# skokec/DAU-ConvNet

Hardware: AMD Instinct MI355X
Metric: DAU fwd+bwd GSamples/s (N*H*W/s) (higher is better)
Workload: dtype f32

## Files before the change

### dau-convnet_amd/csrc/dau_common.hpp

```cpp
#pragma once
#include <hip/hip_runtime.h>
#include <cstddef>
#include <cmath>
#include <cstdint>
#include <type_traits>
#include "dau_conv.h"

#ifdef DAU_TUNING
#include <cstdlib>
#define DAU_TUNE_INT(name, dflt) (getenv(name) ? atoi(getenv(name)) : (dflt))
#define DAU_TUNE_SET(name) (getenv(name) != nullptr)
#else
#define DAU_TUNE_INT(name, dflt) (dflt)
#define DAU_TUNE_SET(name) (false)
#endif

namespace dau {

enum ActFormat : int { kActF32 = 0, kActBF16 = 1, kActF16 = 2 };
__device__ __forceinline__ float f16_bits_to_float(unsigned bits) {
    return (float)__builtin_bit_cast(_Float16, (unsigned short)bits);
}
__device__ __forceinline__ float load_act(const float* base, long idx, int act) {
    if (act == kActF32) return base[idx];
// ... 8 lines not shown
__device__ __forceinline__ typename RawAct<A>::type load_raw(const float* base, long idx) {
    if constexpr (A == kActF32) return base[idx];
    else if constexpr (A == kActBF16) return reinterpret_cast<const unsigned short*>(base)[idx];
    else return F16Bits{reinterpret_cast<const unsigned short*>(base)[idx]};
}
__device__ __forceinline__ float act_of(float v) { return v; }
__device__ __forceinline__ float act_of(unsigned v) { return __uint_as_float(v << 16); }
__device__ __forceinline__ float act_of(F16Bits v) { return f16_bits_to_float(v.bits); }
template <int A>
__device__ __forceinline__ float load_act_t(const float* base, long idx) { return act_of(load_raw<A>(base, idx)); }
template <class F>
__device__ __forceinline__ void with_act(int act, F&& f) {
    if (act == kActBF16) f(std::integral_constant<int, kActBF16>{});
    else if (act == kActF16) f(std::integral_constant<int, kActF16>{});
    else f(std::integral_constant<int, kActF32>{});
}
constexpr int kNhwcArg = 0x100;
template <class T> struct NhwcOut : T {};
template <class T> struct IsNhwcOut : std::false_type {};
template <class T> struct IsNhwcOut<NhwcOut<T>> : std::true_type {};
constexpr int kEpiArg = 0x200;
template <class T> struct EpiOut : T {};
template <class T> struct IsEpiOut : std::false_type {};
template <class T> struct IsEpiOut<EpiOut<T>> : std::true_type {};
template <class T> struct IsNhwcOut<EpiOut<T>> : IsNhwcOut<T> {};
struct Epilogue {
    const float* bias = nullptr;
    bool relu = false;
    const float* residual = nullptr;
    const float* gate = nullptr;
    bool on() const { return bias != nullptr || relu || residual != nullptr || gate != nullptr; }
};
__device__ __forceinline__ float gate_value(float v, float g) { return g <= 0.0f ? 0.0f : v; }
__device__ __forceinline__ float epilogue_value(float v, float b, bool has_bias, bool relu, float r = 0.0f, bool has_res = false) {
    asm("" : "+v"(v));
    if (has_bias) v = v + b;
    asm("" : "+v"(v));
    if (has_res) v = v + r;
    asm("" : "+v"(v));
    return (relu && v <= 0.0f) ? 0.0f : v;
}
__device__ __forceinline__ long nhwc_index(long n, int c, int y, int x, int C, int H, int W) { return ((n * H + y) * W + x) * C + c; }
__device__ __forceinline__ int xcd_contiguous_id(int b, int nblk) {
    const int xcd = b % 8, idx = b / 8, per = nblk / 8, rem = nblk % 8;
    return (xcd < rem ? xcd * (per + 1) : rem * (per + 1) + (xcd - rem) * per) + idx;
}
__device__ __forceinline__ float relu_in(float v, bool on) { return (on && v <= 0.0f) ? 0.0f : v; }
__device__ __forceinline__ float mask_act(float v, bool keep) { return __uint_as_float(__float_as_uint(v) & (keep ? 0xffffffffu : 0u)); }
#ifndef DAU_LOAD_BATCH
#define DAU_LOAD_BATCH 6
#endif
constexpr int kLoadBatch = DAU_LOAD_BATCH;
template <class V, class Load, class Store>
__device__ __forceinline__ void load_phase(int rows_, int cols_, int wave, int nw, int lane, Load&& ld, Store&& st) {
    if (cols_ >= 56) {
        for (int x0 = 0; x0 < cols_; x0 += 64) {
            const int x = x0 + lane, xc = x < cols_ ? x : cols_ - 1;
            for (int r0 = wave; r0 < rows_; r0 += nw * kLoadBatch) {
                V v[kLoadBatch];
#pragma unroll
                for (int u = 0; u < kLoadBatch; ++u) { const int r = r0 + u * nw; v[u] = ld(r < rows_ ? r : rows_ - 1, xc); }
#pragma unroll
                for (int u = 0; u < kLoadBatch; ++u) { const int r = r0 + u * nw; if (r < rows_ && x < cols_) st(r, x, v[u]); }
            }
        }
    } else {
        const int total = rows_ * cols_;
        for (int t0 = wave * 64 + lane; t0 < total; t0 += nw * 64 * kLoadBatch) {
            V v[kLoadBatch];
            int rr[kLoadBatch];
#pragma unroll
            for (int u = 0; u < kLoadBatch; ++u) {
                const int t = t0 + u * nw * 64, tc = t < total ? t : total - 1;
                rr[u] = tc / cols_;
                v[u] = ld(rr[u], tc - rr[u] * cols_);
            }
#pragma unroll
            for (int u = 0; u < kLoadBatch; ++u) { const int t = t0 + u * nw * 64; if (t < total) st(rr[u], t - rr[u] * cols_, v[u]); }
        }
    }
}
__device__ __forceinline__ void store_act(float* base, long idx, float v, bool bf16, bool accumulate) {
    if (!bf16) { base[idx] = accumulate ? base[idx] + v : v; return; }
    unsigned short* p = reinterpret_cast<unsigned short*>(base) + idx;
    if (accumulate) v += __uint_as_float((unsigned)*p << 16);
    unsigned u = __float_as_uint(v);
    u = (v != v) ? 0x7fc00000u : u + 0x7fffu + ((u >> 16) & 1u);
    *p = (unsigned short)(u >> 16);
}
__device__ __forceinline__ unsigned bf16_bits(float v) {
    const unsigned u = __float_as_uint(v);
    return ((v != v) ? 0x7fc00000u : u + 0x7fffu + ((u >> 16) & 1u)) >> 16;
}
__device__ __forceinline__ void store_act_f16(float* base, long idx, float v, bool accumulate) {
    unsigned short* p = reinterpret_cast<unsigned short*>(base) + idx;
    if (accumulate) v += f16_bits_to_float(*p);
    *p = __builtin_bit_cast(unsigned short, (_Float16)v);
}
template <int A>
__device__ __forceinline__ void store_act_t(float* base, long idx, float v, bool accumulate) {
    if constexpr (A == kActF16) store_act_f16(base, idx, v, accumulate);
    else store_act(base, idx, v, A == kActBF16, accumulate);
}
__device__ __forceinline__ void store_act(float* base, long idx, float v, int act, bool accumulate) {
    if (act == kActF16) store_act_f16(base, idx, v, accumulate);
    else store_act(base, idx, v, act == kActBF16, accumulate);
}


constexpr int kMaxBlurSupport = 17;
constexpr int kFilterPlane = kMaxBlurSupport * kMaxBlurSupport;
constexpr int kNumK = 4;
constexpr int kTapPitch = 32;
enum Tap1d { kTapGX = 0, kTapGY, kTapAX, kTapAY, kTapCX, kTapBY, kTapGXR, kTapGYR, kNumTap1d };
constexpr int kTaps1dOffset = 6 * kFilterPlane;
constexpr int kFilterFloats = kTaps1dOffset + kNumTap1d * kTapPitch;

struct Status {
    unsigned int max_abs_mu_bits;
    unsigned int nan_seen;
    unsigned int ticket;
    unsigned int outlier_units;
    unsigned int off_line_units, line_radius;
    unsigned int dot_off_line_units, dot_line_radius;
};
constexpr unsigned kRingTakenBit = 0x80000000u;
static_assert(sizeof(Status) == 32, "the status block is eight words");
static_assert(offsetof(Status, max_abs_mu_bits) == 0 && offsetof(Status, nan_seen) == 4 && offsetof(Status, ticket) == 8 &&
              offsetof(Status, outlier_units) == 12 && offsetof(Status, off_line_units) == 16 && offsetof(Status, line_radius) == 20 &&
              offsetof(Status, dot_off_line_units) == 24 && offsetof(Status, dot_line_radius) == 28,
              "the status block keeps the order of its words");

struct HostStatus {
    unsigned int max_abs_mu_bits, nan_seen, valid, sigma_needed;
    unsigned int bad_max_abs_mu_bits, bad_nan_seen, sigma_worst, pad1;
};
static_assert(sizeof(HostStatus) == 32, "the pinned status mirror is 32 bytes (include/dau_conv.h, Ownership)");

struct Guard {
    const Status* status;
    float lo, hi;
    unsigned cnt_lo = 0u, cnt_hi = 0xffffffffu;
    float cnt_upto = INFINITY;
    int line = 0;
};
__device__ __forceinline__ bool guard_pass(const Guard& g) {
    if (!g.status) return true;
    const float mx = __uint_as_float(g.status->max_abs_mu_bits);
    const unsigned cnt = g.status->outlier_units & ~kRingTakenBit;
    if (!(mx > g.lo && mx <= g.hi && (mx > g.cnt_upto || (cnt >= g.cnt_lo && cnt <= g.cnt_hi)))) return false;
    if (g.line == 0) return true;
    const bool on_line = g.status->off_line_units == 0u;
    return g.line > 0 ? on_line : (mx > (float)-g.line || !on_line);
}

struct UnitRef {
    int ox, oy;
    float w00, w01, w10, w11;
};

struct Shape {
    int N, S, F, G, H, W;
};

void launch_synth_filters(hipStream_t st, const float* sigma_dev, int k, int flags, float* filters6, HostStatus* host_status = nullptr,
                          Status* status = nullptr);
void launch_synth_filters_compact(hipStream_t st, const float* sigma_dev, int k, int flags, float* planes6);
void launch_prepare_units(hipStream_t st, const float* w, const float* mu1, const float* mu2, Shape sh,
                          int ignore, int flags, int bucket, bool transposed_negated, UnitRef* table,
                          Status* status, HostStatus* host_status, int count_ignore = -1, Status* line_status = nullptr,
                          bool line_dot = false);
void launch_finalize_grads(hipStream_t st, const float* r4, const float* w, Shape sh, int ignore, float lr,
                           int need_mask, bool single_dim, float* dw, float* dmu1, float* dmu2, float* dsigma);
void launch_zero_words(hipStream_t st, void* p, size_t bytes);
void launch_blur_direct(hipStream_t st, const float* x, long planes, int H, int W, const float* filters,
                        int nfilt, int k, float* out);
void launch_gather_sum_direct(hipStream_t st, const float* xb, const UnitRef* table, int N, int Sin, int Fout,
                              int G, int H, int W, float* y);
void launch_gather_dot_direct(hipStream_t st, const float* xk4, const float* err, const UnitRef* table, Shape sh,
                              int drop_col, int drop_row, float* r4);

}
```

### dau-convnet_amd/csrc/dau_conv_api.hip

```cpp
#include <cmath>
#include <cstdarg>
#include <cstdio>
#include <algorithm>
#include <atomic>
#include <cstring>
#include <memory>
#include <mutex>
#include <new>
#include <string>
#include <utility>
#include <vector>

#include "dau_common.hpp"
#include "dau_tiled.hpp"

using namespace dau;

namespace {

thread_local std::string g_last_error;

int fail(int code, const char* fmt, ...) {
    char buf[512];
    va_list ap;
    va_start(ap, fmt);
    vsnprintf(buf, sizeof(buf), fmt, ap);
    va_end(ap);
    g_last_error = buf;
    return code;
}

#define DAU_HIP(expr)                                                                        \
    do {                                                                                     \
        hipError_t e_ = (expr);                                                              \
        if (e_ != hipSuccess) return fail(DAU_INTERNAL, "%s failed: %s", #expr, hipGetErrorString(e_)); \
    } while (0)

inline size_t align_up(size_t v, size_t a = 256) { return (v + a - 1) / a * a; }

struct Carver {
    char* base;
    size_t off = 0;
    explicit Carver(void* p) : base(static_cast<char*>(p)) {}
    template <typename T>
    T* take(size_t count) {
        T* p = base ? reinterpret_cast<T*>(base + off) : nullptr;
        off = align_up(off + count * sizeof(T));
        return p;
    }
};

inline const float* slab_ptr(const float* base, size_t elements, size_t esize) {
    return reinterpret_cast<const float*>(reinterpret_cast<const char*>(base) + elements * esize);
}
inline float* slab_ptr(float* base, size_t elements, size_t esize) {
    return reinterpret_cast<float*>(reinterpret_cast<char*>(base) + elements * esize);
}

int edge_disabled(int size) {
    if (size >= 64) return size % 64 == 0;
    if (size >= 32) return size % 32 == 0;
    if (size >= 16) return size % 16 == 0;
    if (size >= 8) return size % 8 == 0;
    return 0;
}

}

enum Member {
    kTiledGather,
    kSplit2, kSplit3, kSplit4,
    kLine4, kLine8,
    kBf16R3, kBf16R4,
    kTiledDot,
    kDotLine4, kDotLine8,
    kSplitDot,
    kWgradR3, kWgradR4,
    kNumMembers
};
enum PassKind { kGatherSum, kGatherDot };
enum Family { kFamTiledGather, kFamDense, kFamTiledDot, kFamSplitDot, kFamWgrad };
struct MemberInfo {
    int kind;
    int family;
    int slot;
    int radius;
    bool ahead;
    bool line;
    int info_bit;
};
constexpr MemberInfo kMember[kNumMembers] = {
    {kGatherSum, kFamTiledGather, 0, 0, false, false, -1},
    {kGatherSum, kFamDense, 0, 2, true, false, 2},
    {kGatherSum, kFamDense, 1, 3, true, false, 3},
    {kGatherSum, kFamDense, 2, 4, true, false, 4},
    {kGatherSum, kFamDense, 3, 4, true, true, 6},
    {kGatherSum, kFamDense, 4, 8, true, true, 7},
    {kGatherSum, kFamDense, 5, 3, true, false, -1},
    {kGatherSum, kFamDense, 6, 4, false, false, -1},
    {kGatherDot, kFamTiledDot, 0, 0, false, false, -1},
    {kGatherDot, kFamSplitDot, 0, 4, true, true, 8},
    {kGatherDot, kFamSplitDot, 1, 8, true, true, 9},
    {kGatherDot, kFamSplitDot, 2, 4, true, false, -1},
    {kGatherDot, kFamWgrad, 0, 3, true, false, -1},
    {kGatherDot, kFamWgrad, 1, 4, false, false, -1},
};
constexpr int kRingInfoBit = 5;
constexpr int kFirst[2] = {kTiledGather, kTiledDot}, kEnd[2] = {kTiledDot, kNumMembers};
enum Dir { kFwd, kDx };

struct DenseFns {
    bool (*configure)(int, int, int, int, int, int, int, int, int, DenseConfig*);
    size_t (*workspace_bytes)(const DenseConfig&);
    void (*init)(const DenseConfig&);
    void (*prepare)(hipStream_t, const DenseConfig&, const float*, const float*, bool, const UnitRef*, void*, const Guard&);
    void (*run)(hipStream_t, const DenseConfig&, float*, void*, const Guard&, const Epilogue&);
};
template <void (*Run)(hipStream_t, const DenseConfig&, float*, void*, const Guard&)>
void run_plain(hipStream_t st, const DenseConfig& c, float* out, void* ws, const Guard& g, const Epilogue&) { Run(st, c, out, ws, g); }
const DenseFns kDense[] = {
    {s2::split_gather_configure, s2::split_gather_workspace_bytes, s2::split_gather_init, s2::split_gather_prepare, s2::split_gather_run},
    {s3::split_gather_configure, s3::split_gather_workspace_bytes, s3::split_gather_init, s3::split_gather_prepare, s3::split_gather_run},
    {s4::split_gather_configure, s4::split_gather_workspace_bytes, s4::split_gather_init, s4::split_gather_prepare, s4::split_gather_run},
    {l4::split_gather_configure, l4::split_gather_workspace_bytes, l4::split_gather_init, l4::split_gather_prepare, l4::split_gather_run},
    {l8::split_gather_configure, l8::split_gather_workspace_bytes, l8::split_gather_init, l8::split_gather_prepare, l8::split_gather_run},
    {r3::dense_gather_configure, r3::dense_gather_workspace_bytes, r3::dense_gather_init, r3::dense_gather_prepare, run_plain<r3::dense_gather_run>},
    {r4::dense_gather_configure, r4::dense_gather_workspace_bytes, r4::dense_gather_init, r4::dense_gather_prepare, run_plain<r4::dense_gather_run>},
};
constexpr int kNumDense = sizeof(kDense) / sizeof(kDense[0]);
struct SplitDotFns {
    bool (*configure)(const Shape&, int, int, SplitDotConfig*);
    size_t (*workspace_bytes)(const SplitDotConfig&);
    void (*init)(const SplitDotConfig&);
    void (*prepare)(hipStream_t, const SplitDotConfig&, const float*, const float*, const float*, int, int, void*, const Guard&);
    void (*run)(hipStream_t, const SplitDotConfig&, const UnitRef*, float*, void*, const Guard&);
};
const SplitDotFns kSplitDotFns[] = {
    {d4::split_dot_configure, d4::split_dot_workspace_bytes, d4::split_dot_init, d4::split_dot_prepare, d4::split_dot_run},
    {d8::split_dot_configure, d8::split_dot_workspace_bytes, d8::split_dot_init, d8::split_dot_prepare, d8::split_dot_run},
    {split_dot_configure, split_dot_workspace_bytes, split_dot_init, split_dot_prepare, split_dot_run},
};
constexpr int kNumSplitDot = sizeof(kSplitDotFns) / sizeof(kSplitDotFns[0]);
struct WgradFns {
    bool (*configure)(const Shape&, int, bool, WgradConfig*);
    size_t (*workspace_bytes)(const WgradConfig&);
    void (*init)(const WgradConfig&);
    void (*run)(hipStream_t, const WgradConfig&, const float*, const float*, const float*, const UnitRef*, int, int, float*, void*,
                const Guard&, int);
};
const WgradFns kWgrad[] = {
    {r3::dense_wgrad_configure, r3::dense_wgrad_workspace_bytes, r3::dense_wgrad_init, r3::dense_wgrad_run},
    {r4::dense_wgrad_configure, r4::dense_wgrad_workspace_bytes, r4::dense_wgrad_init, r4::dense_wgrad_run},
};
static_assert(kMember[kBf16R4].slot == kNumDense - 1 && kMember[kSplitDot].slot == kNumSplitDot - 1 && kMember[kWgradR4].slot == 1,
              "a member's slot is its row in its family's function table");

struct BucketSet {
    int bucket = 0;
    bool has[kNumMembers] = {};
    TiledConfig tiled[2];
    DenseConfig dense[kNumDense][2];
    TiledDotConfig tiled_dot;
    SplitDotConfig sdot[kNumSplitDot];
    WgradConfig wgrad[2];
    int slab_gather = 0, slab_dot = 0;
    bool ring = false;
    unsigned ring_limit = 0;
    RingConfig ringcfg[2];
    const DenseConfig& ring_dense(int dir) const { return dense[kMember[kSplit3].slot][dir]; }
};
constexpr int kRingLimitPermille = 10;
constexpr int kBuckets[] = {4, 8, 16, 18, 20, 24, 32};
constexpr int kNumBuckets = sizeof(kBuckets) / sizeof(kBuckets[0]);

template <class F>
auto with_member(const BucketSet& bs, int m, int dir, F&& f) {
    const int i = kMember[m].slot;
    switch (kMember[m].family) {
    case kFamTiledGather: return f(tiled_gather_workspace_bytes, tiled_gather_init, bs.tiled[dir]);
    case kFamDense: return f(kDense[i].workspace_bytes, kDense[i].init, bs.dense[i][dir]);
    case kFamTiledDot: return f(tiled_dot_workspace_bytes, tiled_dot_init, bs.tiled_dot);
    case kFamSplitDot: return f(kSplitDotFns[i].workspace_bytes, kSplitDotFns[i].init, bs.sdot[i]);
    default: return f(kWgrad[i].workspace_bytes, kWgrad[i].init, bs.wgrad[i]);
    }
}
size_t pass_bytes(const BucketSet& bs, int kind, int dir = kFwd) {
    size_t need = 0;
    for (int m = kFirst[kind]; m < kEnd[kind]; ++m)
        if (bs.has[m]) need = std::max(need, with_member(bs, m, dir, [](auto bytes, auto, const auto& cfg) { return bytes(cfg); }));
    if (kind == kGatherSum && bs.ring) need = std::max(need, s3::split_gather_workspace_bytes(bs.ring_dense(dir)) + ring_workspace_bytes(bs.ringcfg[dir]));
    return need;
}

bool split_pays(double taps, int Cin, int Cout, int G_live, int H, int W) {
    const double hp = (H + 7) / 8 * 8, wp = (W + 7) / 8 * 8, fp = (Cout + 127) / 128 * 128, sp = (Cin + 15) / 16 * 16;
    const double dense = hp * wp * (fp * sp * taps * 3.0 / 16.0 / 0.55 + sp * 430.0);
    const double exact = (double)H * W * Cout * Cin * G_live * 4.0 / ((H < 32 || W < 32) ? 0.45 : 0.60);
    return dense < 1.1 * exact;
}

struct dau_conv_plan {
    dau_conv_desc d;
    Shape sh;
    int bucket;
    int blur_k;
    int drop_col, drop_row;
    int algo_fwd, algo_bwd;
    int nsets = 0;
    BucketSet sets[kNumBuckets];
    bool dynamic = false;
    HostStatus* host_status = nullptr;
    mutable std::atomic<unsigned long long> attrs_devices{0};
    mutable std::mutex attrs_mutex;
    const BucketSet& top() const { return sets[nsets - 1]; }
    long units() const { return (long)sh.S * sh.G * sh.F; }
    size_t esize() const { return (d.flags & (DAU_FLAG_IO_BF16 | DAU_FLAG_IO_F16)) ? 2 : 4; }
    int act() const { return (d.flags & DAU_FLAG_IO_F16) ? kActF16 : (d.flags & DAU_FLAG_IO_BF16) ? kActBF16 : kActF32; }
    mutable bool profiling = false;
    mutable std::vector<std::pair<hipEvent_t, hipEvent_t>> prof_events[DAU_PROFILE_SLOTS];
    mutable size_t prof_used[DAU_PROFILE_SLOTS] = {0, 0, 0};
    mutable int prof_passes[DAU_PROFILE_SLOTS] = {0, 0, 0};
};

namespace {

struct ProfScope {
    const dau_conv_plan* p;
    int slot;
    hipStream_t st;
    hipEvent_t stop = nullptr;
    ProfScope(const dau_conv_plan* plan, int slot_, hipStream_t st_) : p(plan), slot(slot_), st(st_) {
        if (!p->profiling) return;
        auto& pool = p->prof_events[slot];
        size_t& used = p->prof_used[slot];
        if (used == pool.size()) {
            hipEvent_t a, b;
            if (hipEventCreate(&a) != hipSuccess || hipEventCreate(&b) != hipSuccess) return;
            pool.emplace_back(a, b);
        }
        (void)hipEventRecord(pool[used].first, st);
        stop = pool[used].second;
        ++used;
    }
    ~ProfScope() {
        if (stop) (void)hipEventRecord(stop, st);
    }
};

struct Candidate {
    const BucketSet* set;
    Guard guard;
    int member;
    bool ring = false;
};

void clear_host_status(const dau_conv_plan* p) {
    if (!p->host_status) return;
    volatile HostStatus* h = p->host_status;
    h->valid = 0u; h->nan_seen = 0u; h->max_abs_mu_bits = 0u; h->bad_max_abs_mu_bits = 0u; h->bad_nan_seen = 0u;
}
void clear_reported_status(const dau_conv_plan* p, unsigned max_bits, bool nan_seen) {
    if (!p->host_status) return;
    volatile HostStatus* h = p->host_status;
    h->valid = 0u; h->nan_seen = 0u; h->max_abs_mu_bits = 0u;
    if (h->bad_max_abs_mu_bits == max_bits) h->bad_max_abs_mu_bits = 0u;
    if (nan_seen) h->bad_nan_seen = 0u;
}

int status_error(const dau_conv_plan* p, float mx, bool nan_seen) {
    if (nan_seen) return fail(DAU_FAILED_PRECONDITION, "DAUConvOp ERROR: got NaN value in offset (mu1,mu2) variable");
    if (mx > (float)p->bucket)
        return fail(DAU_INVALID_ARGUMENT,
                    "DAUConvOp ERROR: actual offsets (%.3f) larger than what max_kernel_size=%d allows (setup max_kernel_size "
                    "and dau_unit_border_bound correctly to avoid this)",
                    mx, p->d.max_kernel_size);
    return DAU_OK;
}

constexpr int kMaxCandidates = 14;
int pick_candidates(const dau_conv_plan* p, const Status* dev_status, int kind, Candidate out[kMaxCandidates]) {
    const BucketSet* top = &p->top();
    const BucketSet* s0 = &p->sets[0];
    auto member_of = [&](const BucketSet* b) {
        for (int m = kFirst[kind]; m < kEnd[kind]; ++m)
            if (kMember[m].radius && !kMember[m].ahead && b->has[m]) return m;
        return kFirst[kind];
    };
    out[0] = Candidate{top, Guard{nullptr, 0.0f, 0.0f}, member_of(top)};
    if (!p->dynamic) return 1;
    const BucketSet* hinted = nullptr;
    if (p->host_status && p->nsets >= 2) {
        const volatile HostStatus* h = p->host_status;
        float mx = -1.0f;
        if (h->valid == 1u && h->nan_seen == 0u) {
            const unsigned bits = h->max_abs_mu_bits;
            std::memcpy(&mx, &bits, sizeof(float));
        }
        if (mx >= 0.0f)
            for (int i = 0; i + 1 < p->nsets && !hinted; ++i)
                if (mx <= (float)p->sets[i].bucket && p->sets[i].has[kFirst[kind]]) hinted = &p->sets[i];
    }
    int n = 0;
    float lo = -1.0f;
    bool with_ring = false;
    int line_r = 0;
    for (int m = kFirst[kind]; m < kEnd[kind]; ++m) {
        if (!(kMember[m].line && s0->has[m])) continue;
        Guard g{dev_status, (float)line_r - (line_r ? 0.0f : 1.0f), (float)kMember[m].radius};
        g.line = kMember[m].radius;
        out[n++] = Candidate{s0, g, m};
        line_r = kMember[m].radius;
    }
    auto add = [&](const BucketSet* b, int member, float hi) {
        Guard g{dev_status, lo, hi};
        if (lo < (float)line_r) g.line = -line_r;
        if (with_ring && lo < 4.0f) { g.cnt_lo = s0->ring_limit + 1; g.cnt_upto = 4.0f; }
        out[n++] = Candidate{b, g, member};
        lo = hi;
    };
    for (int m = kFirst[kind]; m < kEnd[kind]; ++m) {
        if (!(kMember[m].ahead && s0->has[m]) || kMember[m].line) continue;
        add(s0, m, (float)kMember[m].radius);
        if (m == kSplit3 && s0->ring) {
            Guard g{dev_status, 3.0f, 4.0f, 0u, s0->ring_limit};
            g.line = -line_r;
            out[n++] = Candidate{s0, g, kSplit3, true};
            with_ring = true;
        }
    }
    if (member_of(s0) != kFirst[kind] && hinted != s0 && s0 != top) add(s0, member_of(s0), (float)s0->bucket);
    if (kind == kGatherDot) {
        for (int i = 0; i + 1 < p->nsets; ++i)
            if (p->sets[i].has[kFirst[kind]] && lo < (float)p->sets[i].bucket)
                add(&p->sets[i], member_of(&p->sets[i]), (float)p->sets[i].bucket);
    } else if (hinted && lo < (float)hinted->bucket) add(hinted, member_of(hinted), (float)hinted->bucket);
    if (n == 0) return 1;
    add(top, member_of(top), INFINITY);
    return n;
}

int ensure_attrs(const dau_conv_plan* p) {
    int dev = 0;
    DAU_HIP(hipGetDevice(&dev));
    const unsigned long long bit = 1ull << (dev & 63);
    if (p->attrs_devices.load(std::memory_order_acquire) & bit) return DAU_OK;
    std::lock_guard<std::mutex> lock(p->attrs_mutex);
    if (p->attrs_devices.load(std::memory_order_relaxed) & bit) return DAU_OK;
    (void)hipGetLastError();
    for (int i = 0; i < p->nsets; ++i) {
        const BucketSet& bs = p->sets[i];
        for (int m = 0; m < kNumMembers; ++m) {
            if (!bs.has[m]) continue;
            for (int dir = kFwd; dir <= (kMember[m].kind == kGatherSum ? kDx : kFwd); ++dir)
                with_member(bs, m, dir, [](auto, auto init, const auto& cfg) { init(cfg); });
        }
        if (bs.ring) ring_init();
        const hipError_t e = hipGetLastError();
        if (e != hipSuccess)
            return fail(DAU_INTERNAL, "raising the dynamic-LDS limit of the bucket-%d kernels failed: %s", bs.bucket,
                        hipGetErrorString(e));
    }
    p->attrs_devices.fetch_or(bit, std::memory_order_release);
    return DAU_OK;
}

size_t tiled_pass_bytes(const dau_conv_plan* p, int kind, int dir = kFwd) {
    size_t need = 0;
    for (int i = 0; i < p->nsets; ++i) need = std::max(need, pass_bytes(p->sets[i], kind, dir));
    return need;
}

struct FwdWs {
    Status* status;
    float* filters;
    UnitRef* table;
    void* gather;
    size_t bytes;
};

FwdWs carve_forward(const dau_conv_plan* p, void* ws) {
    Carver c(ws);
    FwdWs w{};
    w.status = c.take<Status>(1);
    w.filters = c.take<float>(kFilterFloats);
    w.table = c.take<UnitRef>(p->units());
    if (p->algo_fwd == DAU_ALGO_TILED) w.gather = c.take<char>(tiled_pass_bytes(p, kGatherSum, kFwd));
    else w.gather = c.take<float>((size_t)p->sh.N * p->sh.S * p->sh.H * p->sh.W);
    w.bytes = c.off;
    return w;
}

struct BwdWs {
    Status* status;
    float* filters;
    UnitRef* table_bare;
    UnitRef* table_t;
    float* r4;
    float* xk4;
    void* gather_dx;
    void* tiled_dot;
    size_t bytes;
};

BwdWs carve_backward(const dau_conv_plan* p, void* ws) {
    Carver c(ws);
    BwdWs w{};
    const Shape& s = p->sh;
    w.status = c.take<Status>(1);
    w.filters = c.take<float>(kFilterFloats);
    w.table_bare = c.take<UnitRef>(p->units());
    w.table_t = c.take<UnitRef>(p->units());
    w.r4 = c.take<float>(kNumK * p->units());
    if (p->algo_bwd == DAU_ALGO_TILED) w.tiled_dot = c.take<char>(tiled_pass_bytes(p, kGatherDot));
    else w.xk4 = c.take<float>((size_t)kNumK * s.N * s.S * s.H * s.W);
    if (p->algo_fwd == DAU_ALGO_TILED) w.gather_dx = c.take<char>(tiled_pass_bytes(p, kGatherSum, kDx));
    else w.gather_dx = c.take<float>((size_t)s.N * s.F * s.H * s.W);
    w.bytes = c.off;
    return w;
}

void run_gather_sum(const dau_conv_plan* p, hipStream_t st, int dir, const float* in, float* out, const float* filters,
                    const UnitRef* table, Status* status, void* ws, const Epilogue& epi = Epilogue{}) {
    const Shape& s = p->sh;
    const int cin = dir == kFwd ? s.S : s.F, cout = dir == kFwd ? s.F : s.S;
    const bool mirrored = dir == kDx;
    if (p->profiling) ++p->prof_passes[dir];
    if (p->algo_fwd != DAU_ALGO_TILED) {
        launch_blur_direct(st, in, (long)s.N * cin, s.H, s.W, filters + (mirrored ? 5 : 0) * kFilterPlane, 1, p->blur_k,
                           static_cast<float*>(ws));
        ProfScope prof(p, dir, st);
        launch_gather_sum_direct(st, static_cast<float*>(ws), table, s.N, cin, cout, s.G, s.H, s.W, out);
        return;
    }
    Candidate cand[kMaxCandidates];
    const int ncand = pick_candidates(p, status, kGatherSum, cand);
    for (int ci = 0; ci < ncand; ++ci) {
        const BucketSet& bs = *cand[ci].set;
        const Guard& g = cand[ci].guard;
        const int m = cand[ci].member;
        const bool ring = cand[ci].ring;
        void* ring_ws = ring ? static_cast<char*>(ws) + s3::split_gather_workspace_bytes(bs.ring_dense(dir)) : nullptr;
        if (ring) ring_build_list(st, bs.ringcfg[dir], table, ring_ws, g);
        for (int n0 = 0; n0 < s.N; n0 += bs.slab_gather) {
            const float* ins = slab_ptr(in, (size_t)n0 * cin * s.H * s.W, p->esize());
            float* outs = slab_ptr(out, (size_t)n0 * cout * s.H * s.W, p->esize());
            Epilogue epis = epi;
            if (epi.residual) epis.residual = slab_ptr(epi.residual, (size_t)n0 * cout * s.H * s.W, p->esize());
            if (epi.gate) epis.gate = slab_ptr(epi.gate, (size_t)n0 * cout * s.H * s.W, p->esize());
            if (m == kTiledGather) {
                const TiledConfig& cfg = bs.tiled[dir];
                const int nwin = tiled_gather_windows(cfg);
                for (int window = 0; window < nwin; ++window) {
                    tiled_gather_prepare(st, cfg, ins, filters, mirrored, table, ws, window, g);
                    ProfScope prof(p, dir, st);
                    tiled_gather_run(st, cfg, outs, ws, window > 0, g, window + 1 == nwin ? epis : Epilogue{});
                }
            } else {
                const DenseFns& fn = kDense[kMember[m].slot];
                const DenseConfig& cfg = bs.dense[kMember[m].slot][dir];
                fn.prepare(st, cfg, ins, filters, mirrored, table, ws, g);
                ProfScope prof(p, dir, st);
                if (ring) {
                    ring_run(st, bs.ringcfg[dir], s3::split_gather_staged(cfg, ws), ring_ws, status, g);
                    s3::split_gather_run_add(st, cfg, outs, ring_partial(bs.ringcfg[dir], ring_ws), ws, g, epis);
                } else {
                    fn.run(st, cfg, outs, ws, g, epis);
                }
            }
        }
    }
}

struct FlagRule {
    int flags, needs, excludes;
    const char* message;
};
constexpr int kWgradFlags = DAU_FLAG_DENSE_WGRAD_NEVER | DAU_FLAG_DENSE_WGRAD_ALWAYS;
constexpr int kNoSplitFlags = DAU_FLAG_DENSE_BF16 | DAU_FLAG_NO_DENSE_SPLIT;
constexpr FlagRule kFlagRules[] = {
    {DAU_FLAG_IO_F16, 0, DAU_FLAG_IO_BF16 | DAU_FLAG_DENSE_BF16 | kWgradFlags,
     "DAU_FLAG_IO_F16 excludes DAU_FLAG_IO_BF16, DAU_FLAG_DENSE_BF16 and DAU_FLAG_DENSE_WGRAD_NEVER / _ALWAYS"},
    {DAU_FLAG_DENSE_BF16, DAU_FLAG_IO_BF16, 0, "DAU_FLAG_DENSE_BF16 needs DAU_FLAG_IO_BF16 (it is the bf16 layer's gather-sum)"},
    {DAU_FLAG_DENSE_SPLIT_F16, 0, kNoSplitFlags, "DAU_FLAG_DENSE_SPLIT_F16 excludes DAU_FLAG_DENSE_BF16 and DAU_FLAG_NO_DENSE_SPLIT"},
    {DAU_FLAG_DENSE_SPLIT_OUTLIERS, 0, kNoSplitFlags, "DAU_FLAG_DENSE_SPLIT_OUTLIERS excludes DAU_FLAG_DENSE_BF16 and DAU_FLAG_NO_DENSE_SPLIT"},
    {DAU_FLAG_DENSE_SPLIT_LINE, DAU_FLAG_SINGLE_DIM_KERNEL, 0, "DAU_FLAG_DENSE_SPLIT_LINE needs DAU_FLAG_SINGLE_DIM_KERNEL"},
    {DAU_FLAG_DENSE_SPLIT_LINE, 0, kNoSplitFlags, "DAU_FLAG_DENSE_SPLIT_LINE excludes DAU_FLAG_DENSE_BF16 and DAU_FLAG_NO_DENSE_SPLIT"},
    {DAU_FLAG_SPLIT_DOT_LINE, DAU_FLAG_SINGLE_DIM_KERNEL, 0, "DAU_FLAG_SPLIT_DOT_LINE needs DAU_FLAG_SINGLE_DIM_KERNEL"},
    {DAU_FLAG_SPLIT_DOT_LINE, DAU_FLAG_USE_INTERPOLATION, 0, "DAU_FLAG_SPLIT_DOT_LINE needs DAU_FLAG_USE_INTERPOLATION"},
    {DAU_FLAG_SPLIT_DOT_LINE, 0, kNoSplitFlags, "DAU_FLAG_SPLIT_DOT_LINE excludes DAU_FLAG_DENSE_BF16 and DAU_FLAG_NO_DENSE_SPLIT"},
    {kWgradFlags, DAU_FLAG_DENSE_BF16, 0, "DAU_FLAG_DENSE_WGRAD_NEVER / _ALWAYS qualify DAU_FLAG_DENSE_BF16 and exclude each other"},
    {DAU_FLAG_DENSE_WGRAD_NEVER, 0, DAU_FLAG_DENSE_WGRAD_ALWAYS, "DAU_FLAG_DENSE_WGRAD_NEVER / _ALWAYS qualify DAU_FLAG_DENSE_BF16 and exclude each other"},
    {DAU_FLAG_IO_NHWC, 0, DAU_FLAG_DENSE_BF16 | kWgradFlags, "DAU_FLAG_IO_NHWC excludes DAU_FLAG_DENSE_BF16 and DAU_FLAG_DENSE_WGRAD_NEVER / _ALWAYS"},
    {DAU_FLAG_INPUT_RELU, 0, DAU_FLAG_DENSE_BF16, "DAU_FLAG_INPUT_RELU excludes DAU_FLAG_DENSE_BF16 (the bf16-product forms have no input prologue)"},
};

int validate_desc(const dau_conv_desc* desc, int& bucket, int& blur_k) {
    if (desc->struct_size != (int32_t)sizeof(dau_conv_desc))
        return fail(DAU_INVALID_ARGUMENT, "dau_conv_desc.struct_size %d != %zu", desc->struct_size, sizeof(dau_conv_desc));
    if (desc->batch < 1 || desc->in_channels < 1 || desc->out_channels < 1 || desc->units_per_channel < 1 ||
        desc->height < 1 || desc->width < 1)
        return fail(DAU_INVALID_ARGUMENT, "all of N,S,F,G,H,W must be >= 1");
    if (desc->number_units_ignore < 0 || desc->number_units_ignore >= desc->units_per_channel)
        return fail(DAU_INVALID_ARGUMENT, "number_units_ignore must be in [0, G)");
    if (desc->max_kernel_size < 3 || desc->max_kernel_size % 2 == 0)
        return fail(DAU_INVALID_ARGUMENT, "kernel_size must be odd and >= 3");
    bucket = 0;
    for (int b : kBuckets)
        if (!bucket && desc->max_kernel_size / 2 <= b) bucket = b;
    if (!bucket)
        return fail(DAU_INVALID_ARGUMENT,
                    "DAUConv: offsets larger than the 32 px the kernels stage (set max_kernel_size <= 65)");
    if (!(desc->sigma_hint > 0.0f))
        return fail(DAU_FAILED_PRECONDITION, "Must use sigma > 0 - initialize it with appropriate value");
    blur_k = dau_conv_filter_support(desc->sigma_hint);
    if (blur_k > kMaxBlurSupport)
        return fail(DAU_INVALID_ARGUMENT, "sigma %.3f needs a %dx%d prefilter; at most %dx%d is supported", desc->sigma_hint,
                    blur_k, blur_k, kMaxBlurSupport, kMaxBlurSupport);
    if (desc->algo < DAU_ALGO_AUTO || desc->algo > DAU_ALGO_TILED) return fail(DAU_INVALID_ARGUMENT, "unknown algo");
    for (const FlagRule& r : kFlagRules)
        if ((desc->flags & r.flags) && ((desc->flags & r.needs) != r.needs || (desc->flags & r.excludes)))
            return fail(DAU_INVALID_ARGUMENT, "%s", r.message);
    return DAU_OK;
}

void configure_set(const dau_conv_plan& p, double budget_bytes, BucketSet& bs) {
    const Shape& s = p.sh;
    const int flags = p.d.flags, b = bs.bucket, blur_k = p.blur_k, act = p.act(), ignore = p.d.number_units_ignore;
    const bool want_dense = (flags & DAU_FLAG_DENSE_BF16) && p.d.algo != DAU_ALGO_DIRECT;
    const bool split_forced = (flags & DAU_FLAG_DENSE_SPLIT_F16) != 0;
    const bool split_allowed = !(flags & kNoSplitFlags) && p.d.algo != DAU_ALGO_DIRECT;
    const int g_live = s.G - ignore;
    const long live_units = (long)s.S * s.F * g_live, ignored_units = (long)s.S * s.F * ignore;
    auto line_wanted = [&](int m, int flag) {
        return (flags & flag) && !(flags & DAU_FLAG_STATIC_BUCKET) && (kMember[m].radius == 4 || (p.bucket >= 8 && bs.has[m - 1]));
    };
    auto pays = [&](double taps) {
        return split_forced || (split_pays(taps, s.S, s.F, g_live, s.H, s.W) && split_pays(taps, s.F, s.S, g_live, s.H, s.W));
    };
    auto configure_dense = [&](int m, int n) {
        const int i = kMember[m].slot, r = kMember[m].radius;
        return kDense[i].configure(n, s.S, s.F, s.G, s.H, s.W, r, blur_k, act, &bs.dense[i][kFwd]) &&
               kDense[i].configure(n, s.F, s.S, s.G, s.H, s.W, r, blur_k, act, &bs.dense[i][kDx]);
    };
    auto configure_gather = [&](int n) {
        bs.has[kTiledGather] = tiled_gather_configure(n, s.S, s.F, s.G, s.H, s.W, b, blur_k, act, &bs.tiled[kFwd]) &&
                               tiled_gather_configure(n, s.F, s.S, s.G, s.H, s.W, b, blur_k, act, &bs.tiled[kDx]);
        const bool dense_set = b == 4 && bs.has[kTiledGather];
        for (int m = kBf16R4; m >= kSplit2; --m) {
            if (kMember[m].line) continue;
            const double side = 2.0 * kMember[m].radius + 1;
            const bool want = m == kBf16R4 ? want_dense : m == kBf16R3 ? bs.has[kBf16R4] : split_allowed && pays(side * side);
            bs.has[m] = dense_set && want && configure_dense(m, n);
        }
        for (int m = kLine4; m <= kLine8; ++m)
            bs.has[m] = dense_set && line_wanted(m, DAU_FLAG_DENSE_SPLIT_LINE) && split_allowed && pays(2.0 * kMember[m].radius + 1) &&
                        configure_dense(m, n);
        bs.ring = (flags & DAU_FLAG_DENSE_SPLIT_OUTLIERS) && bs.has[kSplit3];
        if (bs.ring) {
            bs.ring_limit = (unsigned)(live_units * DAU_TUNE_INT("DAU_RING_LIMIT_PERMILLE", kRingLimitPermille) / 1000);
            for (int dir : {kFwd, kDx}) ring_configure(bs.ring_dense(dir), (long)bs.ring_limit + ignored_units, &bs.ringcfg[dir]);
        }
        return std::max(pass_bytes(bs, kGatherSum, kFwd), pass_bytes(bs, kGatherSum, kDx));
    };
    auto configure_dot = [&](int n) {
        Shape sn = s; sn.N = n;
        bs.has[kTiledDot] = tiled_dot_configure(sn, b, blur_k, act, ignore, &bs.tiled_dot);
        return pass_bytes(bs, kGatherDot);
    };
    auto pick_slab = [&](auto&& configure) {
        int chosen = s.N;
        for (int n = s.N; n >= 2; --n) {
            if (s.N % n || (n != s.N && (n & 1))) continue;
            chosen = n;
            if ((double)configure(n) <= budget_bytes) break;
        }
        configure(chosen);
        return chosen;
    };
    bs.slab_gather = pick_slab(configure_gather);
    bs.slab_dot = pick_slab(configure_dot);
    const bool whole_dot = b == 4 && bs.has[kTiledDot] && bs.slab_dot == s.N;
    const int min_units = (flags & DAU_FLAG_DENSE_WGRAD_NEVER) ? 1 << 30 : (flags & DAU_FLAG_DENSE_WGRAD_ALWAYS) ? 1 : 3;
    for (int m = kWgradR4; m >= kWgradR3; --m) {
        const WgradFns& fn = kWgrad[kMember[m].slot];
        WgradConfig& cfg = bs.wgrad[kMember[m].slot];
        const bool want = m == kWgradR4 ? whole_dot && bs.has[kBf16R4] && s.G >= min_units : bs.has[kWgradR4] && bs.has[kBf16R3];
        bs.has[m] = want && fn.configure(s, blur_k, (flags & DAU_FLAG_IO_BF16) != 0, &cfg) && (double)fn.workspace_bytes(cfg) <= budget_bytes;
    }
    const bool interp2d = (flags & DAU_FLAG_USE_INTERPOLATION) && !(flags & DAU_FLAG_SINGLE_DIM_KERNEL);
    const bool fill = 4 * s.G >= 3 * 4 * ((s.G + 3) / 4);
    for (int m = kDotLine4; m <= kSplitDot; ++m) {
        const SplitDotFns& fn = kSplitDotFns[kMember[m].slot];
        SplitDotConfig& cfg = bs.sdot[kMember[m].slot];
        const bool want = kMember[m].line ? line_wanted(m, DAU_FLAG_SPLIT_DOT_LINE) : interp2d;
        bs.has[m] = split_allowed && whole_dot && (split_forced || fill) && want && fn.configure(s, blur_k, act, &cfg) &&
                    (double)fn.workspace_bytes(cfg) <= budget_bytes;
    }
    const int nhwc = (flags & DAU_FLAG_IO_NHWC) != 0, in_relu = (flags & DAU_FLAG_INPUT_RELU) != 0;
    auto mark = [&](auto& cfg, bool stages_x) { cfg.nhwc = nhwc; cfg.in_relu = stages_x && in_relu; };
    for (int dir : {kFwd, kDx}) {
        mark(bs.tiled[dir], dir == kFwd);
        for (DenseConfig* cfg : bs.dense) mark(cfg[dir], dir == kFwd);
    }
    mark(bs.tiled_dot, true);
    for (SplitDotConfig& cfg : bs.sdot) mark(cfg, true);
}

int finish_plan(dau_conv_plan* p) {
    const int flags = p->d.flags, algo = p->d.algo;
    const bool fwd_ok = p->top().has[kTiledGather], dot_ok = p->top().has[kTiledDot];
    const struct { int flag; const char* name; } tiled_only[] = {
        {DAU_FLAG_IO_F16, "DAU_FLAG_IO_F16"}, {DAU_FLAG_IO_BF16, "DAU_FLAG_IO_BF16"}, {DAU_FLAG_IO_NHWC, "DAU_FLAG_IO_NHWC"},
        {DAU_FLAG_INPUT_RELU, "DAU_FLAG_INPUT_RELU"}};
    for (const auto& t : tiled_only)
        if ((flags & t.flag) && (algo == DAU_ALGO_DIRECT || !(fwd_ok && dot_ok)))
            return fail(DAU_INVALID_ARGUMENT, "%s needs the tiled kernels, which do not support this shape / algo", t.name);
    if (algo == DAU_ALGO_TILED && !(fwd_ok && dot_ok)) return fail(DAU_INVALID_ARGUMENT, "DAU_ALGO_TILED does not support this shape");
    p->algo_fwd = (algo != DAU_ALGO_DIRECT && fwd_ok) ? DAU_ALGO_TILED : DAU_ALGO_DIRECT;
    p->algo_bwd = (algo != DAU_ALGO_DIRECT && dot_ok) ? DAU_ALGO_TILED : DAU_ALGO_DIRECT;
    bool ahead = false;
    for (int m = 0; m < kNumMembers; ++m) ahead = ahead || (kMember[m].ahead && p->sets[0].has[m]);
    p->dynamic = (p->nsets > 1 || ahead) && !(flags & DAU_FLAG_STATIC_BUCKET) &&
                 (p->algo_fwd == DAU_ALGO_TILED || p->algo_bwd == DAU_ALGO_TILED);
    if (!p->dynamic || p->algo_fwd != DAU_ALGO_TILED) p->sets[0].ring = false;
    return DAU_OK;
}

}

extern "C" {

int dau_conv_abi_version(void) { return DAU_CONV_ABI_VERSION; }

#ifndef DAU_BUILD_ID
#define DAU_BUILD_ID "unknown"
#endif
const char* dau_conv_build_id(void) { return DAU_BUILD_ID; }

const char* dau_conv_last_error(void) { return g_last_error.c_str(); }

int dau_conv_filter_support(float sigma) { return 2 * (int)std::ceil(5.0f * sigma) + 1; }

int dau_conv_plan_create(const dau_conv_desc* desc, dau_conv_plan** plan_out) {
    if (!desc || !plan_out) return fail(DAU_INVALID_ARGUMENT, "null argument");
    int bucket, blur_k;
    if (int rc = validate_desc(desc, bucket, blur_k)) return rc;

    std::unique_ptr<dau_conv_plan> p(new (std::nothrow) dau_conv_plan());
    if (!p) return fail(DAU_INTERNAL, "out of host memory");
    p->d = *desc;
    p->sh = Shape{desc->batch, desc->in_channels, desc->out_channels, desc->units_per_channel, desc->height, desc->width};
    p->bucket = bucket;
    p->blur_k = blur_k;
    const bool ut = desc->flags & DAU_FLAG_UNIT_TESTING;
    p->drop_col = ut ? edge_disabled(desc->width) : 0;
    p->drop_row = ut ? edge_disabled(desc->height) : 0;

    const char* budget_env = getenv("DAU_WORKSPACE_BUDGET_GB");
    const double budget_bytes = (budget_env ? atof(budget_env) : 12.0) * 1e9;
    for (int b : kBuckets) {
        if (b > bucket) break;
        BucketSet& bs = p->sets[p->nsets++];
        bs.bucket = b;
        configure_set(*p, budget_bytes, bs);
    }
    if (int rc = finish_plan(p.get())) return rc;
    void* hs = nullptr;
    if (hipHostMalloc(&hs, sizeof(HostStatus), hipHostMallocPortable | hipHostMallocMapped) == hipSuccess && hs) {
        std::memset(hs, 0, sizeof(HostStatus));
        p->host_status = static_cast<HostStatus*>(hs);
    } else {
        (void)hipGetLastError();
    }
    *plan_out = p.release();
    return DAU_OK;
}

int dau_conv_plan_destroy(dau_conv_plan* plan) {
    if (plan) {
        for (auto& pool : plan->prof_events)
            for (auto& ev : pool) { (void)hipEventDestroy(ev.first); (void)hipEventDestroy(ev.second); }
        if (plan->host_status) (void)hipHostFree(plan->host_status);
    }
    delete plan;
    return DAU_OK;
}

int dau_conv_profile_begin(dau_conv_plan* plan) {
    if (!plan) return fail(DAU_INVALID_ARGUMENT, "null argument");
    for (size_t& u : plan->prof_used) u = 0;
    for (int& n : plan->prof_passes) n = 0;
    plan->profiling = true;
    return DAU_OK;
}

int dau_conv_profile_end(dau_conv_plan* plan, double* ms_out, int32_t* passes_out) {
    if (!plan || !ms_out || !passes_out) return fail(DAU_INVALID_ARGUMENT, "null argument");
    plan->profiling = false;
    for (int slot = 0; slot < DAU_PROFILE_SLOTS; ++slot) {
        double total = 0.0;
        for (size_t i = 0; i < plan->prof_used[slot]; ++i) {
            auto& ev = plan->prof_events[slot][i];
            DAU_HIP(hipEventSynchronize(ev.second));
            float ms = 0.0f;
            DAU_HIP(hipEventElapsedTime(&ms, ev.first, ev.second));
            total += ms;
        }
        ms_out[slot] = total;
        passes_out[slot] = plan->prof_passes[slot];
        plan->prof_used[slot] = 0;
        plan->prof_passes[slot] = 0;
    }
    return DAU_OK;
}

int dau_conv_plan_get_info(const dau_conv_plan* plan, dau_conv_plan_info* info) {
    if (!plan || !info) return fail(DAU_INVALID_ARGUMENT, "null argument");
    info->offset_bucket = plan->bucket;
    info->blur_support = plan->blur_k;
    info->algo_forward = plan->algo_fwd;
    info->algo_backward = plan->algo_bwd;
    info->drop_last_col = plan->drop_col;
    info->drop_last_row = plan->drop_row;
    const BucketSet& top = plan->top();
    const bool* s0 = plan->sets[0].has;
    const bool tiled_fwd = plan->algo_fwd == DAU_ALGO_TILED;
    info->gather_patch = tiled_fwd ? top.tiled[kFwd].tiles_x * top.tiled[kFwd].tile_w : 0;
    info->gather_stack = tiled_fwd ? top.tiled[kFwd].stack : 0;
    info->dot_windows = plan->algo_bwd == DAU_ALGO_TILED ? top.tiled_dot.windows : 0;
    info->gather_windows = tiled_fwd ? top.tiled[kFwd].windows : 0;
    info->bucket_sets = plan->dynamic ? plan->nsets : 1;
    const bool dense_reachable = s0[kBf16R4] && (plan->nsets == 1 || plan->dynamic);
    info->gather_dense_bf16 = dense_reachable ? (s0[kWgradR4] ? 2 : 1) : 0;
    info->batch_slab_gather = top.slab_gather;
    info->batch_slab_dot = top.slab_dot;
    info->dot_region = top.has[kTiledDot] ? top.tiled_dot.region_cols * 100 + top.tiled_dot.region_rows : 0;
    info->gather_fblock = tiled_fwd ? top.tiled[kFwd].fblock : 0;
    info->gather_variant = tiled_fwd ? top.tiled[kFwd].variant : -1;
    info->dense_bf16_radius3 = dense_reachable && plan->dynamic && s0[kBf16R3] ? (s0[kWgradR3] ? 2 : 1) : 0;
    info->gather_dense_split = plan->sets[0].ring ? 1 << kRingInfoBit : 0;
    const bool tiled_pass[2] = {tiled_fwd, plan->algo_bwd == DAU_ALGO_TILED};
    for (int m = 0; m < kNumMembers; ++m)
        if (kMember[m].info_bit >= 0 && s0[m] && plan->dynamic && tiled_pass[kMember[m].kind])
            info->gather_dense_split |= 1 << kMember[m].info_bit;
    return DAU_OK;
}

int dau_conv_split_dot_geometry(const dau_conv_plan* plan, int32_t* region_width, int32_t* strip_items, int32_t* strip_k_steps) {
    if (!plan) return fail(DAU_INVALID_ARGUMENT, "null argument");
    int rw = 0, items = 0, steps = 0;
    for (int i = 0; i < plan->nsets && !rw; ++i) {
        const BucketSet& bs = plan->sets[i];
        if (!bs.has[kSplitDot]) continue;
        const SplitDotConfig& cfg = bs.sdot[kMember[kSplitDot].slot];
        rw = cfg.RW;
        split_dot_strip(cfg, &items, &steps);
    }
    if (region_width) *region_width = rw;
    if (strip_items) *strip_items = items;
    if (strip_k_steps) *strip_k_steps = steps;
    return DAU_OK;
}

int dau_conv_workspace_bytes(const dau_conv_plan* plan, int pass, size_t* bytes_out) {
    if (!plan || !bytes_out) return fail(DAU_INVALID_ARGUMENT, "null argument");
    if (pass == DAU_PASS_FORWARD) *bytes_out = carve_forward(plan, nullptr).bytes;
    else if (pass == DAU_PASS_BACKWARD) *bytes_out = carve_backward(plan, nullptr).bytes;
    else if (pass == DAU_PASS_EPILOGUE_BACKWARD)
        *bytes_out = epilogue_grad_workspace_bytes(plan->sh.N, plan->sh.F, plan->sh.H, plan->sh.W, plan->act(), plan->d.flags & DAU_FLAG_IO_NHWC);
    else return fail(DAU_INVALID_ARGUMENT, "pass must be DAU_PASS_FORWARD, DAU_PASS_BACKWARD or DAU_PASS_EPILOGUE_BACKWARD");
    return DAU_OK;
}

namespace {
int forward_pass(const dau_conv_plan* p, void* stream, const float* x, const float* w, const float* mu1,
                 const float* mu2, const float* sigma, float* y, void* workspace, size_t workspace_bytes, const Epilogue& epi) {
    if (!p || !x || !w || !mu1 || !mu2 || !sigma || !y || !workspace) return fail(DAU_INVALID_ARGUMENT, "null argument");
    FwdWs ws = carve_forward(p, workspace);
    if (workspace_bytes < ws.bytes)
        return fail(DAU_INVALID_ARGUMENT, "workspace too small: %zu < %zu", workspace_bytes, ws.bytes);
    hipStream_t st = static_cast<hipStream_t>(stream);
    if (int rc = ensure_attrs(p)) return rc;
    launch_synth_filters(st, sigma, p->blur_k, p->d.flags, ws.filters, p->host_status, ws.status);
    launch_prepare_units(st, w, mu1, mu2, p->sh, p->d.number_units_ignore, p->d.flags, p->bucket, false, ws.table, ws.status,
                         p->host_status, -1, p->sets[0].has[kLine4] ? ws.status : nullptr);
    run_gather_sum(p, st, kFwd, x, y, ws.filters, ws.table, ws.status, ws.gather, epi);
    DAU_HIP(hipPeekAtLastError());
    return DAU_OK;
}
}

int dau_conv_forward(const dau_conv_plan* p, void* stream, const float* x, const float* w, const float* mu1,
                     const float* mu2, const float* sigma, float* y, void* workspace, size_t workspace_bytes) {
    return forward_pass(p, stream, x, w, mu1, mu2, sigma, y, workspace, workspace_bytes, Epilogue{});
}

namespace {
int fused_store_supported(const dau_conv_plan* p, int epilogue, const char* what, const char* bf16_has) {
    if (!p) return fail(DAU_INVALID_ARGUMENT, "null argument");
    if (epilogue & ~(DAU_EPILOGUE_BIAS | DAU_EPILOGUE_RELU))
        return fail(DAU_INVALID_ARGUMENT, "unknown epilogue bits 0x%x (DAU_EPILOGUE_BIAS | DAU_EPILOGUE_RELU)", epilogue);
    if (p->algo_fwd != DAU_ALGO_TILED)
        return fail(DAU_INVALID_ARGUMENT, "the direct kernels take no fused %s (this plan's forward pass runs on them)", what);
    if (p->d.flags & DAU_FLAG_DENSE_BF16)
        return fail(DAU_INVALID_ARGUMENT, "DAU_FLAG_DENSE_BF16 plans take no fused %s (the bf16-product forms have %s)", what, bf16_has);
    return DAU_OK;
}
}

int dau_conv_epilogue_supported(const dau_conv_plan* p, int epilogue) { return fused_store_supported(p, epilogue, "epilogue", "none"); }

int dau_conv_forward_residual(const dau_conv_plan* p, void* stream, const float* x, const float* w, const float* mu1,
                              const float* mu2, const float* sigma, const float* bias, const float* residual, int epilogue,
                              float* y, void* workspace, size_t workspace_bytes) {
    Epilogue epi;
    if (residual || epilogue) {
        if (int rc = residual ? fused_store_supported(p, epilogue, "residual", "no epilogue") : dau_conv_epilogue_supported(p, epilogue)) return rc;
        if ((epilogue & DAU_EPILOGUE_BIAS) && !bias) return fail(DAU_INVALID_ARGUMENT, "DAU_EPILOGUE_BIAS without a bias");
        epi.bias = (epilogue & DAU_EPILOGUE_BIAS) ? bias : nullptr;
        epi.relu = (epilogue & DAU_EPILOGUE_RELU) != 0;
        epi.residual = residual;
    }
    return forward_pass(p, stream, x, w, mu1, mu2, sigma, y, workspace, workspace_bytes, epi);
}

int dau_conv_forward_epilogue(const dau_conv_plan* p, void* stream, const float* x, const float* w, const float* mu1,
                              const float* mu2, const float* sigma, const float* bias, int epilogue, float* y,
                              void* workspace, size_t workspace_bytes) {
    return dau_conv_forward_residual(p, stream, x, w, mu1, mu2, sigma, bias, nullptr, epilogue, y, workspace, workspace_bytes);
}

int dau_conv_epilogue_backward(const dau_conv_plan* p, void* stream, const float* dy, const float* y, int epilogue, float* dz,
                               float* dbias, void* workspace, size_t workspace_bytes) {
    if (!p || !dy) return fail(DAU_INVALID_ARGUMENT, "null argument");
    if (epilogue & ~(DAU_EPILOGUE_BIAS | DAU_EPILOGUE_RELU))
        return fail(DAU_INVALID_ARGUMENT, "unknown epilogue bits 0x%x (DAU_EPILOGUE_BIAS | DAU_EPILOGUE_RELU)", epilogue);
    const bool relu = (epilogue & DAU_EPILOGUE_RELU) != 0;
    if (!(epilogue & DAU_EPILOGUE_BIAS)) dbias = nullptr;
    if (relu && (!y || !dz)) return fail(DAU_INVALID_ARGUMENT, "DAU_EPILOGUE_RELU needs y and dz");
    const bool nhwc = (p->d.flags & DAU_FLAG_IO_NHWC) != 0;
    const Shape& s = p->sh;
    if (dbias) {
        const size_t need = epilogue_grad_workspace_bytes(s.N, s.F, s.H, s.W, p->act(), nhwc);
        if (!workspace || workspace_bytes < need)
            return fail(DAU_INVALID_ARGUMENT, "workspace too small: %zu < %zu", workspace ? workspace_bytes : (size_t)0, need);
    }
    if (!epilogue_grad_run(static_cast<hipStream_t>(stream), s.N, s.F, s.H, s.W, p->act(), nhwc, dy, y, relu, dz, dbias, workspace))
        return fail(DAU_INVALID_ARGUMENT, "activation tensor too large for the epilogue's backward pass");
    DAU_HIP(hipPeekAtLastError());
    return DAU_OK;
}

namespace {

int run_param_sums(const dau_conv_plan* p, hipStream_t st, const float* x, const float* dy, const float* mu1,
                   const float* mu2, const BwdWs& ws, float* r4, int kinds, const float* w = nullptr) {
    const Shape& s = p->sh;
    const bool dot_line = p->algo_bwd == DAU_ALGO_TILED && p->dynamic && p->sets[0].has[kDotLine4];
    launch_prepare_units(st, dot_line ? w : nullptr, mu1, mu2, s, p->d.number_units_ignore, p->d.flags, p->bucket, false, ws.table_bare,
                         ws.status, p->host_status, -1, dot_line ? ws.status : nullptr, true);
    if (p->profiling) ++p->prof_passes[2];
    if (p->algo_bwd == DAU_ALGO_TILED) {
        Candidate cand[kMaxCandidates];
        const int ncand = pick_candidates(p, ws.status, kGatherDot, cand);
        for (int ci = 0; ci < ncand; ++ci) {
            const BucketSet& bs = *cand[ci].set;
            const Guard& g = cand[ci].guard;
            const int m = cand[ci].member;
            const int slot = kMember[m].slot;
            if (kMember[m].family == kFamSplitDot) {
                const SplitDotFns& fn = kSplitDotFns[slot];
                fn.prepare(st, bs.sdot[slot], x, dy, ws.filters, p->drop_col, p->drop_row, ws.tiled_dot, g);
                ProfScope prof(p, 2, st);
                fn.run(st, bs.sdot[slot], ws.table_bare, r4, ws.tiled_dot, g);
            } else if (kMember[m].family == kFamWgrad) {
                ProfScope prof(p, 2, st);
                kWgrad[slot].run(st, bs.wgrad[slot], x, dy, ws.filters, ws.table_bare, p->drop_col, p->drop_row, r4, ws.tiled_dot, g, kinds);
            } else {
                for (int n0 = 0; n0 < s.N; n0 += bs.slab_dot) {
                    tiled_dot_prepare(st, bs.tiled_dot, slab_ptr(x, (size_t)n0 * s.S * s.H * s.W, p->esize()),
                                      slab_ptr(dy, (size_t)n0 * s.F * s.H * s.W, p->esize()), ws.filters, ws.table_bare,
                                      p->drop_col, p->drop_row, ws.tiled_dot, g);
                    ProfScope prof(p, 2, st);
                    tiled_dot_run(st, bs.tiled_dot, r4, ws.tiled_dot, g, n0 > 0);
                }
            }
        }
        if (dot_line) launch_zero_words(st, &ws.status->off_line_units, sizeof(unsigned));
    } else {
        launch_blur_direct(st, x, (long)s.N * s.S, s.H, s.W, ws.filters + 1 * kFilterPlane, kNumK, p->blur_k, ws.xk4);
        ProfScope prof(p, 2, st);
        launch_gather_dot_direct(st, ws.xk4, dy, ws.table_bare, s, p->drop_col, p->drop_row, r4);
    }
    return DAU_OK;
}

int check_backward_ws(const dau_conv_plan* p, void* workspace, size_t workspace_bytes, BwdWs* ws) {
    *ws = carve_backward(p, workspace);
    if (workspace_bytes < ws->bytes)
        return fail(DAU_INVALID_ARGUMENT, "workspace too small: %zu < %zu", workspace_bytes, ws->bytes);
    return DAU_OK;
}

}

int dau_conv_backward(const dau_conv_plan* p, void* stream, const float* x, const float* dy, const float* w,
                      const float* mu1, const float* mu2, const float* sigma, float* dx, float* dw, float* dmu1,
                      float* dmu2, float* dsigma, void* workspace, size_t workspace_bytes, int need_mask) {
    if (p && !x && (p->d.flags & DAU_FLAG_INPUT_RELU) && (need_mask & DAU_NEED_DX))
        return fail(DAU_INVALID_ARGUMENT, "DAU_FLAG_INPUT_RELU: the input-gradient pass masks dx by x, which is null");
    if (!p || !x || !dy || !w || !mu1 || !mu2 || !sigma || !workspace) return fail(DAU_INVALID_ARGUMENT, "null argument");
    if (((need_mask & DAU_NEED_DX) && !dx) || ((need_mask & DAU_NEED_DW) && !dw) ||
        ((need_mask & DAU_NEED_DMU1) && !dmu1) || ((need_mask & DAU_NEED_DMU2) && !dmu2) ||
        ((need_mask & DAU_NEED_DSIGMA) && !dsigma))
        return fail(DAU_INVALID_ARGUMENT, "need_mask asks for a gradient whose output pointer is null");
    BwdWs ws;
    if (int rc = check_backward_ws(p, workspace, workspace_bytes, &ws)) return rc;
    hipStream_t st = static_cast<hipStream_t>(stream);
    const Shape& s = p->sh;
    const int flags = p->d.flags;
    if (int rc = ensure_attrs(p)) return rc;
    launch_synth_filters(st, sigma, p->blur_k, flags, ws.filters, p->host_status, ws.status);

    const int param_mask = DAU_NEED_DW | DAU_NEED_DMU1 | DAU_NEED_DMU2 | DAU_NEED_DSIGMA;
    if (need_mask & param_mask) {
        run_param_sums(p, st, x, dy, mu1, mu2, ws, ws.r4, (need_mask & DAU_NEED_DSIGMA) ? 4 : 3, w);
        launch_finalize_grads(st, ws.r4, w, s, p->d.number_units_ignore, p->d.mu_learning_rate_factor, need_mask,
                              flags & DAU_FLAG_SINGLE_DIM_KERNEL, dw, dmu1, dmu2, dsigma);
    }
    if (need_mask & DAU_NEED_DX) {
        const bool fresh = !(need_mask & param_mask);
        launch_prepare_units(st, w, mu1, mu2, s, 0, flags, p->bucket, true, ws.table_t, fresh ? ws.status : nullptr,
                             p->host_status, p->d.number_units_ignore, p->sets[0].has[kLine4] ? ws.status : nullptr);
        Epilogue gate;
        if (flags & DAU_FLAG_INPUT_RELU) gate.gate = x;
        run_gather_sum(p, st, kDx, dy, dx, ws.filters, ws.table_t, ws.status, ws.gather_dx, gate);
    }
    DAU_HIP(hipPeekAtLastError());
    return DAU_OK;
}

int dau_conv_backward_param_sums(const dau_conv_plan* p, void* stream, const float* x, const float* dy, const float* mu1,
                                 const float* mu2, const float* sigma, float* sums_out, void* workspace,
                                 size_t workspace_bytes) {
    if (!p || !x || !dy || !mu1 || !mu2 || !sigma || !sums_out || !workspace) return fail(DAU_INVALID_ARGUMENT, "null argument");
    BwdWs ws;
    if (int rc = check_backward_ws(p, workspace, workspace_bytes, &ws)) return rc;
    hipStream_t st = static_cast<hipStream_t>(stream);
    if (int rc = ensure_attrs(p)) return rc;
    launch_synth_filters(st, sigma, p->blur_k, p->d.flags, ws.filters, p->host_status, ws.status);
    run_param_sums(p, st, x, dy, mu1, mu2, ws, sums_out, 4);
    DAU_HIP(hipPeekAtLastError());
    return DAU_OK;
}

int dau_conv_finalize_param_grads(const dau_conv_plan* p, void* stream, const float* sums, const float* w, float* dw,
                                  float* dmu1, float* dmu2, float* dsigma, int need_mask) {
    if (!p || !sums || !w) return fail(DAU_INVALID_ARGUMENT, "null argument");
    if (((need_mask & DAU_NEED_DW) && !dw) || ((need_mask & DAU_NEED_DMU1) && !dmu1) ||
        ((need_mask & DAU_NEED_DMU2) && !dmu2) || ((need_mask & DAU_NEED_DSIGMA) && !dsigma))
        return fail(DAU_INVALID_ARGUMENT, "need_mask asks for a gradient whose output pointer is null");
    launch_finalize_grads(static_cast<hipStream_t>(stream), sums, w, p->sh, p->d.number_units_ignore,
                          p->d.mu_learning_rate_factor, need_mask, p->d.flags & DAU_FLAG_SINGLE_DIM_KERNEL, dw, dmu1, dmu2,
                          dsigma);
    DAU_HIP(hipPeekAtLastError());
    return DAU_OK;
}

namespace {
int read_status(const dau_conv_plan* p, void* stream, const void* workspace, Status* h) {
    if (!p || !workspace) return fail(DAU_INVALID_ARGUMENT, "null argument");
    DAU_HIP(hipStreamSynchronize(static_cast<hipStream_t>(stream)));
    DAU_HIP(hipMemcpy(h, workspace, sizeof(Status), hipMemcpyDeviceToHost));
    return DAU_OK;
}
}

int dau_conv_check_status(const dau_conv_plan* p, void* stream, const void* workspace, float* max_abs_mu_out) {
    Status h;
    if (int rc = read_status(p, stream, workspace, &h)) return rc;
    float mx;
    std::memcpy(&mx, &h.max_abs_mu_bits, sizeof(float));
    if (max_abs_mu_out) *max_abs_mu_out = mx;
    if (h.nan_seen || mx > (float)p->bucket) clear_reported_status(p, h.max_abs_mu_bits, h.nan_seen != 0);
    return status_error(p, mx, h.nan_seen != 0);
}

int dau_conv_gather_outlier_status(const dau_conv_plan* p, void* stream, const void* workspace, int32_t* outlier_units,
                                   int32_t* ring_taken) {
    Status h;
    if (int rc = read_status(p, stream, workspace, &h)) return rc;
    if (outlier_units) *outlier_units = (int32_t)(h.outlier_units & ~kRingTakenBit);
    if (ring_taken) *ring_taken = (h.outlier_units & kRingTakenBit) ? 1 : 0;
    return DAU_OK;
}

int dau_conv_gather_line_status(const dau_conv_plan* p, void* stream, const void* workspace, int32_t* off_line_units,
                                int32_t* line_radius_taken) {
    Status h;
    if (int rc = read_status(p, stream, workspace, &h)) return rc;
    if (off_line_units) *off_line_units = (int32_t)h.off_line_units;
    if (line_radius_taken) *line_radius_taken = (int32_t)h.line_radius;
    return DAU_OK;
}

int dau_conv_dot_line_status(const dau_conv_plan* p, void* stream, const void* workspace, int32_t* off_line_units,
                             int32_t* line_radius_taken) {
    Status h;
    if (int rc = read_status(p, stream, workspace, &h)) return rc;
    if (off_line_units) *off_line_units = (int32_t)h.dot_off_line_units;
    if (line_radius_taken) *line_radius_taken = (int32_t)h.dot_line_radius;
    return DAU_OK;
}

int dau_conv_last_status(const dau_conv_plan* p, float* max_abs_mu_out, int32_t* valid_out) {
    if (!p) return fail(DAU_INVALID_ARGUMENT, "null argument");
    if (max_abs_mu_out) *max_abs_mu_out = 0.0f;
    if (valid_out) *valid_out = 0;
    if (!p->host_status) return DAU_OK;
    const volatile HostStatus* h = p->host_status;
    if (h->valid != 1u && h->bad_max_abs_mu_bits == 0u && h->bad_nan_seen == 0u) return DAU_OK;
    const unsigned bad_bits = h->bad_max_abs_mu_bits, bad_nan = h->bad_nan_seen;
    unsigned bits = h->max_abs_mu_bits, nan_seen = h->nan_seen | bad_nan;
    if (bad_bits > bits) bits = bad_bits;
    float mx;
    std::memcpy(&mx, &bits, sizeof(float));
    if (max_abs_mu_out) *max_abs_mu_out = mx;
    if (valid_out) *valid_out = 1;
    if (nan_seen || mx > (float)p->bucket) clear_host_status(p);
    return status_error(p, mx, nan_seen != 0);
}

int dau_conv_sigma_status(const dau_conv_plan* p, int32_t* needed_out, int32_t* planned_out, int32_t* worst_needed_out) {
    if (!p || !needed_out || !planned_out || !worst_needed_out) return fail(DAU_INVALID_ARGUMENT, "null argument");
    *needed_out = 0;
    *planned_out = p->blur_k;
    *worst_needed_out = 0;
    if (!p->host_status) return DAU_OK;
    volatile HostStatus* h = p->host_status;
    *needed_out = (int32_t)h->sigma_needed;
    *worst_needed_out = (int32_t)h->sigma_worst;
    h->sigma_worst = 0u;
    return DAU_OK;
}

int dau_conv_filters(const dau_conv_plan* p, void* stream, const float* sigma, float* filters_out) {
    if (!p || !sigma || !filters_out) return fail(DAU_INVALID_ARGUMENT, "null argument");
    launch_synth_filters_compact(static_cast<hipStream_t>(stream), sigma, p->blur_k, p->d.flags, filters_out);
    DAU_HIP(hipPeekAtLastError());
    return DAU_OK;
}

int dau_conv_unit_table(const dau_conv_plan* p, void* stream, const float* w, const float* mu1, const float* mu2, int form,
                        void* table_out) {
    if (!p || !mu1 || !mu2 || !table_out) return fail(DAU_INVALID_ARGUMENT, "null argument");
    if (form != 0 && form != 1) return fail(DAU_INVALID_ARGUMENT, "form must be 0 ([S][G][F]) or 1 ([F][G][S], negated offsets)");
    launch_prepare_units(static_cast<hipStream_t>(stream), w, mu1, mu2, p->sh, form == 1 ? 0 : p->d.number_units_ignore, p->d.flags,
                         p->bucket, form == 1, static_cast<UnitRef*>(table_out), nullptr, nullptr);
    DAU_HIP(hipPeekAtLastError());
    return DAU_OK;
}

}
```

### dau-convnet_amd/csrc/dau_tiled.hpp

```cpp
#pragma once
#include "dau_common.hpp"

namespace dau {

struct TiledConfig {
    int N, Cin, Cout, G, H, W;
    int R;
    int blur_k;
    int NP;
    int windows;
    int stack;
    int patches;
    int rows, pitch;
    int tiles_x, tiles_y;
    int tile_w;
    int fblock;
    int variant;
    int debug;
    int act;
    int nhwc;
    int in_relu;
};

bool tiled_gather_configure(int N, int Cin, int Cout, int G, int H, int W, int R, int blur_k, int act, TiledConfig* cfg);
size_t tiled_gather_workspace_bytes(const TiledConfig& cfg);
int tiled_gather_windows(const TiledConfig& cfg);
void tiled_gather_prepare(hipStream_t st, const TiledConfig& cfg, const float* in, const float* filters, bool mirrored,
                          const UnitRef* table, void* workspace, int window, const Guard& guard);
void tiled_gather_run(hipStream_t st, const TiledConfig& cfg, float* out, void* workspace, bool accumulate, const Guard& guard,
                      const Epilogue& epi = Epilogue{});
void tiled_gather_init(const TiledConfig& cfg);

struct DenseConfig {
    int N, Cin, Cout, G, H, W;
    int R, blur_k;
    int act;
    int nsub;
    int ftiles;
    int nhwc;
    int in_relu;
};
#define DAU_DECLARE_DENSE_GATHER(NS)                                                                                           \
    namespace NS {                                                                                                            \
    bool dense_gather_configure(int N, int Cin, int Cout, int G, int H, int W, int R, int blur_k, int act, DenseConfig* cfg);  \
    size_t dense_gather_workspace_bytes(const DenseConfig& cfg);                                                              \
    void dense_gather_init(const DenseConfig& cfg);                                                                           \
      \
    void dense_gather_prepare(hipStream_t st, const DenseConfig& cfg, const float* in, const float* filters, bool mirrored,   \
                              const UnitRef* table, void* workspace, const Guard& guard);                                     \
    void dense_gather_run(hipStream_t st, const DenseConfig& cfg, float* out, void* workspace, const Guard& guard);           \
    }
DAU_DECLARE_DENSE_GATHER(r4)
DAU_DECLARE_DENSE_GATHER(r3)

#define DAU_DECLARE_SPLIT_GATHER(NS)                                                                                           \
    namespace NS {                                                                                                            \
    bool split_gather_configure(int N, int Cin, int Cout, int G, int H, int W, int R, int blur_k, int act, DenseConfig* cfg);  \
    size_t split_gather_workspace_bytes(const DenseConfig& cfg);                                                              \
    void split_gather_init(const DenseConfig& cfg);                                                                           \
    void split_gather_prepare(hipStream_t st, const DenseConfig& cfg, const float* in, const float* filters, bool mirrored,   \
                              const UnitRef* table, void* workspace, const Guard& guard);                                     \
                                                      \
    void split_gather_run(hipStream_t st, const DenseConfig& cfg, float* out, void* workspace, const Guard& guard,            \
                          const Epilogue& epi = Epilogue{});                                                                  \
    }
DAU_DECLARE_SPLIT_GATHER(s2)
DAU_DECLARE_SPLIT_GATHER(s3)
DAU_DECLARE_SPLIT_GATHER(s4)
DAU_DECLARE_SPLIT_GATHER(l4)
DAU_DECLARE_SPLIT_GATHER(l8)

struct SplitStaged {
    const float* sx;
    const _Float16* xs;
    int Hs, Ws, nchunk;
};
namespace s3 {
SplitStaged split_gather_staged(const DenseConfig& cfg, const void* workspace);
void split_gather_run_add(hipStream_t st, const DenseConfig& cfg, float* out, const float* partial, void* workspace, const Guard& guard,
                          const Epilogue& epi = Epilogue{});
}
struct RingConfig {
    int N, Cin, Cout, G, H, W;
    int nchunk;
    int capacity;
};
void ring_configure(const DenseConfig& dense, long max_outlier_units, RingConfig* cfg);
size_t ring_workspace_bytes(const RingConfig& cfg);
void ring_build_list(hipStream_t st, const RingConfig& cfg, const UnitRef* table, void* workspace, const Guard& guard);
void ring_run(hipStream_t st, const RingConfig& cfg, const SplitStaged& staged, void* workspace, Status* status, const Guard& guard);
float* ring_partial(const RingConfig& cfg, void* workspace);
void ring_init();

struct TiledDotConfig {
    Shape sh;
    int R, blur_k;
    int NP;
    int variant;
    int windows;
    bool as1, one_tile;
    bool rw8;
    bool ring;
    int region_cols, region_rows;
    int rounds;
    int act;
    int ignore;
    int debug;
    int nhwc;
    int in_relu;
};

bool tiled_dot_configure(const Shape& sh, int R, int blur_k, int act, int ignore, TiledDotConfig* cfg);
size_t tiled_dot_workspace_bytes(const TiledDotConfig& cfg);
void tiled_dot_prepare(hipStream_t st, const TiledDotConfig& cfg, const float* x, const float* dy,
                       const float* filters, const UnitRef* table_bare, int drop_col, int drop_row, void* workspace,
                       const Guard& guard);
void tiled_dot_run(hipStream_t st, const TiledDotConfig& cfg, float* r4, void* workspace, const Guard& guard, bool accumulate);
void tiled_dot_init(const TiledDotConfig& cfg);

void launch_blur4_pack(hipStream_t st, const float* x, const float* filters, int N, int C, int cstride, int H, int W, int Hp,
                       int Wp, int blur_k, int act, float* xk, const Guard& guard, unsigned* kmax = nullptr, bool nhwc = false,
                       bool in_relu = false);
void blur4_pack_init(int blur_k, bool kmax = false, bool nhwc = false);
bool blur4_pack_fits(int blur_k, int Hp, int Wp);

void launch_dot_reduce(hipStream_t st, const void* partial, int partial_f32, long n, int G, int F, int g_split, int slabs0,
                       int slabs1, int zero_from, bool accumulate, float* r4, const Guard& guard);

struct SplitDotConfig {
    Shape sh;
    int blur_k;
    int RW;
    int act;
    int e_limbs;
    int nhwc;
    int in_relu;
};
bool split_dot_configure(const Shape& sh, int blur_k, int act, SplitDotConfig* cfg);
size_t split_dot_workspace_bytes(const SplitDotConfig& cfg);
void split_dot_strip(const SplitDotConfig& cfg, int* items, int* k_steps);
void split_dot_init(const SplitDotConfig& cfg);
void split_dot_prepare(hipStream_t st, const SplitDotConfig& cfg, const float* x, const float* dy, const float* filters,
                       int drop_col, int drop_row, void* workspace, const Guard& guard);
void split_dot_run(hipStream_t st, const SplitDotConfig& cfg, const UnitRef* table, float* r4, void* workspace, const Guard& guard);
#define DAU_DECLARE_SPLIT_DOT_LINE(NS)                                                                                         \
    namespace NS {                                                                                                            \
    bool split_dot_configure(const Shape& sh, int blur_k, int act, SplitDotConfig* cfg);                                      \
    size_t split_dot_workspace_bytes(const SplitDotConfig& cfg);                                                              \
    void split_dot_strip(const SplitDotConfig& cfg, int* items, int* k_steps);                                                \
    void split_dot_init(const SplitDotConfig& cfg);                                                                           \
    void split_dot_prepare(hipStream_t st, const SplitDotConfig& cfg, const float* x, const float* dy, const float* filters,  \
                           int drop_col, int drop_row, void* workspace, const Guard& guard);                                  \
    void split_dot_run(hipStream_t st, const SplitDotConfig& cfg, const UnitRef* table, float* r4, void* workspace,           \
                       const Guard& guard);                                                                                   \
    }
DAU_DECLARE_SPLIT_DOT_LINE(d4)
DAU_DECLARE_SPLIT_DOT_LINE(d8)

struct WgradConfig {
    Shape sh;
    int blur_k;
    int SB, FB, NC;
    int HsT, WsT, WT, nseg;
    int splits;
    int Hp, Wp;
    bool fused;
};
#define DAU_DECLARE_DENSE_WGRAD(NS)                                                                                            \
    namespace NS {                                                                                                            \
    bool dense_wgrad_configure(const Shape& sh, int blur_k, bool bf16, WgradConfig* cfg);                                     \
    size_t dense_wgrad_workspace_bytes(const WgradConfig& cfg);                                                               \
    void dense_wgrad_init(const WgradConfig& cfg);                                                                            \
    void dense_wgrad_run(hipStream_t st, const WgradConfig& cfg, const float* x, const float* dy, const float* filters,       \
                         const UnitRef* table, int drop_col, int drop_row, float* r4, void* workspace, const Guard& guard, int nk); \
    }
DAU_DECLARE_DENSE_WGRAD(r4)
DAU_DECLARE_DENSE_WGRAD(r3)

size_t epilogue_grad_workspace_bytes(long N, int F, int H, int W, int act, bool nhwc);
bool epilogue_grad_run(hipStream_t st, long N, int F, int H, int W, int act, bool nhwc, const float* dy, const float* y, bool relu,
                       float* dz, float* dbias, void* workspace);

}
```

### dau-convnet_amd/csrc/k_dense_split.hip

```cpp
#include <algorithm>
#include <cstdint>
#include <cstdlib>
#include <type_traits>
#include <utility>

#include "dau_tiled.hpp"

#ifndef DAU_SPLIT_R
#define DAU_SPLIT_R 3
#endif
#ifndef DAU_SPLIT_NS
#define DAU_SPLIT_NS s3
#endif

namespace dau {
namespace DAU_SPLIT_NS {

typedef _Float16 f16x8 __attribute__((ext_vector_type(8)));
typedef __attribute__((ext_vector_type(16))) float f32x16;
typedef __attribute__((ext_vector_type(4))) float f32x4;
typedef __attribute__((ext_vector_type(4))) unsigned u32x4;
typedef __attribute__((address_space(3))) void* lds_ptr_t;
typedef __attribute__((address_space(1))) const void* glb_ptr_t;

namespace {

constexpr int kDR = DAU_SPLIT_R;
constexpr int kDK = 2 * kDR + 1;
constexpr int kDSpan = kDK - 1;
#ifndef DAU_SPLIT_1D
#define DAU_SPLIT_1D 0
#endif
constexpr bool kLine = DAU_SPLIT_1D != 0;
#if DAU_SPLIT_1D
#define split_absmax_kernel line_absmax_kernel
#define split_scales_kernel line_scales_kernel
#define split_densify_kernel line_densify_kernel
#define split_stage_kernel line_stage_kernel
#define split_stage_walk_kernel line_stage_walk_kernel
#define split_gather_kernel line_gather_kernel
#endif
constexpr int kDRV = kLine ? 0 : kDR;
constexpr int kDKV = 2 * kDRV + 1;
constexpr int kDSpanV = kDKV - 1;
constexpr int kDTaps = kDKV * kDK;
constexpr int kDRows = 8;
constexpr int kDFB = 128;
constexpr int kAhead = 2;
#ifndef DAU_SPLIT_FLUSH_TAPS
#define DAU_SPLIT_FLUSH_TAPS 0
#endif
constexpr int kFlushTaps = DAU_SPLIT_FLUSH_TAPS > 0 ? DAU_SPLIT_FLUSH_TAPS : kDK;
#ifndef DAU_SPLIT_FLUSH_ROWS
#if DAU_SPLIT_1D
#define DAU_SPLIT_FLUSH_ROWS 1
#else
#define DAU_SPLIT_FLUSH_ROWS 4
#endif
#endif
constexpr int kFlushRows = DAU_SPLIT_FLUSH_ROWS;
#if !defined(DAU_SPLIT_K32)
#if !defined(DAU_SPLIT_MFMA32) && DAU_SPLIT_R == 3 && !DAU_SPLIT_1D
#define DAU_SPLIT_K32 1
#else
#define DAU_SPLIT_K32 0
#endif
#endif
constexpr bool kK32 = DAU_SPLIT_K32 != 0;

inline size_t round_up(size_t v, size_t a) { return (v + a - 1) / a * a; }

struct SplitScales {
    unsigned max_w_bits;
    float sw, inv_sw;
    float pad[5];
};
__host__ __device__ __forceinline__ const float* scales_sx(const SplitScales* sc) { return reinterpret_cast<const float*>(sc + 1); }
__host__ __device__ __forceinline__ const float* scales_inv_sx(const SplitScales* sc, int N) { return reinterpret_cast<const float*>(sc + 1) + N; }
constexpr int kPartials = 1024;
inline int absmax_groups_per_image(int N, long per) {
    const long fit = std::max(1, kPartials / N), want = (per / 4 + 255) / 256 + 1;
    return (int)std::min(fit, want);
}
inline size_t scales_bytes(int N) { return sizeof(SplitScales) + (size_t)2 * N * sizeof(float); }

constexpr int kMaxSub = 4;
struct SplitGeom {
    int sub;
    int nsub_a, nb_a, nsub_b, nb_b;
    int nrb8, nrb4;
    int tall;
    int Hs, Ws, nchunk, CoutP;
    size_t hdr_bytes, xs_bytes, ws_bytes;
};

SplitGeom split_geometry(const DenseConfig& c) {
    SplitGeom g{};
    g.sub = (c.W + 7) / 8;
    const int nblocks = (g.sub + kMaxSub - 1) / kMaxSub, base = g.sub / nblocks, rem = g.sub % nblocks;
    if (rem) { g.nsub_a = base + 1; g.nb_a = rem; g.nsub_b = base; g.nb_b = nblocks - rem; }
    else { g.nsub_a = base; g.nb_a = nblocks; g.nsub_b = 0; g.nb_b = 0; }
    const int left = c.H % kDRows;
    const long wgs = (long)c.N * ((c.H + kDRows - 1) / kDRows) * nblocks * ((c.Cout + kDFB - 1) / kDFB);
    const int rows4 = DAU_TUNE_INT("DAU_SPLIT_ROWS4", 1);
    g.nrb4 = (left >= 1 && left <= 4 && rows4 != 0 && (wgs >= 1024 || rows4 == 2)) ? 1 : 0;
    g.nrb8 = c.H / kDRows + (left && !g.nrb4 ? 1 : 0);
    g.Hs = g.nrb8 * kDRows + g.nrb4 * 4 + kDSpanV;
    {
        const int t4 = (c.W + 3) / 4;
        const long rows8 = (long)g.nrb8 * kDRows;
        const long flat = (long)(g.nrb4 ? rows8 + 4 : (c.H + 3) / 4 * 4) * g.sub * 8;
        const long tall = rows8 * t4 * 4 + (g.nrb4 ? 4L * g.sub * 8 : 0);
        const int want = DAU_TUNE_INT("DAU_SPLIT_TALL", 1);
        g.tall = (want != 0 && g.nrb8 > 0 && (t4 == 5 || t4 == 7) && (tall * 20 <= flat * 19 || want == 2)) ? t4 : 0;
    }
    g.Ws = g.sub * 8 + kDSpan;
    g.nchunk = (c.Cin + 15) / 16;
    g.CoutP = (int)round_up(c.Cout, kDFB);
    g.hdr_bytes = round_up(scales_bytes(c.N) + (size_t)2 * (kPartials + c.N) * sizeof(unsigned), 256);
    g.xs_bytes = round_up((size_t)c.N * g.nchunk * 4 * g.Hs * g.Ws * 16 + 4096, 256);
    g.ws_bytes = round_up(((size_t)g.nchunk * kDTaps + 8) * 2 * g.CoutP * 32, 256);
    return g;
}

constexpr int lds_pitch(int nsub) {
    int p = nsub * 8 + kDSpan;
    while (p % 16 != 8) ++p;
    return p;
}
constexpr int lds_pitch_narrow(int ntiles) {
    int p = ntiles * 4 + kDSpan;
    while (p % 16 != 4 && p % 16 != 12) ++p;
    return p;
}

}

__device__ __forceinline__ unsigned finite_bits(unsigned b) { return b < 0x7f800000u ? b : 0u; }

__device__ __forceinline__ long absmax_head(const void* p, long per, int elem_bytes, int vec_bytes) {
    const uintptr_t a = reinterpret_cast<uintptr_t>(p);
    if (a % elem_bytes) return per;
    const long head = (long)((vec_bytes - a % vec_bytes) % vec_bytes) / elem_bytes;
    return head < per ? head : per;
}

__global__ void __launch_bounds__(256) split_absmax_kernel(const float* __restrict__ in, long per, int gpi, int act, const UnitRef* __restrict__ table,
                                                           long units, unsigned* __restrict__ partial, int cap, const Guard guard, int relu_in) {
    if (!guard_pass(guard)) return;
    unsigned mx = 0, mw = 0;
    const unsigned keep = relu_in ? 0xffffffffu : 0x7fffffffu, keep_hi = keep & 0xffff0000u;
    const int n = blockIdx.x / gpi, j = blockIdx.x - n * gpi;
    const long stride = (long)gpi * blockDim.x, t0 = j * (long)blockDim.x + threadIdx.x;
    if (act == kActF16) {
        auto wide = [keep](unsigned h) { return finite_bits(__float_as_uint(f16_bits_to_float(h)) & keep); };
        const unsigned short* e = reinterpret_cast<const unsigned short*>(in) + n * per;
        const long head = absmax_head(e, per, 2, 8), n4 = (per - head) / 4;
        const uint2* p = reinterpret_cast<const uint2*>(e + head);
        for (long i = t0; i < n4; i += stride) {
            const uint2 v = p[i];
            mx = max(mx, max(max(wide(v.x & 0xffffu), wide(v.x >> 16)), max(wide(v.y & 0xffffu), wide(v.y >> 16))));
        }
        for (long i = t0; i < per - n4 * 4; i += stride) mx = max(mx, wide(e[i < head ? i : i + n4 * 4]));
    } else if (act == kActBF16) {
        const unsigned short* e = reinterpret_cast<const unsigned short*>(in) + n * per;
        const long head = absmax_head(e, per, 2, 8), n4 = (per - head) / 4;
        const uint2* p = reinterpret_cast<const uint2*>(e + head);
        for (long i = t0; i < n4; i += stride) {
            const uint2 v = p[i];
            mx = max(mx, max(max(finite_bits((v.x << 16) & keep), finite_bits(v.x & keep_hi)),
                             max(finite_bits((v.y << 16) & keep), finite_bits(v.y & keep_hi))));
        }
        for (long i = t0; i < per - n4 * 4; i += stride) mx = max(mx, finite_bits(((unsigned)e[i < head ? i : i + n4 * 4] << 16) & keep));
    } else {
        const float* e = in + n * per;
        const long head = absmax_head(e, per, 4, 16), n4 = (per - head) / 4;
        const uint4* p = reinterpret_cast<const uint4*>(e + head);
        for (long i = t0; i < n4; i += stride) {
            const uint4 v = p[i];
            mx = max(mx, max(max(finite_bits(v.x & keep), finite_bits(v.y & keep)),
                             max(finite_bits(v.z & keep), finite_bits(v.w & keep))));
        }
        for (long i = t0; i < per - n4 * 4; i += stride) mx = max(mx, finite_bits(__float_as_uint(e[i < head ? i : i + n4 * 4]) & keep));
    }
    for (long u = blockIdx.x * (long)blockDim.x + threadIdx.x; u < units; u += (long)gridDim.x * blockDim.x) {
        const UnitRef r = table[u];
        mw = max(mw, finite_bits(__float_as_uint(fabsf(r.w00) + fabsf(r.w01) + fabsf(r.w10) + fabsf(r.w11))));
    }
    __shared__ unsigned sx[4], sw[4];
    for (int m = 32; m >= 1; m >>= 1) { mx = max(mx, (unsigned)__shfl_xor((int)mx, m)); mw = max(mw, (unsigned)__shfl_xor((int)mw, m)); }
    if ((threadIdx.x & 63) == 0) { sx[threadIdx.x >> 6] = mx; sw[threadIdx.x >> 6] = mw; }
    __syncthreads();
    if (threadIdx.x == 0) {
        partial[blockIdx.x] = max(max(sx[0], sx[1]), max(sx[2], sx[3]));
        partial[cap + blockIdx.x] = max(max(sw[0], sw[1]), max(sw[2], sw[3]));
    }
}

__device__ __forceinline__ float limb_scale(float m) {
    if (!(m > 0.0f) || !(m < INFINITY)) return 1.0f;
    int e = ilogbf(m);
    e = 13 - e;
    e = e > 100 ? 100 : (e < -100 ? -100 : e);
    return ldexpf(1.0f, e);
}

__global__ void __launch_bounds__(256) split_scales_kernel(const unsigned* __restrict__ partial, int N, int gpi, int cap, int G,
                                                           SplitScales* __restrict__ out, const Guard guard) {
    if (!guard_pass(guard)) return;
    const int n = blockIdx.x;
    const unsigned* src = n < N ? partial + (long)n * gpi : partial + cap;
    const int cnt = n < N ? gpi : N * gpi;
    unsigned m = 0;
    for (int i = threadIdx.x; i < cnt; i += 256) m = max(m, src[i]);
    __shared__ unsigned sm[4];
    for (int k = 32; k >= 1; k >>= 1) m = max(m, (unsigned)__shfl_xor((int)m, k));
    if ((threadIdx.x & 63) == 0) sm[threadIdx.x >> 6] = m;
    __syncthreads();
    if (threadIdx.x == 0) {
        m = max(max(sm[0], sm[1]), max(sm[2], sm[3]));
        float* sx = reinterpret_cast<float*>(out + 1);
        if (n < N) {
            const float s = limb_scale(__uint_as_float(m));
            sx[n] = s; sx[N + n] = 1.0f / s;
        } else {
            const float s = limb_scale(__uint_as_float(m) * (float)G);
            out->max_w_bits = m; out->sw = s; out->inv_sw = 1.0f / s;
            if constexpr (kLine) { if (guard.status) const_cast<Status*>(guard.status)->line_radius = (unsigned)kDR; }
        }
    }
}

constexpr int kScT = 64;
__global__ void __launch_bounds__(kScT) split_densify_kernel(const UnitRef* __restrict__ table, int Cin, int G, int Cout, int CoutP, int nchunk,
                                                             const SplitScales* __restrict__ sc, _Float16* __restrict__ wsd, const Guard guard) {
    __shared__ float acc[kDTaps * kScT];
    if (!guard_pass(guard)) return;
    constexpr int FPB = kScT / 16;
    const int tid = threadIdx.x, sl = tid & 15;
    const int fq = blockIdx.x % (CoutP / FPB), chunk = blockIdx.x / (CoutP / FPB);
    const int f = fq * FPB + (tid >> 4), c = chunk * 16 + sl;
#pragma unroll 7
    for (int tap = 0; tap < kDTaps; ++tap) acc[tap * kScT + tid] = 0.0f;
    if (c < Cin && f < Cout) {
        for (int g = 0; g < G; ++g) {
            const UnitRef u = table[((long)c * G + g) * Cout + f];
            const int ty = u.oy + kDRV, tx = u.ox + kDR;
            const bool y0 = ty >= 0 && ty < kDKV, y1 = ty + 1 >= 0 && ty + 1 < kDKV, x0 = tx >= 0 && tx < kDK, x1 = tx + 1 >= 0 && tx + 1 < kDK;
            if (y0 && x0) acc[(ty * kDK + tx) * kScT + tid] += u.w00;
            if (y0 && x1) acc[(ty * kDK + tx + 1) * kScT + tid] += u.w01;
            if (y1 && x0) acc[((ty + 1) * kDK + tx) * kScT + tid] += u.w10;
            if (y1 && x1) acc[((ty + 1) * kDK + tx + 1) * kScT + tid] += u.w11;
        }
    }
    const float sw = sc->sw;
    _Float16* dst = wsd + ((long)chunk * kDTaps * 2 * CoutP + f) * 16 + sl;
    const long limb = (long)CoutP * 16, tapstride = 2 * limb;
#pragma unroll 7
    for (int tap = 0; tap < kDTaps; ++tap) {
        const float v = acc[tap * kScT + tid] * sw;
        const _Float16 hi = (_Float16)v;
        dst[tap * tapstride] = hi;
        dst[tap * tapstride + limb] = (_Float16)(v - (float)hi);
    }
}

constexpr int kSP = 80;
struct SplitStageArgs {
    const float* in;
    const float* taps;
    const SplitScales* sc;
    _Float16* xs;
    int N, C, H, W, mirrored;
    int Hs, Ws, nchunk;
    int RB, nbands, nsegs;
    int TW;
    int vec;
    int relu_in;
    Guard guard;
};

__device__ __forceinline__ int fast_div(int i, int d, float inv) {
    int q = (int)(((float)i + 0.5f) * inv);
    const int r = i - q * d;
    q += (r >= d) - (r < 0);
    return q;
}

template <int K, int NCH>
__device__ __forceinline__ void split_stage_rows(float* rawl, const float* px, int col, int ch0, int wave, int nw, int lh, int ncols) {
    constexpr int kr = (K - 1) / 2;
    if (col >= ncols) return;
    float gx[K];
#pragma unroll
    for (int j = 0; j < K; ++j) gx[j] = px[j];
    for (int r = wave; r < lh; r += nw) {
        float* row = rawl + (r * 8 + ch0) * kSP + 8 + col;
        float acc[NCH];
#pragma unroll
        for (int ch = 0; ch < NCH; ++ch) {
            acc[ch] = 0.0f;
#pragma unroll
            for (int i = 0; i < K; ++i) acc[ch] = fmaf(row[ch * kSP + i - kr], gx[i], acc[ch]);
        }
#pragma unroll
        for (int ch = 0; ch < NCH; ++ch) row[ch * kSP] = acc[ch];
    }
}

template <int K, int NCH>
__device__ __forceinline__ void split_stage_walk(const float* rawl, const float* py, float sx, int col, int ch0, int ya, int yb,
                                                 int y0, int x0, int x1, int Ws, u32x4* xhi, u32x4* xlo) {
    constexpr int kr = (K - 1) / 2;
    const int x = x0 + col;
    if (x >= x1) return;
    float gy[K];
#pragma unroll
    for (int j = 0; j < K; ++j) gy[j] = py[j];
    float ring[K][NCH];
    const int nin = yb - ya + 2 * kr;
    char* dhi = reinterpret_cast<char*>(xhi + (long)kDRV * Ws + kDR + x) + ch0 * 2;
    char* dlo = reinterpret_cast<char*>(xlo + (long)kDRV * Ws + kDR + x) + ch0 * 2;
    for (int s0 = 0; s0 < nin; s0 += K) {
#pragma unroll
        for (int j = 0; j < K; ++j) {
            const int s = s0 + j;
            if (s < nin) {
                const float* row = rawl + ((ya - y0 + s) * 8 + ch0) * kSP + 8 + col;
#pragma unroll
                for (int ch = 0; ch < NCH; ++ch) ring[j][ch] = row[ch * kSP];
                if (s >= K - 1) {
                    typedef _Float16 f16xn __attribute__((ext_vector_type(NCH)));
                    f16xn oh, ol;
#pragma unroll
                    for (int ch = 0; ch < NCH; ++ch) {
                        float acc = 0.0f;
#pragma unroll
                        for (int i = 0; i < K; ++i) acc = fmaf(ring[(j + 1 + i) % K][ch], gy[i], acc);
                        acc *= sx;
                        const _Float16 hi = (_Float16)acc;
                        oh[ch] = hi;
                        ol[ch] = (_Float16)(acc - (float)hi);
                    }
                    const long o = (long)(ya + s - (K - 1)) * Ws * 16;
                    *reinterpret_cast<f16xn*>(dhi + o) = oh;
                    *reinterpret_cast<f16xn*>(dlo + o) = ol;
                }
            }
        }
    }
}

#ifndef DAU_SPLIT_STAGE_THREADS
#define DAU_SPLIT_STAGE_THREADS 512
#endif
constexpr int kStageThreads = DAU_SPLIT_STAGE_THREADS;
template <int KN, int A>
__global__ void __launch_bounds__(kStageThreads) split_stage_kernel(const SplitStageArgs a) {
    constexpr int K = KN & (kNhwcArg - 1);
    constexpr bool NHWC = (KN & kNhwcArg) != 0;
    extern __shared__ __attribute__((aligned(16))) float rawl[];
    if (!guard_pass(a.guard)) return;
    constexpr int kr = (K - 1) / 2;
    constexpr int PPR = kSP / 4;
    const int lane = threadIdx.x & 63, wave = threadIdx.x >> 6, nw = blockDim.x >> 6;
    int t = blockIdx.x;
    const int seg = t % a.nsegs; t /= a.nsegs;
    const int band = t % a.nbands; t /= a.nbands;
    const int grp = t % (2 * a.nchunk);
    const int n = t / (2 * a.nchunk);
    const int y0 = band * a.RB, y1 = y0 + a.RB < a.H ? y0 + a.RB : a.H;
    const int x0 = seg * 64, x1 = x0 + 64 < a.W ? x0 + 64 : a.W;
    const int lh = y1 - y0 + 2 * kr;
    const long plane = (long)a.H * a.W;
    const bool ri = a.relu_in != 0;
    if constexpr (NHWC) {
        constexpr int CPP = A == kActF32 ? 4 : 8, PARTS = 8 / CPP;
        const int pieces = lh * kSP * PARTS;
        constexpr int UB = (13 * 256 + kStageThreads - 1) / kStageThreads;
        for (int i0 = threadIdx.x; i0 < pieces; i0 += kStageThreads * UB) {
            float v[UB][CPP];
#pragma unroll
            for (int u = 0; u < UB; ++u) {
                const int i = i0 + u * kStageThreads, part = i % PARTS, rj = i / PARTS, r = rj / kSP, j = rj - r * kSP;
// ... 737 lines not shown
        run(std::integral_constant<int, NT0>{});
    }
}

namespace {

template <int NSUB, int RG, bool TT>
constexpr size_t split_lds_bytes() {
    constexpr int plane = (4 * RG + kDSpanV) * (TT ? lds_pitch_narrow(NSUB) : lds_pitch(NSUB));
    return (kK32 ? 4 : 2) * (size_t)((4 * (kK32 ? (plane + 15) / 16 * 16 : plane) + 63) / 64) * 1024;
}

template <int NSUB, int RG, bool TT = false>
void launch_split(hipStream_t st, const SplitArgsEpi* a, int grid, bool h16, bool add, bool nhwc, bool epi) {
    constexpr int NH = NSUB | kNhwcArg;
    constexpr int EP = NSUB | kEpiArg, EH = NH | kEpiArg;
    constexpr size_t lds = split_lds_bytes<NSUB, RG, TT>();
    if (epi) {
        auto kern = h16 ? split_gather_kernel<EP, RG, TT, true> : split_gather_kernel<EP, RG, TT, false>;
        if (nhwc) kern = h16 ? split_gather_kernel<EH, RG, TT, true> : split_gather_kernel<EH, RG, TT, false>;
#if DAU_SPLIT_R == 3
        if (add) kern = h16 ? split_gather_kernel<EP, RG, TT, true, true> : split_gather_kernel<EP, RG, TT, false, true>;
        if (add && nhwc) kern = h16 ? split_gather_kernel<EH, RG, TT, true, true> : split_gather_kernel<EH, RG, TT, false, true>;
#endif
        if (!a) { (void)hipFuncSetAttribute(reinterpret_cast<const void*>(kern), hipFuncAttributeMaxDynamicSharedMemorySize, 160 * 1024); return; }
        hipLaunchKernelGGL(kern, dim3(grid), dim3(512), lds, st, *a);
        return;
    }
    auto kern = h16 ? split_gather_kernel<NSUB, RG, TT, true> : split_gather_kernel<NSUB, RG, TT, false>;
    if (nhwc) kern = h16 ? split_gather_kernel<NH, RG, TT, true> : split_gather_kernel<NH, RG, TT, false>;
#if DAU_SPLIT_R == 3
    if (add) kern = h16 ? split_gather_kernel<NSUB, RG, TT, true, true> : split_gather_kernel<NSUB, RG, TT, false, true>;
    if (add && nhwc) kern = h16 ? split_gather_kernel<NH, RG, TT, true, true> : split_gather_kernel<NH, RG, TT, false, true>;
#endif
    if (!a) { (void)hipFuncSetAttribute(reinterpret_cast<const void*>(kern), hipFuncAttributeMaxDynamicSharedMemorySize, 160 * 1024); return; }
    hipLaunchKernelGGL(kern, dim3(grid), dim3(512), lds, st, static_cast<const SplitArgs&>(*a));
}

void dispatch_split(int nsub, int rg, bool h16, hipStream_t st, const SplitArgsEpi* a, int grid, bool tall, bool add, bool nhwc, bool epi) {
    if (tall) {
        if (nsub == 5) launch_split<5, 2, true>(st, a, grid, h16, add, nhwc, epi);
        else launch_split<7, 2, true>(st, a, grid, h16, add, nhwc, epi);
        return;
    }
    if (rg == 1) {
        switch (nsub) {
            case 1: launch_split<1, 1>(st, a, grid, h16, add, nhwc, epi); break;
            case 2: launch_split<2, 1>(st, a, grid, h16, add, nhwc, epi); break;
            case 3: launch_split<3, 1>(st, a, grid, h16, add, nhwc, epi); break;
            default: launch_split<4, 1>(st, a, grid, h16, add, nhwc, epi); break;
        }
        return;
    }
    switch (nsub) {
        case 1: launch_split<1, 2>(st, a, grid, h16, add, nhwc, epi); break;
        case 2: launch_split<2, 2>(st, a, grid, h16, add, nhwc, epi); break;
        case 3: launch_split<3, 2>(st, a, grid, h16, add, nhwc, epi); break;
        default: launch_split<4, 2>(st, a, grid, h16, add, nhwc, epi); break;
    }
}

const void* stage_for(int blur_k, int act, bool nhwc = false) {
#define DAU_SPLIT_STAGE(K) case K: if (nhwc) return act == kActF16 ? reinterpret_cast<const void*>(split_stage_kernel<K | kNhwcArg, kActF16>) : \
                                          act == kActBF16 ? reinterpret_cast<const void*>(split_stage_kernel<K | kNhwcArg, kActBF16>) : \
                                                            reinterpret_cast<const void*>(split_stage_kernel<K | kNhwcArg, kActF32>); \
                                   return act == kActF16 ? reinterpret_cast<const void*>(split_stage_kernel<K, kActF16>) : \
                                          act == kActBF16 ? reinterpret_cast<const void*>(split_stage_kernel<K, kActBF16>) : \
                                                            reinterpret_cast<const void*>(split_stage_kernel<K, kActF32>)
    switch (blur_k) {
        DAU_SPLIT_STAGE(3);
        DAU_SPLIT_STAGE(5);
        DAU_SPLIT_STAGE(7);
        DAU_SPLIT_STAGE(9);
        DAU_SPLIT_STAGE(11);
        default: return nullptr;
    }
#undef DAU_SPLIT_STAGE
}
const void* stage_walk_for(int blur_k, int act) {
#ifdef DAU_SPLIT_STAGE_REF
    return nullptr;
#else
#define DAU_SPLIT_STAGE_WALK(K) case K: return act == kActF16 ? reinterpret_cast<const void*>(split_stage_walk_kernel<K, kActF16>) : \
                                               act == kActBF16 ? reinterpret_cast<const void*>(split_stage_walk_kernel<K, kActBF16>) : \
                                                                 reinterpret_cast<const void*>(split_stage_walk_kernel<K, kActF32>)
    switch (blur_k) {
        DAU_SPLIT_STAGE_WALK(3);
        DAU_SPLIT_STAGE_WALK(5);
        DAU_SPLIT_STAGE_WALK(7);
        DAU_SPLIT_STAGE_WALK(9);
        DAU_SPLIT_STAGE_WALK(11);
        default: return nullptr;
    }
#undef DAU_SPLIT_STAGE_WALK
#endif
}
void stage_walk_plan(const DenseConfig& c, const SplitGeom& g, SplitStageArgs* s) {
    s->nsegs = (g.Ws + 63) / 64;
    s->TW = (g.Ws + s->nsegs - 1) / s->nsegs;
    s->nsegs = (g.Ws + s->TW - 1) / s->TW;
    const long waves = (long)c.N * 2 * g.nchunk * s->nsegs;
    long nb = (2048 + waves - 1) / waves;
    nb = std::min<long>(nb, std::max(1, g.Hs / (2 * c.blur_k)));
    const int rb = DAU_TUNE_INT("DAU_SPLIT_STAGE_WALK_RB", 0);
    s->RB = rb > 0 ? rb : (int)((g.Hs + nb - 1) / nb);
    s->nbands = (g.Hs + s->RB - 1) / s->RB;
}
void stage_plan(const DenseConfig& c, int* RB, int* nbands, size_t* lds) {
    const int kr = (c.blur_k - 1) / 2;
    int rows = 52 * 1024 / (8 * kSP * 4) - 2 * kr;
    const int rb = DAU_TUNE_INT("DAU_SPLIT_STAGE_RB", 0);
    if (rb > 0) rows = rb;
    rows = rows < 4 ? 4 : rows;
    const int nb = (c.H + rows - 1) / rows;
    *nbands = nb; *RB = (c.H + nb - 1) / nb;
    *lds = (size_t)(*RB + 2 * kr) * 8 * kSP * 4;
}

}

bool split_gather_configure(int N, int Cin, int Cout, int G, int H, int W, int R, int blur_k, int act, DenseConfig* cfg) {
    if (R != kDR || !stage_for(blur_k, act)) return false;
    DenseConfig c{};
    c.N = N; c.Cin = Cin; c.Cout = Cout; c.G = G; c.H = H; c.W = W; c.R = R; c.blur_k = blur_k; c.act = act;
    const SplitGeom g = split_geometry(c);
    c.nsub = g.nsub_a;
    c.ftiles = 1;
    if ((size_t)g.nchunk * 4 * g.Hs * g.Ws > (size_t)1 << 30) return false;
    *cfg = c;
    return true;
}

size_t split_gather_workspace_bytes(const DenseConfig& c) {
    const SplitGeom g = split_geometry(c);
    return g.hdr_bytes + g.xs_bytes + g.ws_bytes;
}

void split_gather_init(const DenseConfig& c) {
    const SplitGeom g = split_geometry(c);
    const bool h16 = c.act == kActF16;
    for (int rg = 1; rg <= 2; ++rg) {
        if (!(rg == 2 ? g.nrb8 : g.nrb4)) continue;
        for (int v = 0; v < (kDR == 3 ? 4 : 2); ++v) {
            const bool add = (v & 2) != 0, epi = (v & 1) != 0;
            if (rg == 2 && g.tall) { dispatch_split(g.tall, 2, h16, nullptr, nullptr, 0, true, add, c.nhwc != 0, epi); continue; }
            dispatch_split(g.nsub_a, rg, h16, nullptr, nullptr, 0, false, add, c.nhwc != 0, epi);
            if (g.nb_b) dispatch_split(g.nsub_b, rg, h16, nullptr, nullptr, 0, false, add, c.nhwc != 0, epi);
        }
    }
    (void)hipFuncSetAttribute(stage_for(c.blur_k, c.act, c.nhwc != 0), hipFuncAttributeMaxDynamicSharedMemorySize, 160 * 1024);
}

void split_gather_prepare(hipStream_t st, const DenseConfig& c, const float* in, const float* filters, bool mirrored,
                          const UnitRef* table, void* workspace, const Guard& guard) {
    const SplitGeom g = split_geometry(c);
    char* ws = static_cast<char*>(workspace);
    SplitScales* sc = reinterpret_cast<SplitScales*>(ws);
    unsigned* partial = reinterpret_cast<unsigned*>(ws + scales_bytes(c.N));
    _Float16* xs = reinterpret_cast<_Float16*>(ws + g.hdr_bytes);
    _Float16* wsd = reinterpret_cast<_Float16*>(ws + g.hdr_bytes + g.xs_bytes);
    const long per = (long)c.Cin * c.H * c.W, units = (long)c.Cin * c.G * c.Cout;
    const int gpi = absmax_groups_per_image(c.N, per), cap = kPartials + c.N;
    hipLaunchKernelGGL(split_absmax_kernel, dim3(c.N * gpi), dim3(256), 0, st, in, per, gpi, c.act, table, units, partial, cap, guard,
                       (c.in_relu && !mirrored) ? 1 : 0);
    hipLaunchKernelGGL(split_scales_kernel, dim3(c.N + 1), dim3(256), 0, st, partial, c.N, gpi, cap, c.G, sc, guard);
    hipLaunchKernelGGL(split_densify_kernel, dim3(g.nchunk * (g.CoutP / (kScT / 16))), dim3(kScT), 0, st, table, c.Cin, c.G, c.Cout, g.CoutP,
                       g.nchunk, sc, wsd, guard);
    SplitStageArgs s{};
    s.in = in; s.taps = filters + kTaps1dOffset; s.sc = sc; s.xs = xs;
    s.N = c.N; s.C = c.Cin; s.H = c.H; s.W = c.W; s.mirrored = mirrored ? 1 : 0;
    s.Hs = g.Hs; s.Ws = g.Ws; s.nchunk = g.nchunk; s.guard = guard;
    s.relu_in = (c.in_relu && !mirrored) ? 1 : 0;
    if (const void* walk = c.nhwc ? nullptr : stage_walk_for(c.blur_k, c.act)) {
        stage_walk_plan(c, g, &s);
        void* args[] = {&s};
        (void)hipLaunchKernel(walk, dim3(c.N * 2 * g.nchunk * s.nbands * s.nsegs), dim3(64), args, 0, st);
        return;
    }
    size_t lds;
    stage_plan(c, &s.RB, &s.nbands, &lds);
    s.nsegs = (c.W + 63) / 64;
    s.vec = c.W % 4 == 0 && reinterpret_cast<uintptr_t>(in) % 16 == 0;
    if (c.nhwc) s.vec = c.Cin % (c.act == kActF32 ? 4 : 8) == 0 && reinterpret_cast<uintptr_t>(in) % 16 == 0;
    void* args[] = {&s};
    (void)hipLaunchKernel(stage_for(c.blur_k, c.act, c.nhwc != 0), dim3(c.N * 2 * g.nchunk * s.nbands * s.nsegs), dim3(kStageThreads), args, lds, st);
}

namespace {
void run_split(hipStream_t st, const DenseConfig& c, float* out, const float* partial, void* workspace, const Guard& guard,
               const Epilogue& epilogue) {
    const SplitGeom g = split_geometry(c);
    const bool add = partial != nullptr;
    const bool h16 = c.act == kActF16;
    char* ws = static_cast<char*>(workspace);
    SplitArgsEpi a{};
    a.sc = reinterpret_cast<const SplitScales*>(ws);
    a.xs = reinterpret_cast<const _Float16*>(ws + g.hdr_bytes);
    a.wsd = reinterpret_cast<const _Float16*>(ws + g.hdr_bytes + g.xs_bytes);
    a.out = out; a.partial = partial;
    a.N = c.N; a.Cout = c.Cout; a.CoutP = g.CoutP; a.H = c.H; a.W = c.W; a.Hs = g.Hs; a.Ws = g.Ws; a.nchunk = g.nchunk;
    a.out_act = c.act; a.guard = guard;
    a.bias = epilogue.bias; a.relu = epilogue.relu ? 1 : 0; a.residual = epilogue.residual;
    const bool epi = epilogue.on();
    const bool nhwc = c.nhwc != 0;
    if (nhwc && c.Cout % 4 == 0 && reinterpret_cast<uintptr_t>(out) % (c.act == kActF32 ? 16 : 8) == 0) a.out_act |= kNhwcVecOut;
    a.res_vec = epilogue.residual && nhwc && c.Cout % 4 == 0 && reinterpret_cast<uintptr_t>(epilogue.residual) % (c.act == kActF32 ? 16 : 8) == 0;
    a.gate = epilogue.gate;
    a.gate_vec = epilogue.gate && nhwc && c.Cout % 4 == 0 && reinterpret_cast<uintptr_t>(epilogue.gate) % (c.act == kActF32 ? 16 : 8) == 0;
    for (int rg = 2; rg >= 1; --rg) {
        a.nrb = rg == 2 ? g.nrb8 : g.nrb4;
        if (!a.nrb) continue;
        a.row0 = rg == 2 ? 0 : g.nrb8 * kDRows;
        if (rg == 2 && g.tall) {
            a.ncb = 1; a.col0 = 0;
            dispatch_split(g.tall, 2, h16, st, &a, c.N * a.nrb * (g.CoutP / kDFB), true, add, nhwc, epi);
            continue;
        }
        a.ncb = g.nb_a; a.col0 = 0;
        dispatch_split(g.nsub_a, rg, h16, st, &a, c.N * a.nrb * g.nb_a * (g.CoutP / kDFB), false, add, nhwc, epi);
        if (g.nb_b) {
            a.ncb = g.nb_b; a.col0 = g.nb_a * g.nsub_a * 8;
            dispatch_split(g.nsub_b, rg, h16, st, &a, c.N * a.nrb * g.nb_b * (g.CoutP / kDFB), false, add, nhwc, epi);
        }
    }
}
}

void split_gather_run(hipStream_t st, const DenseConfig& c, float* out, void* workspace, const Guard& guard, const Epilogue& epi) {
    run_split(st, c, out, nullptr, workspace, guard, epi);
}

#if DAU_SPLIT_R == 3
void split_gather_run_add(hipStream_t st, const DenseConfig& c, float* out, const float* partial, void* workspace, const Guard& guard,
                          const Epilogue& epi) {
    run_split(st, c, out, partial, workspace, guard, epi);
}

SplitStaged split_gather_staged(const DenseConfig& c, const void* workspace) {
    const SplitGeom g = split_geometry(c);
    const char* ws = static_cast<const char*>(workspace);
    SplitStaged s{};
    s.sx = scales_sx(reinterpret_cast<const SplitScales*>(ws));
    s.xs = reinterpret_cast<const _Float16*>(ws + g.hdr_bytes);
    s.Hs = g.Hs; s.Ws = g.Ws; s.nchunk = g.nchunk;
    return s;
}
#endif

}
}
```

### dau-convnet_amd/csrc/k_split_dot.hip

```cpp
#include <algorithm>
#include <cfloat>

#include "dau_tiled.hpp"

#ifndef DAU_SD_RX
#define DAU_SD_RX 4
#endif
#ifndef DAU_SD_1D
#define DAU_SD_1D 0
#endif
#if DAU_SD_1D
#define sd_zero_kernel ld_zero_kernel
#define sd_absmax_x_kernel ld_absmax_x_kernel
#define sd_absmax_e_kernel ld_absmax_e_kernel
#define sd_absmax_nhwc_e_kernel ld_absmax_nhwc_e_kernel
#define sd_stage_x_kernel ld_stage_x_kernel
#define sd_xk_walk_kernel ld_xk_walk_kernel
#define sd_stage_e_kernel ld_stage_e_kernel
#define sd_stage_e1_kernel ld_stage_e1_kernel
#define sd_stage_nhwc_e_kernel ld_stage_nhwc_e_kernel
#define split_gather_dot_kernel line_dot_kernel
#define sd_e1_dot_kernel line_e1_dot_kernel
#endif

namespace dau {
#ifdef DAU_SD_NS
namespace DAU_SD_NS {
#endif

typedef _Float16 h8 __attribute__((ext_vector_type(8)));
typedef float f4s __attribute__((ext_vector_type(4)));

namespace {

constexpr int kSdWaves = 8;
constexpr int kSdAS = 2;
constexpr int kSdGT = 4;
constexpr int kSdSB = kSdWaves * kSdAS;
constexpr int kSdFB = 16;
constexpr bool kSdLine = DAU_SD_1D != 0;
constexpr int kSdRX = DAU_SD_RX;
constexpr int kSdRY = kSdLine ? 0 : kSdRX;
constexpr int kSdRH = 4;
constexpr int kSdFlushItems = 16;
constexpr unsigned kVmcnt0 = 0x0F70, kVmcnt8 = 0x0F78;

inline size_t rup(size_t v, size_t a = 256) { return (v + a - 1) / a * a; }

#ifdef DAU_SD_NO_THIN
constexpr bool kSdThin = false;
#else
constexpr bool kSdThin = true;
#endif

struct SdGeom {
    int Hq, Wq, rq, cq, XTr, XTc, EYs, EXs, octs, nfb, nsb, ngb, items, chunks, per, NP;
    int thin;
    int strip_steps;
};

SdGeom sd_geom(const SplitDotConfig& c) {
    const Shape& s = c.sh;
    SdGeom g{};
    g.Hq = (s.H + 1 + kSdRH - 1) / kSdRH * kSdRH;
    g.Wq = (s.W + 1 + c.RW - 1) / c.RW * c.RW;
    g.rq = g.Hq / kSdRH; g.cq = g.Wq / c.RW;
    g.thin = kSdThin && (s.H + 1) % kSdRH == 1 && g.rq >= 2;
    g.strip_steps = (g.rq - g.thin) * c.RW + g.thin * ((c.RW + kSdRH - 1) / kSdRH);
    g.XTr = g.Hq + 1; g.XTc = g.Wq + 1;
    g.EYs = g.Hq + 2 * kSdRY; g.EXs = g.Wq + 2 * kSdRX;
    g.octs = (s.N + 7) / 8;
    g.NP = (s.N + 1) / 2;
    g.nfb = (s.F + kSdFB - 1) / kSdFB;
    g.nsb = (s.S + kSdSB - 1) / kSdSB;
    g.ngb = (s.G + kSdGT - 1) / kSdGT;
    g.items = g.octs * g.rq * g.cq;
    const int per_chunk = g.nfb * g.nsb * g.ngb;
    int chunks = (1024 + per_chunk - 1) / per_chunk;
    chunks = std::max(1, std::min(chunks, g.items));
    g.per = (g.items + chunks - 1) / chunks;
    g.chunks = (g.items + g.per - 1) / g.per;
    return g;
}

struct SdLayout { size_t maxes_off, xk_off, xs_off, es_off, partial_off, total; };

SdLayout sd_layout(const SplitDotConfig& c, const SdGeom& g) {
    const Shape& s = c.sh;
    SdLayout l{};
    size_t off = 0;
    l.maxes_off = off; off += rup((size_t)(s.S * kNumK + s.F) * 4);
    l.xk_off = off; off += rup((size_t)g.NP * s.S * s.H * s.W * 32);
    l.xs_off = off; off += rup((size_t)g.octs * s.S * kNumK * g.XTr * g.XTc * 32 + 32);
    l.es_off = off; off += rup((size_t)g.octs * g.nfb * g.EYs * g.EXs * 256 * c.e_limbs);
    l.partial_off = off; off += rup((size_t)g.chunks * kNumK * s.S * s.G * s.F * 4);
    l.total = off;
    return l;
}

__device__ __forceinline__ int sd_shift(unsigned maxbits) {
    if (maxbits == 0u) return 0;
    const int e = (int)(maxbits >> 23) - 127;
    const int sh = 13 - e;
    return sh > 120 ? 120 : sh;
}

__device__ __forceinline__ bool finite_abs(float v, float* a) {
    *a = fabsf(v);
    return *a <= FLT_MAX;
}

#ifdef DAU_SD_STAGE_REF
__global__ void __launch_bounds__(256) sd_absmax_x_kernel(const float* __restrict__ xk, int NP, int S, int HW, int split,
                                                          unsigned* __restrict__ xmax, const Guard guard) {
    if (!guard_pass(guard)) return;
    const int s = blockIdx.x % S, part = blockIdx.x / S;
    float m[4] = {0.0f, 0.0f, 0.0f, 0.0f};
    const long per_np = (long)HW * 2;
    const long total = (long)NP * per_np;
    for (long i = part * 256L + threadIdx.x; i < total; i += 256L * split) {
        const long np = i / per_np, r = i - np * per_np;
        const float4 v = reinterpret_cast<const float4*>(xk + ((size_t)np * S + s) * HW * 8)[r];
        const int k0 = (int)(r & 1) * 2;
        float a;
        if (finite_abs(v.x, &a)) m[k0] = fmaxf(m[k0], a);
        if (finite_abs(v.y, &a)) m[k0] = fmaxf(m[k0], a);
        if (finite_abs(v.z, &a)) m[k0 + 1] = fmaxf(m[k0 + 1], a);
        if (finite_abs(v.w, &a)) m[k0 + 1] = fmaxf(m[k0 + 1], a);
    }
    __shared__ float red[4][256];
    for (int k = 0; k < 4; ++k) red[k][threadIdx.x] = m[k];
    __syncthreads();
    for (int w = 128; w >= 1; w >>= 1) {
        if ((int)threadIdx.x < w)
            for (int k = 0; k < 4; ++k) red[k][threadIdx.x] = fmaxf(red[k][threadIdx.x], red[k][threadIdx.x + w]);
        __syncthreads();
    }
    if (threadIdx.x < 4) atomicMax(&xmax[s * kNumK + threadIdx.x], __float_as_uint(red[threadIdx.x][0]));
}
#endif

__device__ __forceinline__ void sd_mark_taken(const Guard& guard) {
    if constexpr (kSdLine) {
        if (guard.status && blockIdx.x == 0 && threadIdx.x == 0) const_cast<Status*>(guard.status)->dot_line_radius = (unsigned)kSdRX;
    }
}

__global__ void __launch_bounds__(256) sd_zero_kernel(unsigned* __restrict__ a, long na, unsigned* __restrict__ b, long nb) {
    for (long i = blockIdx.x * 256L + threadIdx.x; i < na + nb; i += (long)gridDim.x * 256L) {
        if (i < na) a[i] = 0u;
        else b[i - na] = 0u;
    }
}

__global__ void __launch_bounds__(256) sd_absmax_e_kernel(const float* __restrict__ dy, int N, int F, int HW, int split, int act,
                                                          unsigned* __restrict__ emax, const Guard guard) {
    if (!guard_pass(guard)) return;
    sd_mark_taken(guard);
    const int f = blockIdx.x % F, part = blockIdx.x / F;
    float m = 0.0f;
    const long total = (long)N * HW;
    for (long i = part * 256L + threadIdx.x; i < total; i += 256L * split) {
        const long n = i / HW, p = i - n * HW;
        float a;
        if (finite_abs(load_act(dy, ((long)n * F + f) * HW + p, act), &a)) m = fmaxf(m, a);
    }
    for (int o = 32; o >= 1; o >>= 1) m = fmaxf(m, __shfl_xor(m, o));
    if ((threadIdx.x & 63) == 0) atomicMax(&emax[f], __float_as_uint(m));
}

__global__ void __launch_bounds__(256) sd_absmax_nhwc_e_kernel(const float* __restrict__ dy, int N, int F, int HW, int split, int act,
                                                               unsigned* __restrict__ emax, const Guard guard) {
    if (!guard_pass(guard)) return;
    sd_mark_taken(guard);
    const int nfb = (F + 63) / 64;
    const int f = (blockIdx.x % nfb) * 64 + (threadIdx.x & 63), part = blockIdx.x / nfb;
    if (f >= F) return;
    float m = 0.0f;
    const long total = (long)N * HW;
    for (long i = part * 4L + (threadIdx.x >> 6); i < total; i += 4L * split) {
        float a;
        if (finite_abs(load_act(dy, i * F + f, act), &a)) m = fmaxf(m, a);
    }
    atomicMax(&emax[f], __float_as_uint(m));
}

__device__ __forceinline__ void split_limbs(float v, _Float16* hi, _Float16* lo) {
    const _Float16 h = (_Float16)v;
    const float hf = (float)h;
    *hi = h;
    *lo = (hf - hf == 0.0f) ? (_Float16)(v - hf) : (_Float16)0.0f;
}

__global__ void __launch_bounds__(256) sd_stage_x_kernel(const float* __restrict__ xk, const unsigned* __restrict__ xmax, int N,
                                                         int NP, int S, int H, int W, int octs, int XTr, int XTc,
                                                         h8* __restrict__ xs, const Guard guard) {
    if (!guard_pass(guard)) return;
    const long total = (long)octs * S * XTr * XTc;
    for (long idx = blockIdx.x * 256L + threadIdx.x; idx < total; idx += (long)gridDim.x * 256) {
        long t = idx;
        const int tx = (int)(t % XTc); t /= XTc;
        const int ty = (int)(t % XTr); t /= XTr;
        const int s = (int)(t % S);
        const int oct = (int)(t / S);
        const int y = ty - 1, x = tx - 1;
        const bool in = y >= 0 && y < H && x >= 0 && x < W;
        float v[4][8];
#pragma unroll
        for (int p = 0; p < 4; ++p) {
            const int np = oct * 4 + p;
            float4 a = make_float4(0.f, 0.f, 0.f, 0.f), b = a;
            if (in && np < NP) {
                const float4* src = reinterpret_cast<const float4*>(xk + ((((size_t)np * S + s) * H + y) * W + x) * 8);
                a = src[0]; b = src[1];
            }
            v[0][2 * p] = a.x; v[0][2 * p + 1] = a.y; v[1][2 * p] = a.z; v[1][2 * p + 1] = a.w;
            v[2][2 * p] = b.x; v[2][2 * p + 1] = b.y; v[3][2 * p] = b.z; v[3][2 * p + 1] = b.w;
        }
#pragma unroll
        for (int k = 0; k < 4; ++k) {
            const float sc = ldexpf(1.0f, sd_shift(xmax[s * kNumK + k]));
            h8 hi, lo;
#pragma unroll
            for (int i = 0; i < 8; ++i) {
                _Float16 h, l;
                split_limbs(v[k][i] * sc, &h, &l);
                hi[i] = h; lo[i] = l;
            }
            h8* dst = xs + ((((size_t)oct * S + s) * kNumK + k) * XTr * XTc + (size_t)ty * XTc + tx) * 2;
            dst[0] = hi; dst[1] = lo;
        }
    }
}

constexpr int kXwCols = 16;
constexpr int kXwAhead = 3;
constexpr int kXwOut = kNumK * kXwCols * 2 * 4;
struct XkWalkArgs {
    const float* x;
    const float* taps;
    unsigned* xmax;
    h8* xs;
    int N, S, H, W, XTr, XTc, nct, act;
    int relu_in;
    Guard guard;
};

__device__ __forceinline__ void xw_wave_sync() {
    __builtin_amdgcn_fence(__ATOMIC_RELEASE, "wavefront");
    __builtin_amdgcn_wave_barrier();
    __builtin_amdgcn_fence(__ATOMIC_ACQUIRE, "wavefront");
}

typedef float f2 __attribute__((ext_vector_type(2)));
template <int N, class F>
__device__ __forceinline__ void xw_unroll(F&& f) {
    [&]<int... I>(std::integer_sequence<int, I...>) { (f(std::integral_constant<int, I>{}), ...); }(std::make_integer_sequence<int, N>{});
}
template <int HALF>
__device__ __forceinline__ f2 xw_fma_tap(f2 a, unsigned long taps, f2 c) {
    f2 d;
    if constexpr (HALF == 0) asm("v_pk_fma_f32 %0, %1, %2, %3 op_sel_hi:[1,0,1]" : "=v"(d) : "v"(a), "s"(taps), "v"(c));
    else asm("v_pk_fma_f32 %0, %1, %2, %3 op_sel:[0,1,0] op_sel_hi:[1,1,1]" : "=v"(d) : "v"(a), "s"(taps), "v"(c));
    return d;
}

template <int K, bool STORE, int AF>
__device__ __forceinline__ void sd_xk_walk(const XkWalkArgs& a, float* lds) {
    typedef int i4s __attribute__((ext_vector_type(4)));
    typedef _Float16 h2s __attribute__((ext_vector_type(2)));
    typedef typename RawAct<AF>::type Raw;
    constexpr int KR = (K - 1) / 2, CW = kXwCols + 2 * KR, NL = (8 * CW + 63) / 64, kBuf = NL * 64;
    static_assert(kXwAhead < K, "the rows in flight are slots of the unrolled loop");
    int t = blockIdx.x;
    const int ct = t % a.nct; t /= a.nct;
    const int s = t % a.S, oct = t / a.S;
    const int lane = threadIdx.x, c = lane >> 2, p = lane & 3;
    const int H = a.H, W = a.W;
    const int tx0 = ct * kXwCols, x = tx0 + c - 1;
    const float* tp[6] = {a.taps + kTapGX * kTapPitch, a.taps + kTapAX * kTapPitch, a.taps + kTapCX * kTapPitch,
                          a.taps + kTapGY * kTapPitch, a.taps + kTapAY * kTapPitch, a.taps + kTapBY * kTapPitch};
    unsigned long tq[6][(K + 1) / 2];
#pragma unroll
    for (int f = 0; f < 6; ++f)
#pragma unroll
        for (int j = 0; j < (K + 1) / 2; ++j) tq[f][j] = __builtin_bit_cast(unsigned long, f2{tp[f][2 * j], tp[f][2 * j + 1]});
    long poff[NL];
    int lw[NL];
    float mf[NL];
    bool keep[NL];
#pragma unroll
    for (int l = 0; l < NL; ++l) {
        const int tt = l * 64 + lane, tc = tt < 8 * CW ? tt : 8 * CW - 1;
        const int img = tc / CW, col = tc - img * CW;
        const int n = oct * 8 + img;
        const bool second = (n & 1) && n - 1 < a.N;
        const int src = n < a.N ? n : second ? n - 1 : oct * 8;
        const int xx = tx0 - 1 - KR + col;
        keep[l] = tt < 8 * CW && xx >= 0 && xx < W && (n < a.N || second);
        mf[l] = n < a.N ? 1.0f : 0.0f;
        poff[l] = ((long)src * a.S + s) * H * W + (xx < 0 ? 0 : xx < W ? xx : W - 1);
        lw[l] = tt < 8 * CW ? col * 8 + img : tt;
    }
    constexpr unsigned kKeyZero = 1u << 24;
    unsigned km[4] = {kKeyZero, kKeyZero, kKeyZero, kKeyZero}, seen[4] = {0u, 0u, 0u, 0u};
    float sc[4] = {1.0f, 1.0f, 1.0f, 1.0f};
// ... 645 lines not shown
            SD_STEP1(0, k2)
            SD_STEP1(1, k2 + 1)
        }
#undef SD_STEP1
#else
#define SD_NEXT_COL(P, i)                                                                                       \
    aqh[i] = sd_next_col(ahi[P][i], ahi[1 - (P)][i], adx);                                                      \
    aql[i] = sd_next_col(alo[P][i], alo[1 - (P)][i], adx);
#define SD_PAIR(P, rr)                                                                                          \
    {                                                                                                           \
        const size_t an = ioff + (size_t)((rr) + 2) * 4;                                                        \
        (void)an;                                                                                               \
        SD_STEP(2 * (rr), ahi[P], alo[P], SD_NEXT_COL(P, 0) SD_LOAD_A(P, 0, an), SD_NEXT_COL(P, 1) SD_LOAD_A(P, 1, an)) \
        SD_STEP(2 * (rr) + 1, aqh, aql, , )                                                                     \
    }
#define SD_PAIR_LAST(P, rr)                                                                                     \
    {                                                                                                           \
        SD_STEP(2 * (rr), ahi[P], alo[P], SD_NEXT_COL(P, 0) SD_LOAD_NEXT(0, 0, ioff_next), SD_NEXT_COL(P, 1) SD_LOAD_NEXT(0, 1, ioff_next)) \
        SD_STEP(2 * (rr) + 1, aqh, aql, SD_LOAD_NEXT(1, 0, ioff_next + nstep), SD_LOAD_NEXT(1, 1, ioff_next + nstep)) \
    }
        constexpr int kPairs = RW / 2, kLoopPairs = (kPairs - 1) / 2 * 2;
#pragma unroll 1
        for (int r2 = 0; r2 < kLoopPairs; r2 += 2) {
            SD_PAIR(0, r2)
            SD_PAIR(1, r2 + 1)
        }
        if constexpr (kPairs - kLoopPairs == 2) {
            SD_PAIR(0, kPairs - 2)
            SD_PAIR_LAST(1, kPairs - 1)
        } else {
            SD_PAIR_LAST(0, kPairs - 1)
        }
#undef SD_NEXT_COL
#undef SD_PAIR
#undef SD_PAIR_LAST
#endif
            combine();
        }
#undef SD_LOAD_NEXT
#undef SD_LOAD_INTO
#undef SD_READ_B
#undef SD_GROUP
#undef SD_LOAD_A
#undef SD_STEP
        if (++since_flush == kSdFlushItems) { flush(); since_flush = 0; }
    };
    for (int it = it0; it < it1;) {
        const int run_end = a.thin ? min(it1, it + (a.rq - 1 - it % a.rq)) : it1;
        const int full_end = run_end < it1 ? run_end - 1 : run_end;
#pragma unroll 1
        for (; it < full_end; ++it) item(it, std::integral_constant<int, kItemFull>{});
        if (it < run_end) { item(it, std::integral_constant<int, kItemBeforeThin>{}); ++it; }
        if (it < it1) { item(it, std::integral_constant<int, kItemThin>{}); ++it; }
    }
    asm volatile("s_waitcnt vmcnt(0)" ::: "memory");
    if (since_flush) flush();
}

template <int RW>
__global__ void __launch_bounds__(kSdWaves * 64) __attribute__((amdgpu_waves_per_eu(2, 2))) split_gather_dot_kernel(const SdArgs a) {
    sd_dot_body<RW, 2>(a);
}

template <int RW>
__global__ void __launch_bounds__(kSdWaves * 64) __attribute__((amdgpu_waves_per_eu(2, 2))) sd_e1_dot_kernel(const SdArgs a) {
    sd_dot_body<RW, 1>(a);
}

template <int RW, int EL>
void launch_sd(hipStream_t st, const SdArgs* a, int grid) {
    auto kern = [] { if constexpr (EL == 2) return split_gather_dot_kernel<RW>; else return sd_e1_dot_kernel<RW>; }();
    const size_t lds = (size_t)(2 * kSdRH + 2 * kSdRY) * (RW + 2 * kSdRX) * 256 * EL;
    if (!a) { (void)hipFuncSetAttribute(reinterpret_cast<const void*>(kern), hipFuncAttributeMaxDynamicSharedMemorySize, 160 * 1024); return; }
    hipLaunchKernelGGL(kern, dim3(grid), dim3(kSdWaves * 64), lds, st, *a);
}
bool sd_walks(const SplitDotConfig& c) {
#if defined(DAU_SD_XK_COPY) || defined(DAU_SD_STAGE_REF)
    return false;
#else
    const SdGeom g = sd_geom(c);
    const long nct = (g.XTc + kXwCols - 1) / kXwCols;
    return !c.nhwc && (c.blur_k == 5 || c.blur_k == 7 || c.blur_k == 9) && (long)g.octs * c.sh.S * nct < (1L << 31);
#endif
}
template <int K, bool STORE>
void launch_xk_walk(hipStream_t st, const XkWalkArgs& a, int grid) {
    hipLaunchKernelGGL((sd_xk_walk_kernel<K, STORE>), dim3(grid), dim3(64), 0, st, a);
}
template <bool STORE>
void dispatch_xk_walk(hipStream_t st, const SplitDotConfig& c, const SdGeom& g, const float* x, const float* filters, unsigned* xmax,
                      h8* xs, const Guard& guard) {
    XkWalkArgs a{};
    a.x = x; a.taps = filters + kTaps1dOffset; a.xmax = xmax; a.xs = xs;
    a.N = c.sh.N; a.S = c.sh.S; a.H = c.sh.H; a.W = c.sh.W; a.XTr = g.XTr; a.XTc = g.XTc; a.act = c.act; a.relu_in = c.in_relu;
    a.nct = (g.XTc + kXwCols - 1) / kXwCols;
    a.guard = guard;
    const int grid = g.octs * c.sh.S * a.nct;
    if (c.blur_k == 5) launch_xk_walk<5, STORE>(st, a, grid);
    else if (c.blur_k == 7) launch_xk_walk<7, STORE>(st, a, grid);
    else launch_xk_walk<9, STORE>(st, a, grid);
}

void dispatch_sd(int RW, int e_limbs, hipStream_t st, const SdArgs* a, int grid) {
    if (e_limbs == 1) {
        if (RW == 10) launch_sd<10, 1>(st, a, grid);
        else launch_sd<12, 1>(st, a, grid);
    } else {
        if (RW == 10) launch_sd<10, 2>(st, a, grid);
        else launch_sd<12, 2>(st, a, grid);
    }
}

}

bool split_dot_configure(const Shape& sh, int blur_k, int act, SplitDotConfig* cfg) {
    int best = 0;
    long best_cost = 1L << 40;
    for (int rw = 12; rw >= 10; rw -= 2) {
        const long wq = (sh.W + 1 + rw - 1) / rw * rw;
        const long cost = wq * (rw + 2) * (60 / rw);
        if (cost < best_cost) { best_cost = cost; best = rw; }
    }
    if ((size_t)(2 * kSdRH + 2 * kSdRY) * (best + 2 * kSdRX) * 512 > 160 * 1024) return false;
    if (!blur4_pack_fits(blur_k, sh.H, sh.W)) return false;
    SplitDotConfig c{};
    c.sh = sh; c.blur_k = blur_k; c.RW = best; c.act = act;
#ifdef DAU_SD_BF16_E2
    c.e_limbs = 2;
#else
    c.e_limbs = act == kActBF16 ? 1 : 2;
#endif
    const SdGeom g = sd_geom(c);
    if ((long)g.EXs * 512 * 32 > (1L << 31)) return false;
    *cfg = c;
    return true;
}

size_t split_dot_workspace_bytes(const SplitDotConfig& c) { return sd_layout(c, sd_geom(c)).total; }

void split_dot_strip(const SplitDotConfig& c, int* items, int* k_steps) {
    const SdGeom g = sd_geom(c);
    *items = g.rq; *k_steps = g.strip_steps;
}

void split_dot_init(const SplitDotConfig& c) {
    dispatch_sd(c.RW, c.e_limbs, nullptr, nullptr, 0);
#ifndef DAU_SD_STAGE_REF
    blur4_pack_init(c.blur_k, true, c.nhwc != 0);
#else
    blur4_pack_init(c.blur_k, false, c.nhwc != 0);
#endif
}

void split_dot_prepare(hipStream_t st, const SplitDotConfig& c, const float* x, const float* dy, const float* filters,
                       int drop_col, int drop_row, void* workspace, const Guard& guard) {
    const SdGeom g = sd_geom(c);
    const SdLayout l = sd_layout(c, g);
    const Shape& s = c.sh;
    char* ws = static_cast<char*>(workspace);
    unsigned* xmax = reinterpret_cast<unsigned*>(ws + l.maxes_off);
    unsigned* emax = xmax + s.S * kNumK;
    float* xk = reinterpret_cast<float*>(ws + l.xk_off);
    hipLaunchKernelGGL(sd_zero_kernel, dim3(64), dim3(256), 0, st, xmax, (long)(s.S * kNumK + s.F),
                       reinterpret_cast<unsigned*>(ws + l.partial_off), (long)g.chunks * kNumK * s.S * s.G * s.F);
    const int HW = s.H * s.W;
    const bool walks = sd_walks(c);
    h8* xs = reinterpret_cast<h8*>(ws + l.xs_off);
#ifndef DAU_SD_STAGE_REF
    if (walks) dispatch_xk_walk<false>(st, c, g, x, filters, xmax, xs, guard);
    else launch_blur4_pack(st, x, filters, s.N, s.S, s.S, s.H, s.W, s.H, s.W, c.blur_k, c.act, xk, guard, xmax, c.nhwc != 0, c.in_relu != 0);
#else
    launch_blur4_pack(st, x, filters, s.N, s.S, s.S, s.H, s.W, s.H, s.W, c.blur_k, c.act, xk, guard, nullptr, c.nhwc != 0, c.in_relu != 0);
    const int xsplit = std::max(1, std::min(16, 2048 / std::max(1, s.S)));
    hipLaunchKernelGGL(sd_absmax_x_kernel, dim3(s.S * xsplit), dim3(256), 0, st, xk, g.NP, s.S, HW, xsplit, xmax, guard);
#endif
    if (c.nhwc) {
        const int nfb64 = (s.F + 63) / 64;
        const int esplit = (int)std::max(1L, std::min((long)(2048 / nfb64), ((long)s.N * HW + 3) / 4));
        hipLaunchKernelGGL(sd_absmax_nhwc_e_kernel, dim3(nfb64 * esplit), dim3(256), 0, st, dy, s.N, s.F, HW, esplit, c.act, emax, guard);
    } else {
        const int esplit = std::max(1, std::min(16, 2048 / std::max(1, s.F)));
        hipLaunchKernelGGL(sd_absmax_e_kernel, dim3(s.F * esplit), dim3(256), 0, st, dy, s.N, s.F, HW, esplit, c.act, emax, guard);
    }
    if (walks) dispatch_xk_walk<true>(st, c, g, x, filters, xmax, xs, guard);
    else hipLaunchKernelGGL(sd_stage_x_kernel, dim3(8192), dim3(256), 0, st, xk, xmax, s.N, g.NP, s.S, s.H, s.W, g.octs, g.XTr, g.XTc, xs, guard);
    if (c.e_limbs == 1) {
        const int nct = (g.EXs + kSe1TX - 1) / kSe1TX, tx = (g.EXs + nct - 1) / nct;
        if (c.nhwc) {
            hipLaunchKernelGGL(sd_stage_nhwc_e_kernel<1>, dim3((unsigned)(g.octs * g.nfb * g.EYs * nct)), dim3(256), 0, st, dy, emax, s.N, s.F,
                               s.H, s.W, g.nfb, g.EYs, g.EXs, nct, tx, drop_col, drop_row, c.act, reinterpret_cast<h8*>(ws + l.es_off), guard);
            return;
        }
        hipLaunchKernelGGL(sd_stage_e1_kernel, dim3((unsigned)(g.octs * g.nfb * g.EYs * nct)), dim3(256), 0, st, dy, emax, s.N, s.F,
                           s.H, s.W, g.nfb, g.EYs, g.EXs, nct, tx, drop_col, drop_row, c.act, reinterpret_cast<h8*>(ws + l.es_off), guard);
        return;
    }
#ifndef DAU_SD_STAGE_REF
    const int nct = (g.EXs + kSeTX - 1) / kSeTX, tx = (g.EXs + nct - 1) / nct;
    if (c.nhwc) {
        hipLaunchKernelGGL(sd_stage_nhwc_e_kernel<2>, dim3((unsigned)(g.octs * g.nfb * g.EYs * nct)), dim3(256), 0, st, dy, emax, s.N, s.F,
                           s.H, s.W, g.nfb, g.EYs, g.EXs, nct, tx, drop_col, drop_row, c.act, reinterpret_cast<h8*>(ws + l.es_off), guard);
        return;
    }
#ifndef DAU_SD_STAGE_E_ROWS
    SeWalkArgs w{};
    w.dy = dy; w.emax = emax; w.es = reinterpret_cast<h8*>(ws + l.es_off);
    w.N = s.N; w.F = s.F; w.H = s.H; w.W = s.W; w.nfb = g.nfb; w.EYs = g.EYs; w.EXs = g.EXs;
    w.nct = (g.EXs + kSeCols - 1) / kSeCols;
    w.wlim = drop_col ? s.W - 1 : s.W; w.hlim = drop_row ? s.H - 1 : s.H; w.act = c.act; w.guard = guard;
    const long cols = (long)g.octs * g.nfb * w.nct, nb = (5120 + cols - 1) / cols;
    const int rb = DAU_TUNE_INT("DAU_SD_STAGE_E_RB", 0);
    w.RB = rb > 0 ? rb : std::max(4, (int)((g.EYs + nb - 1) / nb));
    w.nbands = (g.EYs + w.RB - 1) / w.RB;
    hipLaunchKernelGGL(sd_stage_e_kernel, dim3((unsigned)(cols * w.nbands)), dim3(64), 0, st, w);
    return;
#else
    hipLaunchKernelGGL(sd_stage_e_kernel, dim3((unsigned)(g.octs * g.nfb * g.EYs * nct)), dim3(256), 0, st, dy, emax, s.N, s.F, s.H,
                       s.W, g.nfb, g.EYs, g.EXs, nct, tx, drop_col, drop_row, c.act, reinterpret_cast<h8*>(ws + l.es_off), guard);
#endif
#else
    hipLaunchKernelGGL(sd_stage_e_kernel, dim3(4096), dim3(256), 0, st, dy, emax, s.N, s.F, s.H, s.W, g.octs, g.nfb, g.EYs, g.EXs,
                       drop_col, drop_row, c.act, c.nhwc, reinterpret_cast<h8*>(ws + l.es_off), guard);
#endif
}

void split_dot_run(hipStream_t st, const SplitDotConfig& c, const UnitRef* table, float* r4, void* workspace, const Guard& guard) {
    const SdGeom g = sd_geom(c);
    const SdLayout l = sd_layout(c, g);
    const Shape& s = c.sh;
    char* ws = static_cast<char*>(workspace);
    SdArgs a{};
    a.xs = reinterpret_cast<const h8*>(ws + l.xs_off);
    a.es = ws + l.es_off;
    a.xmax = reinterpret_cast<const unsigned*>(ws + l.maxes_off);
    a.emax = a.xmax + s.S * kNumK;
    a.table = table;
    a.partial = reinterpret_cast<float*>(ws + l.partial_off);
    a.S = s.S; a.F = s.F; a.G = s.G;
    a.nfb = g.nfb; a.nsb = g.nsb; a.ngb = g.ngb; a.per = g.per; a.items = g.items; a.rq = g.rq; a.cq = g.cq;
    a.XTr = g.XTr; a.XTc = g.XTc; a.EYs = g.EYs; a.EXs = g.EXs;
    a.thin = g.thin;
    a.guard = guard;
    dispatch_sd(c.RW, c.e_limbs, st, &a, g.chunks * g.nfb * g.nsb * g.ngb);
    launch_dot_reduce(st, a.partial, 1, (long)kNumK * s.S * s.G * s.F, s.G, s.F, s.G, g.chunks, g.chunks, s.G, false, r4, guard);
}

#ifdef DAU_SD_NS
}
#endif
}
```

### dau-convnet_amd/dau_conv/_capi.py

```python
import collections
import ctypes
import os
import sys
import threading

import torch

_HERE = os.path.dirname(os.path.abspath(__file__))
_LIB_PATH = os.environ.get("DAU_CONV_LIB") or os.path.join(_HERE, "libdau_conv_hip.so")

DAU_OK, DAU_INVALID_ARGUMENT, DAU_FAILED_PRECONDITION, DAU_INTERNAL = 0, 1, 2, 3

FLAG_USE_INTERPOLATION = 1 << 0
FLAG_UNIT_TESTING = 1 << 1
FLAG_SINGLE_DIM_KERNEL = 1 << 2
FLAG_FORBID_POSITIVE_DIM1 = 1 << 3
FLAG_IO_BF16 = 1 << 4
FLAG_STATIC_BUCKET = 1 << 5
FLAG_DENSE_BF16 = 1 << 6
FLAG_DENSE_WGRAD_NEVER = 1 << 7
FLAG_DENSE_WGRAD_ALWAYS = 1 << 8
FLAG_DENSE_SPLIT_F16 = 1 << 9
FLAG_NO_DENSE_SPLIT = 1 << 10
FLAG_DENSE_SPLIT_LINE = 1 << 15
FLAG_SPLIT_DOT_LINE = 1 << 16
FLAG_DENSE_SPLIT_OUTLIERS = 1 << 12
FLAG_IO_F16 = 1 << 11
FLAG_IO_NHWC = 1 << 13
FLAG_INPUT_RELU = 1 << 14

ALGO_AUTO, ALGO_DIRECT, ALGO_TILED = 0, 1, 2
PASS_FORWARD, PASS_BACKWARD, PASS_EPILOGUE_BACKWARD = 1, 2, 3
EPILOGUE_BIAS, EPILOGUE_RELU = 1, 2
NEED_DX, NEED_DW, NEED_DMU1, NEED_DMU2, NEED_DSIGMA, NEED_ALL = 1, 2, 4, 8, 16, 31


class DAUConvError(RuntimeError):
    code = DAU_INTERNAL


class InvalidArgumentError(DAUConvError, ValueError):
    code = DAU_INVALID_ARGUMENT


class FailedPreconditionError(DAUConvError):
    code = DAU_FAILED_PRECONDITION


class InternalError(DAUConvError):
    code = DAU_INTERNAL


class _Desc(ctypes.Structure):
    _fields_ = [
        ("struct_size", ctypes.c_int32), ("batch", ctypes.c_int32), ("in_channels", ctypes.c_int32),
        ("out_channels", ctypes.c_int32), ("units_per_channel", ctypes.c_int32), ("height", ctypes.c_int32),
        ("width", ctypes.c_int32), ("max_kernel_size", ctypes.c_int32), ("number_units_ignore", ctypes.c_int32),
        ("flags", ctypes.c_int32), ("algo", ctypes.c_int32), ("sigma_hint", ctypes.c_float),
        ("mu_learning_rate_factor", ctypes.c_float),
    ]


class _Info(ctypes.Structure):
    _fields_ = [(n, ctypes.c_int32) for n in
                ("offset_bucket", "blur_support", "algo_forward", "algo_backward", "drop_last_col", "drop_last_row",
                 "gather_patch", "gather_stack", "dot_windows", "gather_windows", "bucket_sets", "gather_dense_bf16", "batch_slab_gather", "batch_slab_dot", "dot_region", "gather_fblock", "gather_variant", "dense_bf16_radius3", "gather_dense_split")]


def _load():
    if not os.path.exists(_LIB_PATH):
        raise ImportError(
            "dau_conv: %s not found. Build it with `make -C dau-convnet_amd/csrc` (hipcc, gfx950) or "
            "`python -c 'import __graft_entry__ as g; g.build()'`. There is no CPU fallback." % _LIB_PATH)
    lib = ctypes.CDLL(_LIB_PATH)
    vp, fp, ip = ctypes.c_void_p, ctypes.c_void_p, ctypes.c_void_p
    lib.dau_conv_abi_version.restype = ctypes.c_int
    lib.dau_conv_last_error.restype = ctypes.c_char_p
    lib.dau_conv_build_id.restype = ctypes.c_char_p
    lib.dau_conv_plan_create.argtypes = [ctypes.POINTER(_Desc), ctypes.POINTER(vp)]
    lib.dau_conv_plan_destroy.argtypes = [vp]
    lib.dau_conv_plan_get_info.argtypes = [vp, ctypes.POINTER(_Info)]
    lib.dau_conv_workspace_bytes.argtypes = [vp, ctypes.c_int, ctypes.POINTER(ctypes.c_size_t)]
    lib.dau_conv_forward.argtypes = [vp, vp, fp, fp, fp, fp, fp, fp, vp, ctypes.c_size_t]
    lib.dau_conv_backward.argtypes = [vp, vp] + [fp] * 11 + [vp, ctypes.c_size_t, ctypes.c_int]
    lib.dau_conv_backward_param_sums.argtypes = [vp, vp] + [fp] * 6 + [vp, ctypes.c_size_t]
    lib.dau_conv_finalize_param_grads.argtypes = [vp, vp] + [fp] * 6 + [ctypes.c_int]
    lib.dau_conv_check_status.argtypes = [vp, vp, vp, ctypes.POINTER(ctypes.c_float)]
    if hasattr(lib, "dau_conv_gather_outlier_status"):
        lib.dau_conv_gather_outlier_status.argtypes = [vp, vp, vp, ctypes.POINTER(ctypes.c_int32), ctypes.POINTER(ctypes.c_int32)]
    if hasattr(lib, "dau_conv_gather_line_status"):
        lib.dau_conv_gather_line_status.argtypes = [vp, vp, vp, ctypes.POINTER(ctypes.c_int32), ctypes.POINTER(ctypes.c_int32)]
    if hasattr(lib, "dau_conv_dot_line_status"):
        lib.dau_conv_dot_line_status.argtypes = [vp, vp, vp, ctypes.POINTER(ctypes.c_int32), ctypes.POINTER(ctypes.c_int32)]
    if hasattr(lib, "dau_conv_split_dot_geometry"):
        lib.dau_conv_split_dot_geometry.argtypes = [vp] + [ctypes.POINTER(ctypes.c_int32)] * 3
    if hasattr(lib, "dau_conv_forward_epilogue"):
        lib.dau_conv_epilogue_supported.argtypes = [vp, ctypes.c_int]
        lib.dau_conv_forward_epilogue.argtypes = [vp, vp, fp, fp, fp, fp, fp, fp, ctypes.c_int, fp, vp, ctypes.c_size_t]
        lib.dau_conv_epilogue_backward.argtypes = [vp, vp, fp, fp, ctypes.c_int, fp, fp, vp, ctypes.c_size_t]
    if hasattr(lib, "dau_conv_forward_residual"):
        lib.dau_conv_forward_residual.argtypes = [vp, vp, fp, fp, fp, fp, fp, fp, fp, ctypes.c_int, fp, vp, ctypes.c_size_t]
    if hasattr(lib, "dau_conv_sigma_status"):
        lib.dau_conv_sigma_status.argtypes = [vp] + [ctypes.POINTER(ctypes.c_int32)] * 3
    lib.dau_conv_last_status.argtypes = [vp, ctypes.POINTER(ctypes.c_float), ctypes.POINTER(ctypes.c_int32)]
    lib.dau_conv_filters.argtypes = [vp, vp, fp, fp]
    lib.dau_conv_unit_table.argtypes = [vp, vp, fp, fp, fp, ctypes.c_int, vp]
    lib.dau_conv_filter_support.argtypes = [ctypes.c_float]
    lib.dau_conv_filter_support.restype = ctypes.c_int
    lib.dau_conv_profile_begin.argtypes = [vp]
    lib.dau_conv_profile_end.argtypes = [vp, ctypes.POINTER(ctypes.c_double), ctypes.POINTER(ctypes.c_int32)]
    if lib.dau_conv_abi_version() != 4:
        raise ImportError("dau_conv: ABI version mismatch in %s" % _LIB_PATH)
    return lib


lib = _load()


def filter_support(sigma):
    return int(lib.dau_conv_filter_support(ctypes.c_float(float(sigma))))


def build_id():
    return lib.dau_conv_build_id().decode()


def _check(code):
    if code == DAU_OK:
        return
    msg = lib.dau_conv_last_error().decode("utf-8", "replace")
    raise {DAU_INVALID_ARGUMENT: InvalidArgumentError, DAU_FAILED_PRECONDITION: FailedPreconditionError}.get(
        code, InternalError)(msg)


def _ptr(t):
    return None if t is None else ctypes.c_void_p(t.data_ptr())


def _stream(device):
    return ctypes.c_void_p(torch.cuda.current_stream(device).cuda_stream)


def _same_device(*tensors):
    dev = tensors[0].device
    for t in tensors[1:]:
        if t is not None and t.device != dev:
            raise InvalidArgumentError("all tensors of a call must be on the same device (%s vs %s)" % (dev, t.device))
    return dev


def _req(t, name, shape=None, dtype=torch.float32, memory_format=torch.contiguous_format):
    if not (t.is_cuda and t.dtype == dtype and t.is_contiguous(memory_format=memory_format)):
        raise InvalidArgumentError("%s must be a %s %s tensor on the GPU" % (
            name, "channels_last" if memory_format == torch.channels_last else "contiguous", str(dtype).replace("torch.", "")))
    if shape is not None and tuple(t.shape) != tuple(shape):
        raise InvalidArgumentError("%s has shape %s, expected %s" % (name, tuple(t.shape), tuple(shape)))
    return t


_SHARED_WS = {}


def capturing(device):
    if device.type != "cuda" or not torch.cuda.is_initialized():
        return False
    if device.index is None or device.index == torch.cuda.current_device():
        return torch.cuda.is_current_stream_capturing()
    with torch.cuda.device(device):
        return torch.cuda.is_current_stream_capturing()


def _pool_warmup(device):
    trees = sys.modules.get("torch._inductor.cudagraph_trees")
    if trees is None:
        return False
    try:
        manager = trees.get_manager(device.index, create_if_none_exists=False)
        return manager is not None and bool(manager.in_warmup)
    except AttributeError:
        return False


_Call = collections.namedtuple("_Call", "ws captured transient")
_NO_CALL = _Call(None, False, False)


class Plan(object):

    def __init__(self, N, S, F, G, H, W, max_kernel_size=9, number_units_ignore=0, flags=FLAG_USE_INTERPOLATION,
                 algo=ALGO_AUTO, sigma_hint=0.5, mu_learning_rate_factor=1.0, device=None):
        d = _Desc(ctypes.sizeof(_Desc), N, S, F, G, H, W, int(max_kernel_size), int(number_units_ignore), int(flags),
                  int(algo), float(sigma_hint), float(mu_learning_rate_factor))
        self._h = ctypes.c_void_p()
        if device is not None and torch.cuda.is_available():
            with torch.cuda.device(device):
                _check(lib.dau_conv_plan_create(ctypes.byref(d), ctypes.byref(self._h)))
        else:
            _check(lib.dau_conv_plan_create(ctypes.byref(d), ctypes.byref(self._h)))
        self.N, self.S, self.F, self.G, self.H, self.W = N, S, F, G, H, W
        self.io_dtype = torch.bfloat16 if int(flags) & FLAG_IO_BF16 else torch.float16 if int(flags) & FLAG_IO_F16 else torch.float32
        self._io_format = torch.channels_last if int(flags) & FLAG_IO_NHWC else torch.contiguous_format
        self.input_relu = bool(int(flags) & FLAG_INPUT_RELU)
        info = _Info()
        _check(lib.dau_conv_plan_get_info(self._h, ctypes.byref(info)))
        self.info = {n: getattr(info, n) for n, _ in _Info._fields_}
        self._ws = {}
        self._warm = set()
        self._calls = {}
        self._tls = threading.local()
        self._any_key = None

    def __del__(self):
        h = getattr(self, "_h", None)
        if h and lib is not None:
            lib.dau_conv_plan_destroy(h)
            self._h = None

    def _call(self):
        return self._calls.get(getattr(self._tls, "key", None) or self._any_key, _NO_CALL)

    @property
    def captured(self):
        return self._call().captured

    @property
    def _transient(self):
        return self._call().transient

    @property
    def _last_ws(self):
        return self._call().ws

    @property
    def io_layout(self):
        return "NHWC" if self._io_format == torch.channels_last else "NCHW"

    def workspace_bytes(self, which):
        n = ctypes.c_size_t()
        _check(lib.dau_conv_workspace_bytes(self._h, which, ctypes.byref(n)))
        return n.value

    def _ws_bytes(self, which):
        need = self._ws.get(which)
        if need is None:
            need = self._ws[which] = self.workspace_bytes(which)
        return need

    def _workspace(self, which, device):
# ... 16 lines not shown
        return ws

    def _called(self, ws, device):
        key, captured, transient = self._tls.pending
        self._calls[key] = _Call(None if captured or transient else ws, captured, transient)
        self._tls.key = self._any_key = key
        if not captured:
            self._warm.add(device.index)

    def _status_ws(self, what):
        call = self._call()
        if call.captured:
            raise FailedPreconditionError(
                "DAUConv: %s() reads the workspace of the plan's last call, and that call was captured into a graph (its workspace "
                "belongs to the graph's pool); ask last_status() / sigma_status(), which read the plan's pinned mirror" % what)
        if call.ws is None:
            raise FailedPreconditionError("DAUConv: %s() before any forward / backward call of this plan that kept its workspace" % what)
        return call.ws

    def _status_pair(self, what, query):
        a, b = ctypes.c_int32(), ctypes.c_int32()
        ws = self._status_ws(what)
        dev = ws.device
        with torch.cuda.device(dev):
            _check(getattr(lib, query)(self._h, _stream(dev), _ptr(ws), ctypes.byref(a), ctypes.byref(b)))
        return a.value, b.value

    def epilogue_supported(self, epilogue=EPILOGUE_BIAS | EPILOGUE_RELU):
        if not hasattr(lib, "dau_conv_epilogue_supported"):
            raise InvalidArgumentError("this build of the library has no fused epilogue")
        _check(lib.dau_conv_epilogue_supported(self._h, int(epilogue)))
        return True

    def _residual_supported(self):
        if not hasattr(lib, "dau_conv_forward_residual"):
            raise InvalidArgumentError("this build of the library has no fused residual")
        try:
            return self.epilogue_supported(EPILOGUE_BIAS)
        except InvalidArgumentError as e:
            raise InvalidArgumentError("no fused residual: %s" % e)

    def _req_call(self, x, dy=None, **params):
        _req(x, "input", (self.N, self.S, self.H, self.W), self.io_dtype, self._io_format)
        if dy is not None:
            _req(dy, "grad", (self.N, self.F, self.H, self.W), self.io_dtype, self._io_format)
        for name, t in params.items():
            _req(t, name, (1, self.S, self.G, self.F))

    def _new_grads(self, need_mask, dev):
        return tuple(torch.empty((1, self.S, self.G, self.F), dtype=torch.float32, device=dev) if need_mask & bit else None
                     for bit in (NEED_DW, NEED_DMU1, NEED_DMU2, NEED_DSIGMA))

    def forward(self, x, w, mu1, mu2, sigma, bias=None, relu=False, residual=None):
        if residual is not None:
            self._residual_supported()
            yshape = (self.N, self.F, self.H, self.W)
            if tuple(residual.shape) != yshape:
                raise InvalidArgumentError("residual has shape %s, expected %s" % (tuple(residual.shape), yshape))
            _req(residual, "residual", yshape, self.io_dtype, self._io_format)
        self._req_call(x, weights=w, mu1=mu1, mu2=mu2, sigma=sigma)
        if bias is not None:
            _req(bias, "bias", (self.F,))
        dev = _same_device(x, w, mu1, mu2, sigma, bias, residual)
        epilogue = (EPILOGUE_BIAS if bias is not None else 0) | (EPILOGUE_RELU if relu else 0)
        if epilogue:
            self.epilogue_supported(epilogue)
        with torch.cuda.device(dev):
            y = torch.empty((self.N, self.F, self.H, self.W), dtype=self.io_dtype, device=dev, memory_format=self._io_format)
            ws = self._workspace(PASS_FORWARD, dev)
            if residual is not None:
                _check(lib.dau_conv_forward_residual(self._h, _stream(dev), _ptr(x), _ptr(w), _ptr(mu1), _ptr(mu2), _ptr(sigma),
                                                     _ptr(bias) if bias is not None else None, _ptr(residual), epilogue, _ptr(y),
                                                     _ptr(ws), ws.numel()))
            elif epilogue:
                _check(lib.dau_conv_forward_epilogue(self._h, _stream(dev), _ptr(x), _ptr(w), _ptr(mu1), _ptr(mu2), _ptr(sigma),
                                                     _ptr(bias), epilogue, _ptr(y), _ptr(ws), ws.numel()))
            else:
                _check(lib.dau_conv_forward(self._h, _stream(dev), _ptr(x), _ptr(w), _ptr(mu1), _ptr(mu2), _ptr(sigma), _ptr(y),
                                            _ptr(ws), ws.numel()))
        self._called(ws, dev)
        return y

    def epilogue_backward(self, dy, y=None, relu=False, need_dbias=True, dz=None):
        shape = (self.N, self.F, self.H, self.W)
        _req(dy, "grad", shape, self.io_dtype, self._io_format)
        if relu:
            if y is None:
                raise InvalidArgumentError("epilogue_backward(relu=True) needs the stored y")
            _req(y, "output", shape, self.io_dtype, self._io_format)
            if dz is not None:
                _req(dz, "dz", shape, self.io_dtype, self._io_format)
        dev = _same_device(dy, y if relu else None, dz if relu else None)
        epilogue = (EPILOGUE_BIAS if need_dbias else 0) | (EPILOGUE_RELU if relu else 0)
        if not epilogue:
            return None, None
        with torch.cuda.device(dev):
            if relu and dz is None:
                dz = torch.empty(shape, dtype=self.io_dtype, device=dev, memory_format=self._io_format)
            dbias = torch.empty((self.F,), dtype=torch.float32, device=dev) if need_dbias else None
            need = self._ws_bytes(PASS_EPILOGUE_BACKWARD)
            ws = torch.empty(max(need, 1), dtype=torch.uint8, device=dev) if need_dbias else None
            _check(lib.dau_conv_epilogue_backward(self._h, _stream(dev), _ptr(dy), _ptr(y) if relu else None, epilogue,
                                                  _ptr(dz) if relu else None, _ptr(dbias), _ptr(ws), need if need_dbias else 0))
        return (dz if relu else None), dbias

    def backward(self, x, dy, w, mu1, mu2, sigma, need_mask=NEED_ALL):
        self._req_call(x, dy, weights=w, mu1=mu1, mu2=mu2, sigma=sigma)
        dev = _same_device(x, dy, w, mu1, mu2, sigma)
        with torch.cuda.device(dev):
            dx = torch.empty(x.shape, dtype=self.io_dtype, device=dev, memory_format=self._io_format) if need_mask & NEED_DX else None
            dw, dmu1, dmu2, dsigma = self._new_grads(need_mask, dev)
            ws = self._workspace(PASS_BACKWARD, dev)
            _check(lib.dau_conv_backward(self._h, _stream(dev), _ptr(x), _ptr(dy), _ptr(w), _ptr(mu1), _ptr(mu2), _ptr(sigma),
                                         _ptr(dx), _ptr(dw), _ptr(dmu1), _ptr(dmu2), _ptr(dsigma), _ptr(ws), ws.numel(),
                                         int(need_mask)))
        self._called(ws, dev)
        return dx, dw, dmu1, dmu2, dsigma

    def backward_param_sums(self, x, dy, mu1, mu2, sigma, out=None):
        self._req_call(x, dy, mu1=mu1, mu2=mu2, sigma=sigma)
        dev = _same_device(x, dy, mu1, mu2, sigma, out)
        with torch.cuda.device(dev):
            if out is None:
                out = torch.empty((4, self.S, self.G, self.F), dtype=torch.float32, device=dev)
            _req(out, "sums", (4, self.S, self.G, self.F))
            ws = self._workspace(PASS_BACKWARD, dev)
            _check(lib.dau_conv_backward_param_sums(self._h, _stream(dev), _ptr(x), _ptr(dy), _ptr(mu1), _ptr(mu2), _ptr(sigma),
                                                    _ptr(out), _ptr(ws), ws.numel()))
        self._called(ws, dev)
        return out

    def finalize_param_grads(self, sums, w, need_mask=NEED_DW | NEED_DMU1 | NEED_DMU2 | NEED_DSIGMA):
        _req(sums, "sums", (4, self.S, self.G, self.F))
        _req(w, "weights", (1, self.S, self.G, self.F))
        dev = _same_device(sums, w)
        with torch.cuda.device(dev):
            dw, dmu1, dmu2, dsigma = self._new_grads(need_mask, dev)
            _check(lib.dau_conv_finalize_param_grads(self._h, _stream(dev), _ptr(sums), _ptr(w), _ptr(dw), _ptr(dmu1),
                                                     _ptr(dmu2), _ptr(dsigma), int(need_mask)))
        return dw, dmu1, dmu2, dsigma

    def check_status(self):
        mx = ctypes.c_float()
        ws = self._status_ws("check_status")
        dev = ws.device
        with torch.cuda.device(dev):
            _check(lib.dau_conv_check_status(self._h, _stream(dev), _ptr(ws), ctypes.byref(mx)))
        return mx.value

    def outlier_status(self):
        units, taken = self._status_pair("outlier_status", "dau_conv_gather_outlier_status")
        return units, bool(taken)

    def split_dot_geometry(self):
        v = [ctypes.c_int32() for _ in range(3)]
        _check(lib.dau_conv_split_dot_geometry(self._h, *[ctypes.byref(c) for c in v]))
        return tuple(c.value for c in v)

    def line_status(self):
        return self._status_pair("line_status", "dau_conv_gather_line_status")

    def dot_line_status(self):
        return self._status_pair("dot_line_status", "dau_conv_dot_line_status")

    def last_status(self):
        mx, valid = ctypes.c_float(), ctypes.c_int32()
        _check(lib.dau_conv_last_status(self._h, ctypes.byref(mx), ctypes.byref(valid)))
        return mx.value if valid.value else None

    def sigma_status(self):
        if not hasattr(lib, "dau_conv_sigma_status"):
            return 0, self.info["blur_support"], 0
        v = [ctypes.c_int32() for _ in range(3)]
        _check(lib.dau_conv_sigma_status(self._h, *[ctypes.byref(c) for c in v]))
        return tuple(c.value for c in v)

    def profile_begin(self):
        _check(lib.dau_conv_profile_begin(self._h))

    def profile_end(self):
        ms = (ctypes.c_double * 3)()
        n = (ctypes.c_int32 * 3)()
        _check(lib.dau_conv_profile_end(self._h, ms, n))
        return {name: (ms[i], n[i]) for i, name in enumerate(("gather_sum_fwd", "gather_sum_dx", "gather_dot"))}

    def filters(self, sigma):
        k = self.info["blur_support"]
        out = torch.empty((6, k, k), dtype=torch.float32, device=sigma.device)
        with torch.cuda.device(sigma.device):
            _check(lib.dau_conv_filters(self._h, _stream(sigma.device), _ptr(sigma), _ptr(out)))
        return out

    def unit_table(self, mu1, mu2, w=None, form=0):
        units = self.S * self.G * self.F
        raw = torch.empty((units, 6), dtype=torch.int32, device=mu1.device)
        with torch.cuda.device(mu1.device):
            _check(lib.dau_conv_unit_table(self._h, _stream(mu1.device), _ptr(w), _ptr(mu1), _ptr(mu2), int(form), _ptr(raw)))
        return raw[:, :2].contiguous(), raw[:, 2:].contiguous().view(torch.float32)
```

### include/dau_conv.h

```cpp
#ifndef DAU_CONV_H_
#define DAU_CONV_H_

#include <stddef.h>
#include <stdint.h>

#ifdef __cplusplus
extern "C" {
#endif

#define DAU_CONV_ABI_VERSION 4

#if defined(__GNUC__)
#define DAU_API __attribute__((visibility("default")))
#else
#define DAU_API
#endif

enum {
    DAU_OK = 0,
    DAU_INVALID_ARGUMENT = 1,
    DAU_FAILED_PRECONDITION = 2,
    DAU_INTERNAL = 3
};

enum {
    DAU_FLAG_USE_INTERPOLATION = 1 << 0,
    DAU_FLAG_UNIT_TESTING = 1 << 1,
    DAU_FLAG_SINGLE_DIM_KERNEL = 1 << 2,
    DAU_FLAG_FORBID_POSITIVE_DIM1 = 1 << 3,
    DAU_FLAG_IO_BF16 = 1 << 4,
    DAU_FLAG_STATIC_BUCKET = 1 << 5,
    DAU_FLAG_DENSE_BF16 = 1 << 6,
    DAU_FLAG_DENSE_WGRAD_NEVER = 1 << 7,
    DAU_FLAG_DENSE_WGRAD_ALWAYS = 1 << 8,
    DAU_FLAG_DENSE_SPLIT_F16 = 1 << 9,
    DAU_FLAG_NO_DENSE_SPLIT = 1 << 10,
    DAU_FLAG_IO_F16 = 1 << 11,
    DAU_FLAG_DENSE_SPLIT_OUTLIERS = 1 << 12,
    DAU_FLAG_IO_NHWC = 1 << 13,
    DAU_FLAG_INPUT_RELU = 1 << 14,
    DAU_FLAG_DENSE_SPLIT_LINE = 1 << 15,
    DAU_FLAG_SPLIT_DOT_LINE = 1 << 16,
    DAU_FLAG_DEFAULT = DAU_FLAG_USE_INTERPOLATION
};

enum {
    DAU_ALGO_AUTO = 0,
    DAU_ALGO_DIRECT = 1,
    DAU_ALGO_TILED = 2
};

enum { DAU_PASS_FORWARD = 1, DAU_PASS_BACKWARD = 2, DAU_PASS_EPILOGUE_BACKWARD = 3 };

enum {
    DAU_EPILOGUE_BIAS = 1,
    DAU_EPILOGUE_RELU = 2
};

enum {
    DAU_NEED_DX = 1 << 0,
    DAU_NEED_DW = 1 << 1,
    DAU_NEED_DMU1 = 1 << 2,
    DAU_NEED_DMU2 = 1 << 3,
    DAU_NEED_DSIGMA = 1 << 4,
    DAU_NEED_ALL = 31
};

typedef struct dau_conv_desc {
    int32_t struct_size;
    int32_t batch;
    int32_t in_channels;
    int32_t out_channels;
    int32_t units_per_channel;
    int32_t height, width;
    int32_t max_kernel_size;
    int32_t number_units_ignore;
    int32_t flags;
    int32_t algo;
    float sigma_hint;
    float mu_learning_rate_factor;
} dau_conv_desc;

typedef struct dau_conv_plan dau_conv_plan;

typedef struct dau_conv_plan_info {
    int32_t offset_bucket;
    int32_t blur_support;
    int32_t algo_forward;
    int32_t algo_backward;
    int32_t drop_last_col;
    int32_t drop_last_row;
    int32_t gather_patch;
    int32_t gather_stack;
    int32_t dot_windows;
    int32_t gather_windows;
    int32_t bucket_sets;
    int32_t gather_dense_bf16;
    int32_t batch_slab_gather;
    int32_t batch_slab_dot;
    int32_t dot_region;
    int32_t gather_fblock;
    int32_t gather_variant;
    int32_t dense_bf16_radius3;
    int32_t gather_dense_split;
} dau_conv_plan_info;

DAU_API int dau_conv_abi_version(void);
DAU_API const char *dau_conv_build_id(void);
DAU_API const char *dau_conv_last_error(void);

DAU_API int dau_conv_filter_support(float sigma);

DAU_API int dau_conv_plan_create(const dau_conv_desc *desc, dau_conv_plan **plan_out);
DAU_API int dau_conv_plan_destroy(dau_conv_plan *plan);
DAU_API int dau_conv_plan_get_info(const dau_conv_plan *plan, dau_conv_plan_info *info);
DAU_API int dau_conv_workspace_bytes(const dau_conv_plan *plan, int pass, size_t *bytes_out);
DAU_API int dau_conv_split_dot_geometry(const dau_conv_plan *plan, int32_t *region_width, int32_t *strip_items, int32_t *strip_k_steps);

DAU_API int dau_conv_forward(const dau_conv_plan *plan, void *stream, const float *x, const float *w,
                     const float *mu1, const float *mu2, const float *sigma, float *y,
                     void *workspace, size_t workspace_bytes);

DAU_API int dau_conv_epilogue_supported(const dau_conv_plan *plan, int epilogue);
DAU_API int dau_conv_forward_epilogue(const dau_conv_plan *plan, void *stream, const float *x, const float *w,
                     const float *mu1, const float *mu2, const float *sigma, const float *bias, int epilogue,
                     float *y, void *workspace, size_t workspace_bytes);

DAU_API int dau_conv_forward_residual(const dau_conv_plan *plan, void *stream, const float *x, const float *w,
                     const float *mu1, const float *mu2, const float *sigma, const float *bias, const float *residual,
                     int epilogue, float *y, void *workspace, size_t workspace_bytes);

DAU_API int dau_conv_epilogue_backward(const dau_conv_plan *plan, void *stream, const float *dy, const float *y, int epilogue,
                     float *dz, float *dbias, void *workspace, size_t workspace_bytes);

DAU_API int dau_conv_backward(const dau_conv_plan *plan, void *stream, const float *x, const float *dy,
                      const float *w, const float *mu1, const float *mu2, const float *sigma,
                      float *dx, float *dw, float *dmu1, float *dmu2, float *dsigma,
                      void *workspace, size_t workspace_bytes, int need_mask);

DAU_API int dau_conv_backward_param_sums(const dau_conv_plan *plan, void *stream, const float *x, const float *dy,
                                 const float *mu1, const float *mu2, const float *sigma, float *sums_out,
                                 void *workspace, size_t workspace_bytes);
DAU_API int dau_conv_finalize_param_grads(const dau_conv_plan *plan, void *stream, const float *sums, const float *w,
                                  float *dw, float *dmu1, float *dmu2, float *dsigma, int need_mask);

DAU_API int dau_conv_check_status(const dau_conv_plan *plan, void *stream, const void *workspace,
                          float *max_abs_mu_out);

DAU_API int dau_conv_gather_outlier_status(const dau_conv_plan *plan, void *stream, const void *workspace,
                                   int32_t *outlier_units, int32_t *ring_taken);

DAU_API int dau_conv_gather_line_status(const dau_conv_plan *plan, void *stream, const void *workspace,
                                int32_t *off_line_units, int32_t *line_radius_taken);

DAU_API int dau_conv_dot_line_status(const dau_conv_plan *plan, void *stream, const void *workspace,
                             int32_t *off_line_units, int32_t *line_radius_taken);

DAU_API int dau_conv_last_status(const dau_conv_plan *plan, float *max_abs_mu_out, int32_t *valid_out);

DAU_API int dau_conv_sigma_status(const dau_conv_plan *plan, int32_t *needed_out, int32_t *planned_out, int32_t *worst_needed_out);

DAU_API int dau_conv_filters(const dau_conv_plan *plan, void *stream, const float *sigma, float *filters_out);
DAU_API int dau_conv_unit_table(const dau_conv_plan *plan, void *stream, const float *w, const float *mu1, const float *mu2,
                        int form, void *table_out);

enum { DAU_PROFILE_SLOTS = 3 };
DAU_API int dau_conv_profile_begin(dau_conv_plan *plan);
DAU_API int dau_conv_profile_end(dau_conv_plan *plan, double *ms_out, int32_t *passes_out);

#ifdef __cplusplus
}
#endif
#endif
```

Before: 0.01986.

## Share per-plane dy abs-max between split-dot wgrad and split-gather dx passes

Adds one kernel that computes per-(n,f) plane abs-max of dy once in backward, then feeds it both to the split-dot prepare (seeding emax via the zero kernel instead of a separate dy absmax pass) and to the split-gather dx prepare (scales computed from plane maxima instead of rescanning dy). When several split-gather candidates share bucket set 0, their scale computation is done once under an OR'd guard set. This removes redundant full reads of dy at the cost of extra workspace aliasing and more complex guard logic.

```diff
diff --git a/dau-convnet_amd/csrc/dau_common.hpp b/dau-convnet_amd/csrc/dau_common.hpp
--- a/dau-convnet_amd/csrc/dau_common.hpp
+++ b/dau-convnet_amd/csrc/dau_common.hpp
@@ -184,6 +184,22 @@
     if (g.line == 0) return true;
     const bool on_line = g.status->off_line_units == 0u;
     return g.line > 0 ? on_line : (mx > (float)-g.line || !on_line);
+}
+
+constexpr int kMaxGuards = 4;
+struct GuardSet {
+    Guard g[kMaxGuards];
+    int n = 0;
+};
+inline GuardSet guard_set(const Guard& g) {
+    GuardSet s{};
+    s.g[0] = g; s.n = 1;
+    return s;
+}
+__device__ __forceinline__ bool guard_pass(const GuardSet& s) {
+    bool pass = false;
+    for (int i = 0; i < s.n; ++i) pass = pass || guard_pass(s.g[i]);
+    return pass;
 }
 
 struct UnitRef {
diff --git a/dau-convnet_amd/csrc/dau_conv_api.hip b/dau-convnet_amd/csrc/dau_conv_api.hip
--- a/dau-convnet_amd/csrc/dau_conv_api.hip
+++ b/dau-convnet_amd/csrc/dau_conv_api.hip
@@ -113,26 +113,29 @@
     bool (*configure)(int, int, int, int, int, int, int, int, int, DenseConfig*);
     size_t (*workspace_bytes)(const DenseConfig&);
     void (*init)(const DenseConfig&);
-    void (*prepare)(hipStream_t, const DenseConfig&, const float*, const float*, bool, const UnitRef*, void*, const Guard&);
+    void (*prepare)(hipStream_t, const DenseConfig&, const float*, const float*, bool, const UnitRef*, void*, const Guard&, const SplitShared&);
     void (*run)(hipStream_t, const DenseConfig&, float*, void*, const Guard&, const Epilogue&);
 };
 template <void (*Run)(hipStream_t, const DenseConfig&, float*, void*, const Guard&)>
 void run_plain(hipStream_t st, const DenseConfig& c, float* out, void* ws, const Guard& g, const Epilogue&) { Run(st, c, out, ws, g); }
+template <void (*Prepare)(hipStream_t, const DenseConfig&, const float*, const float*, bool, const UnitRef*, void*, const Guard&)>
+void prepare_plain(hipStream_t st, const DenseConfig& c, const float* in, const float* filters, bool mirrored, const UnitRef* table, void* ws,
+                   const Guard& g, const SplitShared&) { Prepare(st, c, in, filters, mirrored, table, ws, g); }
 const DenseFns kDense[] = {
     {s2::split_gather_configure, s2::split_gather_workspace_bytes, s2::split_gather_init, s2::split_gather_prepare, s2::split_gather_run},
     {s3::split_gather_configure, s3::split_gather_workspace_bytes, s3::split_gather_init, s3::split_gather_prepare, s3::split_gather_run},
     {s4::split_gather_configure, s4::split_gather_workspace_bytes, s4::split_gather_init, s4::split_gather_prepare, s4::split_gather_run},
     {l4::split_gather_configure, l4::split_gather_workspace_bytes, l4::split_gather_init, l4::split_gather_prepare, l4::split_gather_run},
     {l8::split_gather_configure, l8::split_gather_workspace_bytes, l8::split_gather_init, l8::split_gather_prepare, l8::split_gather_run},
-    {r3::dense_gather_configure, r3::dense_gather_workspace_bytes, r3::dense_gather_init, r3::dense_gather_prepare, run_plain<r3::dense_gather_run>},
-    {r4::dense_gather_configure, r4::dense_gather_workspace_bytes, r4::dense_gather_init, r4::dense_gather_prepare, run_plain<r4::dense_gather_run>},
+    {r3::dense_gather_configure, r3::dense_gather_workspace_bytes, r3::dense_gather_init, prepare_plain<r3::dense_gather_prepare>, run_plain<r3::dense_gather_run>},
+    {r4::dense_gather_configure, r4::dense_gather_workspace_bytes, r4::dense_gather_init, prepare_plain<r4::dense_gather_prepare>, run_plain<r4::dense_gather_run>},
 };
 constexpr int kNumDense = sizeof(kDense) / sizeof(kDense[0]);
 struct SplitDotFns {
     bool (*configure)(const Shape&, int, int, SplitDotConfig*);
     size_t (*workspace_bytes)(const SplitDotConfig&);
     void (*init)(const SplitDotConfig&);
-    void (*prepare)(hipStream_t, const SplitDotConfig&, const float*, const float*, const float*, int, int, void*, const Guard&);
+    void (*prepare)(hipStream_t, const SplitDotConfig&, const float*, const float*, const float*, int, int, void*, const Guard&, const unsigned*);
     void (*run)(hipStream_t, const SplitDotConfig&, const UnitRef*, float*, void*, const Guard&);
 };
 const SplitDotFns kSplitDotFns[] = {
@@ -402,6 +405,16 @@
     size_t bytes;
 };
 
+bool is_split_gather(int m) { return m == kSplit2 || m == kSplit3 || m == kSplit4; }
+long dy_maxima_offset(const dau_conv_plan* p, int need_mask) {
+    const BucketSet& s0 = p->sets[0];
+    const int param_mask = DAU_NEED_DW | DAU_NEED_DMU1 | DAU_NEED_DMU2 | DAU_NEED_DSIGMA;
+    const bool both = split_dot_shares_dy_maxima() && p->dynamic && p->algo_fwd == DAU_ALGO_TILED && p->algo_bwd == DAU_ALGO_TILED &&
+                      s0.has[kSplitDot] && (s0.has[kSplit2] || s0.has[kSplit3] || s0.has[kSplit4]) && s0.slab_gather == p->sh.N &&
+                      !(p->d.flags & (DAU_FLAG_IO_NHWC | DAU_FLAG_INPUT_RELU)) && (need_mask & param_mask) && (need_mask & DAU_NEED_DX);
+    return both ? split_dot_plane_max_offset(s0.sdot[kMember[kSplitDot].slot]) : -1;
+}
+
 BwdWs carve_backward(const dau_conv_plan* p, void* ws) {
     Carver c(ws);
     BwdWs w{};
@@ -420,7 +433,7 @@
 }
 
 void run_gather_sum(const dau_conv_plan* p, hipStream_t st, int dir, const float* in, float* out, const float* filters,
-                    const UnitRef* table, Status* status, void* ws, const Epilogue& epi = Epilogue{}) {
+                    const UnitRef* table, Status* status, void* ws, const Epilogue& epi = Epilogue{}, const unsigned* plane_max = nullptr) {
     const Shape& s = p->sh;
     const int cin = dir == kFwd ? s.S : s.F, cout = dir == kFwd ? s.F : s.S;
     const bool mirrored = dir == kDx;
@@ -434,11 +447,24 @@
     }
     Candidate cand[kMaxCandidates];
     const int ncand = pick_candidates(p, status, kGatherSum, cand);
+    SplitShared shared;
+    shared.plane_max = plane_max;
+    for (int ci = 0; ci < ncand && split_dot_shares_dy_maxima(); ++ci)
+        if (is_split_gather(cand[ci].member) && cand[ci].set == &p->sets[0] && cand[ci].set->slab_gather == s.N && shared.guards.n < kMaxGuards)
+            shared.guards.g[shared.guards.n++] = cand[ci].guard;
+    const int sharing = shared.guards.n;
+    if (sharing < 2) shared.guards.n = 0;
+    int split_seen = 0;
     for (int ci = 0; ci < ncand; ++ci) {
         const BucketSet& bs = *cand[ci].set;
         const Guard& g = cand[ci].guard;
         const int m = cand[ci].member;
         const bool ring = cand[ci].ring;
+        if (is_split_gather(m) && sharing >= 2) {
+            shared.scales = split_seen == 0 || split_seen >= sharing;
+            if (split_seen >= sharing) shared.guards.n = 0;
+            ++split_seen;
+        }
         void* ring_ws = ring ? static_cast<char*>(ws) + s3::split_gather_workspace_bytes(bs.ring_dense(dir)) : nullptr;
         if (ring) ring_build_list(st, bs.ringcfg[dir], table, ring_ws, g);
         for (int n0 = 0; n0 < s.N; n0 += bs.slab_gather) {
@@ -458,7 +484,7 @@
             } else {
                 const DenseFns& fn = kDense[kMember[m].slot];
                 const DenseConfig& cfg = bs.dense[kMember[m].slot][dir];
-                fn.prepare(st, cfg, ins, filters, mirrored, table, ws, g);
+                fn.prepare(st, cfg, ins, filters, mirrored, table, ws, g, is_split_gather(m) ? shared : SplitShared{});
                 ProfScope prof(p, dir, st);
                 if (ring) {
                     ring_run(st, bs.ringcfg[dir], s3::split_gather_staged(cfg, ws), ring_ws, status, g);
@@ -762,6 +788,10 @@
     return DAU_OK;
 }
 
+int dau_conv_backward_reads_dy_once(const dau_conv_plan* plan, int need_mask) {
+    return plan && dy_maxima_offset(plan, need_mask) >= 0 ? 1 : 0;
+}
+
 int dau_conv_workspace_bytes(const dau_conv_plan* plan, int pass, size_t* bytes_out) {
     if (!plan || !bytes_out) return fail(DAU_INVALID_ARGUMENT, "null argument");
     if (pass == DAU_PASS_FORWARD) *bytes_out = carve_forward(plan, nullptr).bytes;
@@ -854,7 +884,7 @@
 namespace {
 
 int run_param_sums(const dau_conv_plan* p, hipStream_t st, const float* x, const float* dy, const float* mu1,
-                   const float* mu2, const BwdWs& ws, float* r4, int kinds, const float* w = nullptr) {
+                   const float* mu2, const BwdWs& ws, float* r4, int kinds, const float* w = nullptr, const unsigned* plane_max = nullptr) {
     const Shape& s = p->sh;
     const bool dot_line = p->algo_bwd == DAU_ALGO_TILED && p->dynamic && p->sets[0].has[kDotLine4];
     launch_prepare_units(st, dot_line ? w : nullptr, mu1, mu2, s, p->d.number_units_ignore, p->d.flags, p->bucket, false, ws.table_bare,
@@ -870,7 +900,7 @@
             const int slot = kMember[m].slot;
             if (kMember[m].family == kFamSplitDot) {
                 const SplitDotFns& fn = kSplitDotFns[slot];
-                fn.prepare(st, bs.sdot[slot], x, dy, ws.filters, p->drop_col, p->drop_row, ws.tiled_dot, g);
+                fn.prepare(st, bs.sdot[slot], x, dy, ws.filters, p->drop_col, p->drop_row, ws.tiled_dot, g, m == kSplitDot ? plane_max : nullptr);
                 ProfScope prof(p, 2, st);
                 fn.run(st, bs.sdot[slot], ws.table_bare, r4, ws.tiled_dot, g);
             } else if (kMember[m].family == kFamWgrad) {
@@ -923,8 +953,11 @@
     launch_synth_filters(st, sigma, p->blur_k, flags, ws.filters, p->host_status, ws.status);
 
     const int param_mask = DAU_NEED_DW | DAU_NEED_DMU1 | DAU_NEED_DMU2 | DAU_NEED_DSIGMA;
+    const long plane_off = dy_maxima_offset(p, need_mask);
+    unsigned* plane_max = plane_off >= 0 ? reinterpret_cast<unsigned*>(static_cast<char*>(ws.tiled_dot) + plane_off) : nullptr;
+    if (plane_max) s3::launch_plane_absmax(st, dy, (long)s.N * s.F, (long)s.H * s.W, p->act(), plane_max);
     if (need_mask & param_mask) {
-        run_param_sums(p, st, x, dy, mu1, mu2, ws, ws.r4, (need_mask & DAU_NEED_DSIGMA) ? 4 : 3, w);
+        run_param_sums(p, st, x, dy, mu1, mu2, ws, ws.r4, (need_mask & DAU_NEED_DSIGMA) ? 4 : 3, w, plane_max);
         launch_finalize_grads(st, ws.r4, w, s, p->d.number_units_ignore, p->d.mu_learning_rate_factor, need_mask,
                               flags & DAU_FLAG_SINGLE_DIM_KERNEL, dw, dmu1, dmu2, dsigma);
     }
@@ -934,7 +967,7 @@
                              p->host_status, p->d.number_units_ignore, p->sets[0].has[kLine4] ? ws.status : nullptr);
         Epilogue gate;
         if (flags & DAU_FLAG_INPUT_RELU) gate.gate = x;
-        run_gather_sum(p, st, kDx, dy, dx, ws.filters, ws.table_t, ws.status, ws.gather_dx, gate);
+        run_gather_sum(p, st, kDx, dy, dx, ws.filters, ws.table_t, ws.status, ws.gather_dx, gate, plane_max);
     }
     DAU_HIP(hipPeekAtLastError());
     return DAU_OK;
diff --git a/dau-convnet_amd/csrc/dau_tiled.hpp b/dau-convnet_amd/csrc/dau_tiled.hpp
--- a/dau-convnet_amd/csrc/dau_tiled.hpp
+++ b/dau-convnet_amd/csrc/dau_tiled.hpp
@@ -53,13 +53,19 @@
 DAU_DECLARE_DENSE_GATHER(r4)
 DAU_DECLARE_DENSE_GATHER(r3)
 
+struct SplitShared {
+    const unsigned* plane_max = nullptr;
+    bool scales = true;
+    GuardSet guards;
+};
 #define DAU_DECLARE_SPLIT_GATHER(NS)                                                                                           \
     namespace NS {                                                                                                            \
     bool split_gather_configure(int N, int Cin, int Cout, int G, int H, int W, int R, int blur_k, int act, DenseConfig* cfg);  \
     size_t split_gather_workspace_bytes(const DenseConfig& cfg);                                                              \
     void split_gather_init(const DenseConfig& cfg);                                                                           \
     void split_gather_prepare(hipStream_t st, const DenseConfig& cfg, const float* in, const float* filters, bool mirrored,   \
-                              const UnitRef* table, void* workspace, const Guard& guard);                                     \
+                              const UnitRef* table, void* workspace, const Guard& guard,                                      \
+                              const SplitShared& shared = SplitShared{});                                                     \
                                                       \
     void split_gather_run(hipStream_t st, const DenseConfig& cfg, float* out, void* workspace, const Guard& guard,            \
                           const Epilogue& epi = Epilogue{});                                                                  \
@@ -76,6 +82,7 @@
     int Hs, Ws, nchunk;
 };
 namespace s3 {
+void launch_plane_absmax(hipStream_t st, const float* in, long planes, long HW, int act, unsigned* out);
 SplitStaged split_gather_staged(const DenseConfig& cfg, const void* workspace);
 void split_gather_run_add(hipStream_t st, const DenseConfig& cfg, float* out, const float* partial, void* workspace, const Guard& guard,
                           const Epilogue& epi = Epilogue{});
@@ -141,8 +148,10 @@
 void split_dot_strip(const SplitDotConfig& cfg, int* items, int* k_steps);
 void split_dot_init(const SplitDotConfig& cfg);
 void split_dot_prepare(hipStream_t st, const SplitDotConfig& cfg, const float* x, const float* dy, const float* filters,
-                       int drop_col, int drop_row, void* workspace, const Guard& guard);
+                       int drop_col, int drop_row, void* workspace, const Guard& guard, const unsigned* plane_max = nullptr);
 void split_dot_run(hipStream_t st, const SplitDotConfig& cfg, const UnitRef* table, float* r4, void* workspace, const Guard& guard);
+bool split_dot_shares_dy_maxima();
+long split_dot_plane_max_offset(const SplitDotConfig& cfg);
 #define DAU_DECLARE_SPLIT_DOT_LINE(NS)                                                                                         \
     namespace NS {                                                                                                            \
     bool split_dot_configure(const Shape& sh, int blur_k, int act, SplitDotConfig* cfg);                                      \
@@ -150,7 +159,8 @@
     void split_dot_strip(const SplitDotConfig& cfg, int* items, int* k_steps);                                                \
     void split_dot_init(const SplitDotConfig& cfg);                                                                           \
     void split_dot_prepare(hipStream_t st, const SplitDotConfig& cfg, const float* x, const float* dy, const float* filters,  \
-                           int drop_col, int drop_row, void* workspace, const Guard& guard);                                  \
+                           int drop_col, int drop_row, void* workspace, const Guard& guard,                                   \
+                           const unsigned* plane_max = nullptr);                                                              \
     void split_dot_run(hipStream_t st, const SplitDotConfig& cfg, const UnitRef* table, float* r4, void* workspace,           \
                        const Guard& guard);                                                                                   \
     }
diff --git a/dau-convnet_amd/csrc/k_dense_split.hip b/dau-convnet_amd/csrc/k_dense_split.hip
--- a/dau-convnet_amd/csrc/k_dense_split.hip
+++ b/dau-convnet_amd/csrc/k_dense_split.hip
@@ -146,7 +146,7 @@
 }
 
 __global__ void __launch_bounds__(256) split_absmax_kernel(const float* __restrict__ in, long per, int gpi, int act, const UnitRef* __restrict__ table,
-                                                           long units, unsigned* __restrict__ partial, int cap, const Guard guard, int relu_in) {
+                                                           long units, unsigned* __restrict__ partial, int cap, const GuardSet guard, int relu_in) {
     if (!guard_pass(guard)) return;
     unsigned mx = 0, mw = 0;
     const unsigned keep = relu_in ? 0xffffffffu : 0x7fffffffu, keep_hi = keep & 0xffff0000u;
@@ -205,12 +205,12 @@
     return ldexpf(1.0f, e);
 }
 
-__global__ void __launch_bounds__(256) split_scales_kernel(const unsigned* __restrict__ partial, int N, int gpi, int cap, int G,
-                                                           SplitScales* __restrict__ out, const Guard guard) {
+__global__ void __launch_bounds__(256) split_scales_kernel(const unsigned* __restrict__ image, int N, int gpi, const unsigned* __restrict__ wpartial,
+                                                           int wcnt, int G, SplitScales* __restrict__ out, const GuardSet guard) {
     if (!guard_pass(guard)) return;
     const int n = blockIdx.x;
-    const unsigned* src = n < N ? partial + (long)n * gpi : partial + cap;
-    const int cnt = n < N ? gpi : N * gpi;
+    const unsigned* src = n < N ? image + (long)n * gpi : wpartial;
+    const int cnt = n < N ? gpi : wcnt;
     unsigned m = 0;
     for (int i = threadIdx.x; i < cnt; i += 256) m = max(m, src[i]);
     __shared__ unsigned sm[4];
@@ -226,10 +226,58 @@
         } else {
             const float s = limb_scale(__uint_as_float(m) * (float)G);
             out->max_w_bits = m; out->sw = s; out->inv_sw = 1.0f / s;
-            if constexpr (kLine) { if (guard.status) const_cast<Status*>(guard.status)->line_radius = (unsigned)kDR; }
-        }
-    }
-}
+            if constexpr (kLine) { if (guard.g[0].status) const_cast<Status*>(guard.g[0].status)->line_radius = (unsigned)kDR; }
+        }
+    }
+}
+
+#if DAU_SPLIT_R == 3 && !DAU_SPLIT_1D
+constexpr int kPlaneWaves = 4;
+__global__ void __launch_bounds__(kPlaneWaves * 64) split_plane_absmax_kernel(const float* __restrict__ in, long planes, long per, int act,
+                                                                             unsigned* __restrict__ out) {
+    const long plane = blockIdx.x * (long)kPlaneWaves + (threadIdx.x >> 6);
+    if (plane >= planes) return;
+    const int lane = threadIdx.x & 63;
+    unsigned mx = 0;
+    if (act == kActF16) {
+        auto wide = [](unsigned h) { return finite_bits(__float_as_uint(f16_bits_to_float(h)) & 0x7fffffffu); };
+        const unsigned short* e = reinterpret_cast<const unsigned short*>(in) + plane * per;
+        const long head = absmax_head(e, per, 2, 16), n8 = (per - head) / 8;
+        const uint4* p = reinterpret_cast<const uint4*>(e + head);
+#pragma unroll 4
+        for (long i = lane; i < n8; i += 64) {
+            const uint4 v = p[i];
+            mx = max(max(mx, max(max(wide(v.x & 0xffffu), wide(v.x >> 16)), max(wide(v.y & 0xffffu), wide(v.y >> 16)))),
+                     max(max(wide(v.z & 0xffffu), wide(v.z >> 16)), max(wide(v.w & 0xffffu), wide(v.w >> 16))));
+        }
+        for (long i = lane; i < per - n8 * 8; i += 64) mx = max(mx, wide(e[i < head ? i : i + n8 * 8]));
+    } else if (act == kActBF16) {
+        auto pair = [](unsigned v) { return max(finite_bits((v << 16) & 0x7fffffffu), finite_bits(v & 0x7fff0000u)); };
+        const unsigned short* e = reinterpret_cast<const unsigned short*>(in) + plane * per;
+        const long head = absmax_head(e, per, 2, 16), n8 = (per - head) / 8;
+        const uint4* p = reinterpret_cast<const uint4*>(e + head);
+#pragma unroll 4
+        for (long i = lane; i < n8; i += 64) {
+            const uint4 v = p[i];
+            mx = max(mx, max(max(pair(v.x), pair(v.y)), max(pair(v.z), pair(v.w))));
+        }
+        for (long i = lane; i < per - n8 * 8; i += 64) mx = max(mx, finite_bits(((unsigned)e[i < head ? i : i + n8 * 8] << 16) & 0x7fffffffu));
+    } else {
+        const float* e = in + plane * per;
+        const long head = absmax_head(e, per, 4, 16), n4 = (per - head) / 4;
+        const uint4* p = reinterpret_cast<const uint4*>(e + head);
+#pragma unroll 4
+        for (long i = lane; i < n4; i += 64) {
+            const uint4 v = p[i];
+            mx = max(mx, max(max(finite_bits(v.x & 0x7fffffffu), finite_bits(v.y & 0x7fffffffu)),
+                             max(finite_bits(v.z & 0x7fffffffu), finite_bits(v.w & 0x7fffffffu))));
+        }
+        for (long i = lane; i < per - n4 * 4; i += 64) mx = max(mx, finite_bits(__float_as_uint(e[i < head ? i : i + n4 * 4]) & 0x7fffffffu));
+    }
+    for (int m = 32; m >= 1; m >>= 1) mx = max(mx, (unsigned)__shfl_xor((int)mx, m));
+    if (lane == 0) out[plane] = mx;
+}
+#endif
 
 constexpr int kScT = 64;
 __global__ void __launch_bounds__(kScT) split_densify_kernel(const UnitRef* __restrict__ table, int Cin, int G, int Cout, int CoutP, int nchunk,
@@ -1273,7 +1321,7 @@
 }
 
 void split_gather_prepare(hipStream_t st, const DenseConfig& c, const float* in, const float* filters, bool mirrored,
-                          const UnitRef* table, void* workspace, const Guard& guard) {
+                          const UnitRef* table, void* workspace, const Guard& guard, const SplitShared& shared) {
     const SplitGeom g = split_geometry(c);
     char* ws = static_cast<char*>(workspace);
     SplitScales* sc = reinterpret_cast<SplitScales*>(ws);
@@ -1282,9 +1330,14 @@
     _Float16* wsd = reinterpret_cast<_Float16*>(ws + g.hdr_bytes + g.xs_bytes);
     const long per = (long)c.Cin * c.H * c.W, units = (long)c.Cin * c.G * c.Cout;
     const int gpi = absmax_groups_per_image(c.N, per), cap = kPartials + c.N;
-    hipLaunchKernelGGL(split_absmax_kernel, dim3(c.N * gpi), dim3(256), 0, st, in, per, gpi, c.act, table, units, partial, cap, guard,
-                       (c.in_relu && !mirrored) ? 1 : 0);
-    hipLaunchKernelGGL(split_scales_kernel, dim3(c.N + 1), dim3(256), 0, st, partial, c.N, gpi, cap, c.G, sc, guard);
+    if (shared.scales) {
+        const GuardSet gs = shared.guards.n ? shared.guards : guard_set(guard);
+        const bool planes = shared.plane_max != nullptr;
+        hipLaunchKernelGGL(split_absmax_kernel, dim3(c.N * gpi), dim3(256), 0, st, in, planes ? 0L : per, gpi, c.act, table, units, partial, cap, gs,
+                           (c.in_relu && !mirrored) ? 1 : 0);
+        hipLaunchKernelGGL(split_scales_kernel, dim3(c.N + 1), dim3(256), 0, st, planes ? shared.plane_max : partial, c.N, planes ? c.Cin : gpi,
+                           partial + cap, c.N * gpi, c.G, sc, gs);
+    }
     hipLaunchKernelGGL(split_densify_kernel, dim3(g.nchunk * (g.CoutP / (kScT / 16))), dim3(kScT), 0, st, table, c.Cin, c.G, c.Cout, g.CoutP,
                        g.nchunk, sc, wsd, guard);
     SplitStageArgs s{};
@@ -1357,6 +1410,11 @@
     run_split(st, c, out, partial, workspace, guard, epi);
 }
 
+void launch_plane_absmax(hipStream_t st, const float* in, long planes, long HW, int act, unsigned* out) {
+    hipLaunchKernelGGL(split_plane_absmax_kernel, dim3((unsigned)((planes + kPlaneWaves - 1) / kPlaneWaves)), dim3(kPlaneWaves * 64), 0, st, in,
+                       planes, HW, act, out);
+}
+
 SplitStaged split_gather_staged(const DenseConfig& c, const void* workspace) {
     const SplitGeom g = split_geometry(c);
     const char* ws = static_cast<const char*>(workspace);
diff --git a/dau-convnet_amd/csrc/k_split_dot.hip b/dau-convnet_amd/csrc/k_split_dot.hip
--- a/dau-convnet_amd/csrc/k_split_dot.hip
+++ b/dau-convnet_amd/csrc/k_split_dot.hip
@@ -146,12 +146,28 @@
     }
 }
 
+#ifdef DAU_DY_MAXIMA_REF
 __global__ void __launch_bounds__(256) sd_zero_kernel(unsigned* __restrict__ a, long na, unsigned* __restrict__ b, long nb) {
     for (long i = blockIdx.x * 256L + threadIdx.x; i < na + nb; i += (long)gridDim.x * 256L) {
         if (i < na) a[i] = 0u;
         else b[i - na] = 0u;
     }
 }
+#else
+__global__ void __launch_bounds__(256) sd_zero_kernel(unsigned* __restrict__ a, long na, unsigned* __restrict__ b, long nb,
+                                                      const unsigned* __restrict__ plane_max, int N, int F) {
+    for (long i = blockIdx.x * 256L + threadIdx.x; i < na + nb; i += (long)gridDim.x * 256L) {
+        if (i >= na) { b[i - na] = 0u; continue; }
+        unsigned m = 0u;
+        if (plane_max && i >= na - F) {
+            const unsigned* col = plane_max + (i - (na - F));
+#pragma unroll 8
+            for (int n = 0; n < N; ++n) m = max(m, col[(long)n * F]);
+        }
+        a[i] = m;
+    }
+}
+#endif
 
 __global__ void __launch_bounds__(256) sd_absmax_e_kernel(const float* __restrict__ dy, int N, int F, int HW, int split, int act,
                                                           unsigned* __restrict__ emax, const Guard guard) {
@@ -1103,8 +1119,24 @@
 #endif
 }
 
+#if !DAU_SD_1D
+bool split_dot_shares_dy_maxima() {
+#ifdef DAU_DY_MAXIMA_REF
+    return false;
+#else
+    return true;
+#endif
+}
+long split_dot_plane_max_offset(const SplitDotConfig& c) {
+    const SdGeom g = sd_geom(c);
+    const SdLayout l = sd_layout(c, g);
+    if (!split_dot_shares_dy_maxima() || !sd_walks(c) || (size_t)c.sh.N * c.sh.F * 4 > l.xs_off - l.xk_off) return -1;
+    return (long)l.xk_off;
+}
+#endif
+
 void split_dot_prepare(hipStream_t st, const SplitDotConfig& c, const float* x, const float* dy, const float* filters,
-                       int drop_col, int drop_row, void* workspace, const Guard& guard) {
+                       int drop_col, int drop_row, void* workspace, const Guard& guard, const unsigned* plane_max) {
     const SdGeom g = sd_geom(c);
     const SdLayout l = sd_layout(c, g);
     const Shape& s = c.sh;
@@ -1112,8 +1144,15 @@
     unsigned* xmax = reinterpret_cast<unsigned*>(ws + l.maxes_off);
     unsigned* emax = xmax + s.S * kNumK;
     float* xk = reinterpret_cast<float*>(ws + l.xk_off);
+#ifdef DAU_DY_MAXIMA_REF
+    plane_max = nullptr;
     hipLaunchKernelGGL(sd_zero_kernel, dim3(64), dim3(256), 0, st, xmax, (long)(s.S * kNumK + s.F),
                        reinterpret_cast<unsigned*>(ws + l.partial_off), (long)g.chunks * kNumK * s.S * s.G * s.F);
+#else
+    if (kSdLine || c.nhwc) plane_max = nullptr;
+    hipLaunchKernelGGL(sd_zero_kernel, dim3(64), dim3(256), 0, st, xmax, (long)(s.S * kNumK + s.F),
+                       reinterpret_cast<unsigned*>(ws + l.partial_off), (long)g.chunks * kNumK * s.S * s.G * s.F, plane_max, s.N, s.F);
+#endif
     const int HW = s.H * s.W;
     const bool walks = sd_walks(c);
     h8* xs = reinterpret_cast<h8*>(ws + l.xs_off);
@@ -1125,7 +1164,8 @@
     const int xsplit = std::max(1, std::min(16, 2048 / std::max(1, s.S)));
     hipLaunchKernelGGL(sd_absmax_x_kernel, dim3(s.S * xsplit), dim3(256), 0, st, xk, g.NP, s.S, HW, xsplit, xmax, guard);
 #endif
-    if (c.nhwc) {
+    if (plane_max) {
+    } else if (c.nhwc) {
         const int nfb64 = (s.F + 63) / 64;
         const int esplit = (int)std::max(1L, std::min((long)(2048 / nfb64), ((long)s.N * HW + 3) / 4));
         hipLaunchKernelGGL(sd_absmax_nhwc_e_kernel, dim3(nfb64 * esplit), dim3(256), 0, st, dy, s.N, s.F, HW, esplit, c.act, emax, guard);
diff --git a/dau-convnet_amd/dau_conv/_capi.py b/dau-convnet_amd/dau_conv/_capi.py
--- a/dau-convnet_amd/dau_conv/_capi.py
+++ b/dau-convnet_amd/dau_conv/_capi.py
@@ -94,6 +94,8 @@
         lib.dau_conv_dot_line_status.argtypes = [vp, vp, vp, ctypes.POINTER(ctypes.c_int32), ctypes.POINTER(ctypes.c_int32)]
     if hasattr(lib, "dau_conv_split_dot_geometry"):
         lib.dau_conv_split_dot_geometry.argtypes = [vp] + [ctypes.POINTER(ctypes.c_int32)] * 3
+    if hasattr(lib, "dau_conv_backward_reads_dy_once"):
+        lib.dau_conv_backward_reads_dy_once.argtypes = [vp, ctypes.c_int]
     if hasattr(lib, "dau_conv_forward_epilogue"):
         lib.dau_conv_epilogue_supported.argtypes = [vp, ctypes.c_int]
         lib.dau_conv_forward_epilogue.argtypes = [vp, vp, fp, fp, fp, fp, fp, fp, ctypes.c_int, fp, vp, ctypes.c_size_t]
@@ -416,6 +418,9 @@
         units, taken = self._status_pair("outlier_status", "dau_conv_gather_outlier_status")
         return units, bool(taken)
 
+    def backward_reads_dy_once(self, need_mask=NEED_ALL):
+        return bool(lib.dau_conv_backward_reads_dy_once(self._h, need_mask))
+
     def split_dot_geometry(self):
         v = [ctypes.c_int32() for _ in range(3)]
         _check(lib.dau_conv_split_dot_geometry(self._h, *[ctypes.byref(c) for c in v]))
diff --git a/include/dau_conv.h b/include/dau_conv.h
--- a/include/dau_conv.h
+++ b/include/dau_conv.h
@@ -116,6 +116,7 @@
 DAU_API int dau_conv_plan_get_info(const dau_conv_plan *plan, dau_conv_plan_info *info);
 DAU_API int dau_conv_workspace_bytes(const dau_conv_plan *plan, int pass, size_t *bytes_out);
 DAU_API int dau_conv_split_dot_geometry(const dau_conv_plan *plan, int32_t *region_width, int32_t *strip_items, int32_t *strip_k_steps);
+DAU_API int dau_conv_backward_reads_dy_once(const dau_conv_plan *plan, int need_mask);
 
 DAU_API int dau_conv_forward(const dau_conv_plan *plan, void *stream, const float *x, const float *w,
                      const float *mu1, const float *mu2, const float *sigma, float *y,
```

Result: slower. 0.01938 (-2.4%).
